# HKUDS/GPT-ST

Hardware: AMD Instinct MI355X
Metric: pretrain steps/sec at (B=32,T=12,N=170,C=64) (higher is better)
Workload: dtype f32; 1 GPU; BASELINE configs[1]: PEMS08-shape synthetic pretrain step, per-GPU B=32 T=12 N=170 C=64 base=1, epoch 200/300 (adaptive mask + KL), fwd+loss+bwd+clip+Adam, hipGraph=True, 4 full optimiser steps on 4 different resident batches per graph replay; global_batch=32, parallelism=dp1

## Files before the change

gpt-st_amd/csrc/encin.hip:

```cpp
#include "common.h"

#define EI_T 12
GPTST_STAMP_TABLES(encin)

template <int C>
__global__ __launch_bounds__(256) void encin_fwd_kernel(const float* __restrict__ src, int lda, const float* __restrict__ mask, float fill,
                                                        const float* __restrict__ w, const float* __restrict__ bi, const float* __restrict__ G,
                                                        const float* __restrict__ Wbt, const float* __restrict__ bbt, float* __restrict__ out,
                                                        float* __restrict__ ab, float* __restrict__ wv, int N) {
    constexpr int LPR = C / 4, RPP = 256 / LPR, NQ = 256 / C;
    extern __shared__ __attribute__((aligned(16))) float smem[];
    float* part = smem;
    float* vec = part + NQ * 2 * C;
    float* al = vec + 3 * C;
    float* be = al + N;
    float* mm = be + N;
    const int bt = blockIdx.x, b = bt / EI_T, t = bt % EI_T, tid = threadIdx.x;
    GPTST_WG_BEGIN(); GPTST_STAMP(0);
    {
        const int q = tid / C, o = tid % C;
        const float* W = Wbt + (size_t)bt * C * C;
        float aw = 0.f, abv = 0.f;
#pragma unroll 8
        for (int i = q * (C / NQ); i < (q + 1) * (C / NQ); ++i) {
            const float x = W[(size_t)i * C + o];
            aw = fmaf(w[i], x, aw);
            abv = fmaf(bi[i], x, abv);
        }
        part[(q * 2 + 0) * C + o] = aw;
        part[(q * 2 + 1) * C + o] = abv;
    }
    GPTST_STAMP(1);
    for (int n = tid; n < N; n += 256) {
        float g[EI_T];
        const float* gr = G + (size_t)n * EI_T * EI_T + t * EI_T;
#pragma unroll
        for (int k = 0; k < EI_T / 4; ++k) { const float4 v = ld4(gr + 4 * k); g[4 * k] = v.x; g[4 * k + 1] = v.y; g[4 * k + 2] = v.z; g[4 * k + 3] = v.w; }
        float sv[EI_T], mk[EI_T];
#pragma unroll
        for (int u = 0; u < EI_T; ++u) {
            const size_t r = ((size_t)b * EI_T + u) * N + n;
            sv[u] = src[r * lda];
            mk[u] = mask ? mask[r] : 1.f;
        }
        float a_ = 0.f, b_ = 0.f, mt = 0.f;
#pragma unroll
        for (int u = 0; u < EI_T; ++u) {
            const float m = mk[u] != 0.f ? sv[u] : fill;
            a_ = fmaf(g[u], m, a_);
            b_ += g[u];
            if (u == t) mt = m;
        }
        al[n] = a_; be[n] = b_; mm[n] = mt;
        ab[((size_t)bt * N + n) * 2] = a_;
        ab[((size_t)bt * N + n) * 2 + 1] = b_;
    }
    __syncthreads();
    GPTST_STAMP(2);
    if (tid < C) {
        float s0 = 0.f, s1 = 0.f;
#pragma unroll
        for (int q = 0; q < NQ; ++q) { s0 += part[(q * 2 + 0) * C + tid]; s1 += part[(q * 2 + 1) * C + tid]; }
        vec[tid] = s0; vec[C + tid] = s1; vec[2 * C + tid] = bbt[(size_t)bt * C + tid] + bi[tid];
        wv[(size_t)bt * 2 * C + tid] = s0;
        wv[(size_t)bt * 2 * C + C + tid] = s1;
    }
    __syncthreads();
    const int slot = tid / LPR, c4 = tid % LPR;
    const float4 wW = ld4(vec + 4 * c4), bW = ld4(vec + C + 4 * c4), cst = ld4(vec + 2 * C + 4 * c4), w4 = ld4(w + 4 * c4);
    for (int n = slot; n < N; n += RPP) {
        const float a_ = al[n], b_ = be[n], m = mm[n];
        float4 y = f4fma(a_, wW, f4fma(b_, bW, f4fma(m, w4, cst)));
        y.x = lrelu(y.x); y.y = lrelu(y.y); y.z = lrelu(y.z); y.w = lrelu(y.w);
        st4(out + ((size_t)bt * N + n) * C + 4 * c4, y);
    }
    GPTST_STAMP(3); GPTST_WG_END();
}

template <int C>
__global__ __launch_bounds__(256) void encin_bwd_kernel(const float* __restrict__ dPre, const float* __restrict__ src, int lda,
                                                        const float* __restrict__ mask, float fill, const float* __restrict__ w,
                                                        const float* __restrict__ bi, const float* __restrict__ Wbt, const float* __restrict__ ab,
                                                        const float* __restrict__ wv, float* __restrict__ dWb, float* __restrict__ dG,
                                                        float* __restrict__ dinp, int N, int B) {
    constexpr int LPR = C / 4, RPP = 256 / LPR, U = 4;
    extern __shared__ __attribute__((aligned(16))) float smem[];
    float* red = smem;
    float* vec = red + RPP * 4 * C;
    float* as_ = vec + 6 * C;
    float* cs_ = as_ + N;
    const int bt = blockIdx.x, b = bt / EI_T, t = bt % EI_T, tid = threadIdx.x;
    GPTST_WG_BEGIN(); GPTST_STAMP(0);
    if (tid < 2 * C) vec[4 * C + tid] = wv[(size_t)bt * 2 * C + tid];
    __syncthreads();
    const int slot = tid / LPR, c4 = tid % LPR;
    const float4 wW = ld4(vec + 4 * C + 4 * c4), bW = ld4(vec + 5 * C + 4 * c4);
    float4 A = f4zero(), Bv = f4zero(), Cv = f4zero(), Mv = f4zero();
    for (int n0 = slot; n0 < N; n0 += RPP * U) {
        float4 d[U];
        float a_[U], b_[U], m_[U];
#pragma unroll
        for (int u = 0; u < U; ++u) {
            const int n = min(n0 + u * RPP, N - 1);
            const size_t r = (size_t)bt * N + n;
            d[u] = ld4(dPre + r * C + 4 * c4);
            a_[u] = ab[r * 2]; b_[u] = ab[r * 2 + 1];
            m_[u] = (mask ? mask[r] : 1.f) != 0.f ? src[r * lda] : fill;
        }
#pragma unroll
        for (int u = 0; u < U; ++u) {
            const int n = n0 + u * RPP;
            const bool ok = n < N;
            const float4 dd = ok ? d[u] : f4zero();
            A = f4fma(a_[u], dd, A); Bv = f4fma(b_[u], dd, Bv); Cv = f4add(Cv, dd); Mv = f4fma(m_[u], dd, Mv);
            const float pa = group_sum<LPR>(f4dot(dd, wW)), pc = group_sum<LPR>(f4dot(dd, bW));
            if (ok && c4 == 0) { as_[n] = pa; cs_[n] = pc; }
        }
    }
    GPTST_STAMP(1);
    st4(red + (slot * 4 + 0) * C + 4 * c4, A); st4(red + (slot * 4 + 1) * C + 4 * c4, Bv);
    st4(red + (slot * 4 + 2) * C + 4 * c4, Cv); st4(red + (slot * 4 + 3) * C + 4 * c4, Mv);
    __syncthreads();
    for (int i = tid; i < 4 * C; i += 256) {
        float s = 0.f;
#pragma unroll 4
        for (int sl = 0; sl < RPP; ++sl) s += red[(sl * 4 + i / C) * C + i % C];
        vec[i] = s;
    }
    __syncthreads();
    GPTST_STAMP(2);
    float* row = dWb + (size_t)bt * (C * C + C);
    for (int f = tid; f < C * C / 4; f += 256) {
        const int i = f / LPR, o4 = f % LPR;
        const float wi = w[i], bb = bi[i];
        const float4 a4 = ld4(vec + 4 * o4), b4 = ld4(vec + C + 4 * o4);
        st4(row + (size_t)i * C + 4 * o4, make_float4(fmaf(wi, a4.x, bb * b4.x), fmaf(wi, a4.y, bb * b4.y), fmaf(wi, a4.z, bb * b4.z), fmaf(wi, a4.w, bb * b4.w)));
    }
    if (tid < C) row[C * C + tid] = vec[2 * C + tid];
    {
        constexpr int PP = 256 / C;
        const int i = tid / PP, pq = tid % PP;
        const float* Wr = Wbt + (size_t)bt * C * C + (size_t)i * C + pq * (C / PP);
        float p1 = 0.f, p2 = 0.f;
#pragma unroll
        for (int k = 0; k < C / PP / 4; ++k) {
            const float4 x = ld4(Wr + 4 * k);
            p1 += f4dot(x, ld4(vec + pq * (C / PP) + 4 * k));
            p2 += f4dot(x, ld4(vec + C + pq * (C / PP) + 4 * k));
        }
        p1 = group_sum<PP>(p1); p2 = group_sum<PP>(p2);
        if (pq == 0) {
            dinp[(size_t)bt * 2 * C + i] = vec[3 * C + i] + p1;
            dinp[(size_t)bt * 2 * C + C + i] = vec[2 * C + i] + p2;
        }
    }
    GPTST_STAMP(3);
    for (int n = tid; n < N; n += 256) {
        const float a = as_[n], c = cs_[n];
        float v[EI_T];
#pragma unroll
        for (int u = 0; u < EI_T; ++u) {
            const size_t r = ((size_t)b * EI_T + u) * N + n;
            const float m = (mask ? mask[r] : 1.f) != 0.f ? src[r * lda] : fill;
            v[u] = fmaf(m, a, c);
        }
        float* o = dG + ((size_t)b * N + n) * EI_T * EI_T + t * EI_T;
#pragma unroll
        for (int k = 0; k < EI_T / 4; ++k) st4(o + 4 * k, make_float4(v[4 * k], v[4 * k + 1], v[4 * k + 2], v[4 * k + 3]));
    }
    GPTST_STAMP(4); GPTST_WG_END();
}

extern "C" int gptst_encin_ht1_fwd(const float* src, int lda, const float* mask, float fill, const float* w, const float* bi, const float* G,
                                   const float* Wbt, const float* bbt, float* out, float* ab, float* wv, int B, int T, int N, int C, void* stream) {
    if (!src || !w || !bi || !G || !Wbt || !bbt || !out || !ab || !wv || B <= 0 || N <= 0 || lda <= 0) return GPTST_EARG;
    if (T != EI_T || (C != 64 && C != 128)) return GPTST_ESHAPE;
    const size_t smem = ((size_t)(256 / C) * 2 * C + 3 * C + 3 * (size_t)N) * sizeof(float);
    if (smem > 64 * 1024) return GPTST_ESHAPE;
    if (C == 64) hipLaunchKernelGGL((encin_fwd_kernel<64>), dim3(B * T), dim3(256), smem, (hipStream_t)stream, src, lda, mask, fill, w, bi, G, Wbt, bbt, out, ab, wv, N);
    else hipLaunchKernelGGL((encin_fwd_kernel<128>), dim3(B * T), dim3(256), smem, (hipStream_t)stream, src, lda, mask, fill, w, bi, G, Wbt, bbt, out, ab, wv, N);
    GPTST_CHECK_LAUNCH();
    return GPTST_OK;
}

extern "C" int gptst_encin_ht1_bwd(const float* dPre, const float* src, int lda, const float* mask, float fill, const float* w, const float* bi,
                                   const float* Wbt, const float* ab, const float* wv, float* dWb, float* dG, float* dinp, int B, int T, int N,
                                   int C, void* stream) {
    if (!dPre || !src || !w || !bi || !Wbt || !ab || !wv || !dWb || !dG || !dinp || B <= 0 || N <= 0 || lda <= 0) return GPTST_EARG;
    if (T != EI_T || (C != 64 && C != 128)) return GPTST_ESHAPE;
    const size_t smem = ((size_t)(256 / (C / 4)) * 4 * C + 6 * C + 2 * (size_t)N) * sizeof(float);
    if (smem > 64 * 1024) return GPTST_ESHAPE;
    if (C == 64) hipLaunchKernelGGL((encin_bwd_kernel<64>), dim3(B * T), dim3(256), smem, (hipStream_t)stream, dPre, src, lda, mask, fill, w, bi, Wbt, ab, wv, dWb, dG, dinp, N, B);
    else hipLaunchKernelGGL((encin_bwd_kernel<128>), dim3(B * T), dim3(256), smem, (hipStream_t)stream, dPre, src, lda, mask, fill, w, bi, Wbt, ab, wv, dWb, dG, dinp, N, B);
    GPTST_CHECK_LAUNCH();
    return GPTST_OK;
}
```

gpt-st_amd/csrc/poolgen.hip:

```cpp
#include "common.h"
#include "poolgen_dev.h"
#include <algorithm>
#include <vector>

#define PG_ROWS 16


#ifndef PJ_OCC
#define PJ_OCC 6
#endif

#define PG_MAXROWS 64
template <int V>
__device__ __forceinline__ void pj_fwd(const PJob& a, int bx, int by, int rows, float* __restrict__ embs ) {
    const float* __restrict__ emb = a.emb;
    const float* __restrict__ pool = a.pool;
    float* __restrict__ out = a.out;
    const int cols = a.cols, K = a.K, R = a.R;
    const int r0 = by * rows, nr = min(R, r0 + rows) - r0;
    for (int i = threadIdx.x; i < nr * PG_MAXK; i += 256) {
        const int r = i / PG_MAXK, k = i % PG_MAXK;
        embs[i] = k < K ? emb[(size_t)(r0 + r) * K + k] : 0.f;
    }
    const int c4 = bx * 256 + threadIdx.x;
    const bool ok = V * c4 < cols;
    float4 pv[PG_MAXK];
#pragma unroll
    for (int k = 0; k < PG_MAXK; ++k) pv[k] = (k < K && ok) ? ldv<V>(pool + (size_t)k * cols + V * c4) : f4zero();
    __syncthreads();
    if (!ok) return;
#pragma unroll 2
    for (int r = 0; r < nr; ++r) {
        float4 acc = f4zero();
#pragma unroll
        for (int k = 0; k < PG_MAXK; k += 4) {
            const float4 e = ld4(embs + r * PG_MAXK + k);
            acc = f4fma(e.x, pv[k], acc); acc = f4fma(e.y, pv[k + 1], acc); acc = f4fma(e.z, pv[k + 2], acc); acc = f4fma(e.w, pv[k + 3], acc);
        }
        stv<V>(out + (size_t)(r0 + r) * cols + V * c4, acc);
    }
}




#define PJ_DET_T 1024
__global__ __launch_bounds__(PJ_DET_T) void pool_emb_det_kernel(PJobs t) {
    __shared__ float fold[PJ_DET_T / 64][16][17];
    const int lane = threadIdx.x & 63, wave = threadIdx.x >> 6;
    const int i = lane & 15, kk = lane >> 4;
    int q0 = 0;
    for (int q = 1; q < t.n; ++q) if ((int)blockIdx.x >= t.j[q].blk0) q0 = q;
    const int g0 = t.j[q0].blk0, tile = blockIdx.x - g0;
    f32x4 acc = {0.f, 0.f, 0.f, 0.f};
    int chunk_id = 0, first = q0;
    for (int q = 0; q <= q0; ++q) {
        const PJob& a = t.j[q];
        if (a.blk0 != g0) continue;
        if (q < first) first = q;
        const bool v4 = ((a.cols | a.ldx) & 3) == 0;
        const int nch = (a.cols + 255) / 256;
        for (int ch = 0; ch < nch; ++ch, ++chunk_id) {
            if ((chunk_id & (PJ_DET_T / 64 - 1)) != wave) continue;
            if (v4) pj_emb_accum<4>(a, tile, ch, acc, threadIdx.x); else pj_emb_accum<1>(a, tile, ch, acc, threadIdx.x);
        }
    }
#pragma unroll
    for (int r = 0; r < 4; ++r) fold[wave][kk * 4 + r][i] = acc[r];
    __syncthreads();
    if (threadIdx.x < 256) {
        const int R = t.j[first].R, K = t.j[first].K;
        const int rr = threadIdx.x >> 4, k = threadIdx.x & 15, orow = tile * 16 + rr;
        float s = 0.f;
#pragma unroll
        for (int w = 0; w < PJ_DET_T / 64; ++w) s += fold[w][rr][k];
        if (orow < R && k < K) t.j[first].out[(size_t)orow * K + k] += s;
    }
}

__global__ __launch_bounds__(256, PJ_OCC) void pool_jobs_kernel(PJobs t, int fwd_rows, int fwd_mfma) {
    __shared__ __attribute__((aligned(16))) float fold[4][PG_MAXK][65];
    int p = 0;
    for (int q = 1; q < t.n; ++q) if ((int)blockIdx.x >= t.j[q].blk0) p = q;
    const PJob& a = t.j[p];
    const int rel = blockIdx.x - a.blk0, bx = rel % a.nbx, by = rel / a.nbx;
    const bool v4 = ((a.cols | a.ldx) & 3) == 0;
    if (a.kind == PJ_FWD) {
        if (v4 && fwd_mfma) pj_fwd_mfma(a, bx, by, fwd_mfma, threadIdx.x);
        else if (v4) pj_fwd<4>(a, bx, by, fwd_rows, &fold[0][0][0]);
        else pj_fwd<1>(a, bx, by, fwd_rows, &fold[0][0][0]);
    }
    else if (a.kind == PJ_GRAM) pj_gram(a, rel, &fold[0][0][0], 256);
    else if (a.kind == PJ_BWD_POOL) { if (v4) pj_bwd_pool<4>(a, bx, fold, threadIdx.x); else pj_bwd_pool<1>(a, bx, fold, threadIdx.x); }
// ... 3 lines not shown
thread_local int g_pg_rows = PG_ROWS;
thread_local int g_pg_sort = 1;
thread_local int g_pg_mfma = 1;
static int pj_blocks(PJob& j) {
    const int V = ((j.cols | j.ldx) & 3) ? 1 : 4;
    if (j.kind == PJ_FWD && V == 4 && g_pg_mfma) { j.nbx = (j.cols + 255) / 256; return j.nbx * ((j.R + PG_MFMA_ROWS - 1) / PG_MFMA_ROWS); }
    if (j.kind == PJ_FWD) { j.nbx = ((j.cols + V - 1) / V + 255) / 256; return j.nbx * ((j.R + g_pg_rows - 1) / g_pg_rows); }
    if (j.kind == PJ_GRAM) { const int nb = pj_gram_rows(j.K, j.cols); j.nbx = (j.R + nb - 1) / nb; return j.nbx; }
    if (j.kind == PJ_BWD_POOL) { j.nbx = (j.cols + 16 * V - 1) / (16 * V); return j.nbx; }
    j.nbx = (j.R + 15) / 16;
    return j.nbx * (((j.cols + 255) / 256 + 3) / 4);
}

extern "C" int gptst_pool_jobs_gram_rows(int K, int cols) { return (K <= 0 || K > PG_MAXK || cols <= 0 || cols % 12) ? 0 : pj_gram_rows(K, cols); }

static int pj_launch(PJobs& t, hipStream_t st) {
    int nb = 0;
    for (int p = 0; p < t.n; ++p) {
        PJob& j = t.j[p];
        if (j.R <= 0 || j.K <= 0 || j.K > PG_MAXK || j.cols <= 0 || j.nsplit <= 0 || !j.out) return GPTST_EARG;
        if ((j.kind == PJ_FWD || j.kind == PJ_BWD_POOL || j.kind == PJ_GRAM) && !j.emb) return GPTST_EARG;
        if (j.kind == PJ_GRAM && (!j.pool || j.cols % 12 || pj_gram_rows(j.K, j.cols) <= 0)) return GPTST_EARG;
        if ((j.kind == PJ_BWD_POOL || j.kind == PJ_BWD_EMB) && !j.x) return GPTST_EARG;
        if ((j.kind == PJ_FWD || j.kind == PJ_BWD_EMB) && !j.pool) return GPTST_EARG;
        j.blk0 = nb;
        if (j.ldx <= 0) j.ldx = j.cols;
        if (j.ldx < j.cols) return GPTST_EARG;
        nb += pj_blocks(j);
    }
    if (nb == 0) return GPTST_OK;
    hipLaunchKernelGGL(pool_jobs_kernel, dim3(nb), dim3(256), 0, st, t, g_pg_rows, g_pg_mfma ? PG_MFMA_ROWS : 0);
    GPTST_CHECK_LAUNCH();
    return GPTST_OK;
}

GPTST_INTERNAL int gptst_pj_embed_table(PJobs* t, int njobs, const int* kind, const void* const* emb, const void* const* pool, const void* const* out,
                                        const int* R, const int* K, const int* cols, int* nf, int* nvb, int* ngw) {
    if (njobs > PJ_MAX || !g_pg_mfma) return GPTST_ESHAPE;
    t->n = 0;
    *nf = *nvb = *ngw = 0;
    for (int pass = 0; pass < 2; ++pass) {
        for (int p = 0; p < njobs; ++p) {
            const int kd = kind ? kind[p] : (int)PJ_FWD;
            if (kd != PJ_FWD && kd != PJ_GRAM) return GPTST_ESHAPE;
            if ((kd == PJ_GRAM) != (pass == 1)) continue;
            PJob j{(const float*)emb[p], nullptr, (const float*)pool[p], (float*)out[p], R[p], K[p], cols[p], 1, 0, kd, 0, cols[p]};
            if (!j.emb || !j.pool || !j.out || j.R <= 0 || j.K <= 0 || j.K > PG_MAXK || j.cols <= 0) return GPTST_EARG;
            if (kd == PJ_FWD) {
                if (j.cols & 3) return GPTST_ESHAPE;
                j.blk0 = *nvb; *nvb += pj_blocks(j); ++*nf;
            } else {
                if (j.cols % 12 || pj_gram_rows(j.K, j.cols) <= 0) return GPTST_EARG;
                j.blk0 = *ngw; *ngw += pj_blocks(j);
            }
            t->j[t->n++] = j;
        }
    }
    return GPTST_OK;
}

GPTST_INTERNAL int gptst_pj_reduce_table(PJobs* t, int njobs, const int* kind, const void* const* emb, const void* const* x, const void* const* pool,
                                         const void* const* out, const int* R, const int* K, const int* cols, const int* nsplit, const int* ldx,
                                         int* npool, int* npb, int* neb) {
    if (njobs > PJ_MAX || g_deterministic) return GPTST_ESHAPE;
    t->n = 0;
    *npool = *npb = *neb = 0;
    for (int pass = 0; pass < 2; ++pass) {
        for (int p = 0; p < njobs; ++p) {
            if (kind[p] != PJ_BWD_POOL && kind[p] != PJ_BWD_EMB) return GPTST_ESHAPE;
            if ((kind[p] == PJ_BWD_EMB) != (pass == 1)) continue;
            PJob j{(const float*)emb[p], (const float*)x[p], (const float*)pool[p], (float*)out[p], R[p], K[p], cols[p], nsplit[p], 0, kind[p], 0, ldx ? ldx[p] : 0};
            if (j.R <= 0 || j.K <= 0 || j.K > PG_MAXK || j.cols <= 0 || j.nsplit <= 0 || !j.out || !j.x) return GPTST_EARG;
            if (kind[p] == PJ_BWD_POOL ? !j.emb : !j.pool) return GPTST_EARG;
            if (j.ldx <= 0) j.ldx = j.cols;
            if (j.ldx < j.cols) return GPTST_EARG;
            if (pass == 0) { j.blk0 = *npb; *npb += pj_blocks(j); ++*npool; }
            else { j.blk0 = *neb; *neb += pj_blocks(j); }
            t->j[t->n++] = j;
        }
    }
    return GPTST_OK;
}

extern "C" int gptst_pool_jobs(int njobs, const int* kind, const void* const* emb, const void* const* x, const void* const* pool,
                               const void* const* out, const int* R, const int* K, const int* cols, const int* nsplit, const int* ldx,
                               void* stream) {
    if (njobs < 0 || (njobs && (!kind || !emb || !x || !pool || !out || !R || !K || !cols || !nsplit))) return GPTST_EARG;
    for (int p = 0; p < njobs; ++p) if (kind[p] < PJ_FWD || kind[p] > PJ_GRAM) return GPTST_EARG;
    auto job = [&](int p) {
        return PJob{(const float*)emb[p], (const float*)x[p], (const float*)pool[p], (float*)out[p], R[p], K[p], cols[p], nsplit[p],
                    0, kind[p], 0, ldx ? ldx[p] : 0};
    };
    const bool det = g_deterministic != 0;
    std::vector<int> ord(njobs);
    std::vector<long> cost(njobs);
    for (int p = 0; p < njobs; ++p) {
        ord[p] = p;
        const long rr = (long)R[p] * nsplit[p], cc = cols[p];
        cost[p] = kind[p] == PJ_BWD_POOL ? rr * (cc < 64 ? cc : 64) : kind[p] == PJ_BWD_EMB ? 16L * nsplit[p] * (cc < 1024 ? cc : 1024)
                : kind[p] == PJ_FWD ? 64L * (cc < 256 ? cc : 256) : 1L;
    }
    if (g_pg_sort) std::stable_sort(ord.begin(), ord.end(), [&](int a, int b) { return cost[a] > cost[b]; });
    PJobs t; t.n = 0;
    for (int o = 0; o < njobs; ++o) {
        const int p = ord[o];
        if (det && kind[p] == PJ_BWD_EMB) continue;
        t.j[t.n++] = job(p);
        if (t.n == PJ_MAX) { const int rc = pj_launch(t, (hipStream_t)stream); if (rc) return rc; t.n = 0; }
    }
    if (t.n) { const int rc = pj_launch(t, (hipStream_t)stream); if (rc) return rc; }
    if (!det) return GPTST_OK;
    PJobs g; g.n = 0;
    int nb = 0;
    auto flush = [&]() {
        if (g.n) { hipLaunchKernelGGL(pool_emb_det_kernel, dim3(nb), dim3(PJ_DET_T), 0, (hipStream_t)stream, g); g.n = 0; nb = 0; }
    };
    for (int p = 0; p < njobs; ++p) {
        if (kind[p] != PJ_BWD_EMB) continue;
        bool seen = false;
        for (int q = 0; q < p; ++q) if (kind[q] == PJ_BWD_EMB && out[q] == out[p]) seen = true;
        if (seen) continue;
        int members = 0;
        for (int q = p; q < njobs; ++q) if (kind[q] == PJ_BWD_EMB && out[q] == out[p]) ++members;
        if (members > PJ_MAX) return GPTST_EARG;
        if (g.n + members > PJ_MAX) flush();
        const int tiles = (R[p] + 15) / 16;
        for (int q = p; q < njobs; ++q) {
            if (kind[q] != PJ_BWD_EMB || out[q] != out[p]) continue;
            if (R[q] != R[p] || K[q] != K[p]) return GPTST_EARG;
            PJob j = job(q);
            if (!j.x || !j.pool || !j.out || j.R <= 0 || j.K <= 0 || j.K > PG_MAXK || j.cols <= 0 || j.nsplit <= 0) return GPTST_EARG;
            if (j.ldx <= 0) j.ldx = j.cols;
            if (j.ldx < j.cols) return GPTST_EARG;
            j.blk0 = nb; j.nbx = tiles;
            g.j[g.n++] = j;
        }
        nb += tiles;
    }
    flush();
    GPTST_CHECK_LAUNCH();
    return GPTST_OK;
}

extern thread_local int g_wgrad_ns_override;
extern thread_local int g_wgrad_ns0_override;
extern thread_local int g_apply_v1;
extern thread_local int g_apply_tpw;
extern thread_local int g_tl_nb;
extern thread_local int g_wgrad_v1;
extern thread_local int g_apply128_v1;
extern thread_local int g_apply128_minwg;
extern thread_local int g_tl_mfma;
extern thread_local int g_cap_route_v2;
extern thread_local int g_cap_bwd_noroles;
extern thread_local int g_cap_split;
extern thread_local int g_cap_split_roles;
extern "C" int gptst_tune(int id, int value) {
    if (id == 15) g_tl_mfma = value;
    if (id == 20) g_cap_route_v2 = value;
    if (id == 23) g_cap_bwd_noroles = value;
    if (id == 25) g_cap_split = value;
    if (id == 26) g_cap_split_roles = value;
    if (id == 19) g_pg_sort = value;
    if (id == 1 && value > 0 && value <= PG_MAXROWS) g_pg_rows = value;
    if (id == 6 && value > 0) g_tl_nb = value;
    if (id == 2) g_wgrad_ns_override = value;
    if (id == 5) g_wgrad_ns0_override = value;
    if (id == 3) g_apply_v1 = value;
    if (id == 4) g_apply_tpw = value;
    if (id == 7) g_wgrad_v1 = value;
    if (id == 8) g_apply128_v1 = value;
    if (id == 24 && value > 0) g_apply128_minwg = value;
    if (id == 10) g_pg_mfma = value;
    return GPTST_OK;
}

extern "C" int gptst_poolgen_fwd_multi(const float* emb, int nprob, const void* pools, const void* outs, const int* cols, int R, int K,
                                       void* stream) {
    if (!emb || !pools || !outs || !cols || nprob <= 0 || nprob > PJ_MAX || K > PG_MAXK || K <= 0) return GPTST_EARG;
    PJobs t; t.n = nprob;
    for (int p = 0; p < nprob; ++p)
        t.j[p] = PJob{emb, nullptr, ((const float* const*)pools)[p], ((float* const*)outs)[p], R, K, cols[p], 1, 0, PJ_FWD, 0, 0};
    return pj_launch(t, (hipStream_t)stream);
}

// ... 38 lines not shown
```

gpt-st_amd/csrc/poolgen_dev.h:

```cpp
#pragma once
#include "common.h"

#define PG_MAXK 16
#define PG_MFMA_ROWS 64
#define PJ_MAX 112
enum { PJ_FWD = 0, PJ_BWD_POOL = 1, PJ_BWD_EMB = 2, PJ_GRAM = 3 };
struct PJob {
    const float* emb;
    const float* x;
    const float* pool;
    float* out;
    int R, K, cols, nsplit;
    int blk0, kind, nbx, ldx;
};
struct PJobs { PJob j[PJ_MAX]; int n; };

__device__ __forceinline__ void pj_fwd_mfma(const PJob& a, int bx, int by, int rows, int tid) {
    const float* __restrict__ emb = a.emb;
    const float* __restrict__ pool = a.pool;
    float* __restrict__ out = a.out;
    const int cols = a.cols, K = a.K, R = a.R;
    const int lane = tid & 63, wave = tid >> 6, j = lane & 15, kk = lane >> 4;
    const int c = bx * 256 + wave * 64 + 4 * j;
    if (bx * 256 + wave * 64 >= cols) return;
    const bool cok = c < cols;
    const int nks = (K + 3) >> 2;
    float4 bf[4];
#pragma unroll
    for (int s = 0; s < 4; ++s) bf[s] = (cok && 4 * s + kk < K) ? ld4(pool + (size_t)(4 * s + kk) * cols + c) : f4zero();
    const int r0 = by * rows, r1 = min(R, r0 + rows);
    for (int rt = r0; rt < r1; rt += 16) {
        float av[4];
        const int row = rt + j;
#pragma unroll
        for (int s = 0; s < 4; ++s) av[s] = (row < r1 && 4 * s + kk < K) ? emb[(size_t)row * K + 4 * s + kk] : 0.f;
        f32x4 acc[4];
#pragma unroll
        for (int ct = 0; ct < 4; ++ct) acc[ct] = (f32x4){0.f, 0.f, 0.f, 0.f};
#pragma unroll
        for (int s = 0; s < 4; ++s) {
            if (s < nks) {
                acc[0] = __builtin_amdgcn_mfma_f32_16x16x4f32(av[s], bf[s].x, acc[0], 0, 0, 0);
                acc[1] = __builtin_amdgcn_mfma_f32_16x16x4f32(av[s], bf[s].y, acc[1], 0, 0, 0);
                acc[2] = __builtin_amdgcn_mfma_f32_16x16x4f32(av[s], bf[s].z, acc[2], 0, 0, 0);
                acc[3] = __builtin_amdgcn_mfma_f32_16x16x4f32(av[s], bf[s].w, acc[3], 0, 0, 0);
            }
        }
        if (cok) {
#pragma unroll
            for (int r = 0; r < 4; ++r) {
                const int orow = rt + 4 * kk + r;
                if (orow < r1) st4(out + (size_t)orow * cols + c, make_float4(acc[0][r], acc[1][r], acc[2][r], acc[3][r]));
            }
        }
    }
}

#define PJ_GRAM_SCR (4 * PG_MAXK * 65)
__host__ __device__ inline int pj_gram_rows(int K, int cols) {
    const int nb = (PJ_GRAM_SCR - K * cols) / cols;
    return nb > 16 ? 16 : nb;
}
__device__ __forceinline__ void pj_gram(const PJob& a, int bx, float* __restrict__ scr, int nt) {
    const int K = a.K, cols = a.cols, Hm = cols / 12, NB = pj_gram_rows(K, cols);
    float* pl = scr;
    float* As = scr + K * cols;
    const int r0 = bx * NB, nr = min(NB, a.R - r0);
    for (int i = threadIdx.x; i < K * cols; i += nt) pl[i] = a.pool[i];
    __syncthreads();
    for (int i = threadIdx.x; i < nr * cols; i += nt) {
        const int r = i / cols, c = i % cols;
        const float* __restrict__ e = a.emb + (size_t)(r0 + r) * K;
        float acc = 0.f;
        for (int k = 0; k < K; ++k) acc = fmaf(e[k], pl[k * cols + c], acc);
        As[i] = acc;
    }
    __syncthreads();
    for (int i = threadIdx.x; i < nr * 144; i += nt) {
        const int r = i / 144, t = (i % 144) / 12, u = i % 12;
        const float* ar = As + r * cols;
        float s = 0.f;
        for (int h = 0; h < Hm; ++h) s = fmaf(ar[h * 12 + t], ar[h * 12 + u], s);
        a.out[(size_t)(r0 + r) * 144 + i % 144] = s;
    }
}

#ifndef PJ_UC
#define PJ_UC 4
#endif
#ifndef PJ_NU
#define PJ_NU 4
#endif
template <int V> __device__ __forceinline__ float4 ldv(const float* p) { return ld4(p); }
template <> __device__ __forceinline__ float4 ldv<1>(const float* p) { return make_float4(*p, 0.f, 0.f, 0.f); }
template <int V> __device__ __forceinline__ void stv(float* p, float4 v) { st4(p, v); }
template <> __device__ __forceinline__ void stv<1>(float* p, float4 v) { *p = v.x; }

template <int V>
__device__ __forceinline__ void pj_bwd_pool(const PJob& a, int bx, float (*fold)[PG_MAXK][65], int tid) {
    constexpr int SLAB = 16 * V;
    const float* __restrict__ emb = a.emb;
    const float* __restrict__ dW = a.x;
    float* __restrict__ dpool = a.out;
    const int cols = a.cols, R = a.R, K = a.K, RR = R * a.nsplit;
    const int lane = tid & 63, wave = tid >> 6;
    const int j = lane & 15, kk = lane >> 4;
    int nchunk = 4;
    if (nchunk * 16 > RR) nchunk = (RR + 15) / 16;
    int per = (RR + nchunk - 1) / nchunk;
    per = (per + 3) & ~3;
    const int r0 = wave < nchunk ? wave * per : RR, r1 = min(RR, r0 + per);
    const int c = bx * SLAB + V * j;
    const bool cok = c < cols;
    f32x4 acc[V];
#pragma unroll
    for (int e = 0; e < V; ++e) acc[e] = (f32x4){0.f, 0.f, 0.f, 0.f};
    constexpr int NU = PJ_NU;
    const int cl = cok ? c : 0;
    for (int rb = r0; rb < r1; rb += 4 * NU) {
        float av[NU];
        float4 b[NU];
#pragma unroll
        for (int u = 0; u < NU; ++u) {
            const int row = min(rb + 4 * u + kk, r1 - 1);
            av[u] = emb[(size_t)(row % R) * K + min(j, K - 1)];
            b[u] = ldv<V>(dW + (size_t)row * a.ldx + cl);
        }
        SB();
#pragma unroll
        for (int u = 0; u < NU; ++u) {
            const float a_ = (rb + 4 * u + kk < r1 && j < K) ? av[u] : 0.f;
            acc[0] = __builtin_amdgcn_mfma_f32_16x16x4f32(a_, b[u].x, acc[0], 0, 0, 0);
            if (V == 4) {
                acc[V > 1 ? 1 : 0] = __builtin_amdgcn_mfma_f32_16x16x4f32(a_, b[u].y, acc[V > 1 ? 1 : 0], 0, 0, 0);
                acc[V > 2 ? 2 : 0] = __builtin_amdgcn_mfma_f32_16x16x4f32(a_, b[u].z, acc[V > 2 ? 2 : 0], 0, 0, 0);
                acc[V > 3 ? 3 : 0] = __builtin_amdgcn_mfma_f32_16x16x4f32(a_, b[u].w, acc[V > 3 ? 3 : 0], 0, 0, 0);
            }
        }
    }
#pragma unroll
    for (int e = 0; e < V; ++e)
#pragma unroll
        for (int r = 0; r < 4; ++r) fold[wave][kk * 4 + r][V * j + e] = acc[e][r];
    __syncthreads();
    for (int o = tid; o < PG_MAXK * SLAB; o += 256) {
        const int k = o / SLAB, cc = o % SLAB, col = bx * SLAB + cc;
        if (k < K && col < cols) {
            float* d = dpool + (size_t)k * cols + col;
            *d += (fold[0][k][cc] + fold[1][k][cc]) + (fold[2][k][cc] + fold[3][k][cc]);
        }
    }
}

template <int V>
__device__ __forceinline__ void pj_emb_accum(const PJob& a, int bx, int chunk, f32x4& acc, int tid) {
    constexpr int chunk_cols = 256;
    const int lane = tid & 63;
    const int i = lane & 15, kk = lane >> 4;
    const int R = a.R, K = a.K;
    const int row = bx * 16 + i;
    const float* __restrict__ w = a.x;
    const float* __restrict__ pl = a.pool;
    const int cc = a.cols, ns = a.nsplit, ldx = a.ldx;
    const int cbeg = chunk * chunk_cols, cend = min(cc, cbeg + chunk_cols);
    if (cbeg >= cc) return;
    if (V == 4) {
        constexpr int UC = PJ_UC;
        const int rowc = min(row, R - 1), ic = min(i, K - 1);
        const bool rok = row < R, kok = i < K;
        for (int c0 = cbeg; c0 < cend; c0 += 16 * UC) {
            float4 av[UC], b[UC];
#pragma unroll
            for (int u = 0; u < UC; ++u) {
                const int c = min(c0 + 16 * u + 4 * kk, cc - 4);
                av[u] = ld4(w + (size_t)rowc * ldx + c);
                b[u] = ld4(pl + (size_t)ic * cc + c);
            }
            for (int s = 1; s < ns; ++s) {
#pragma unroll
                for (int u = 0; u < UC; ++u) {
                    const int c = min(c0 + 16 * u + 4 * kk, cc - 4);
                    av[u] = f4add(av[u], ld4(w + ((size_t)s * R + rowc) * ldx + c));
                }
            }
            SB();
#pragma unroll
            for (int u = 0; u < UC; ++u) {
                const bool ok = c0 + 16 * u + 4 * kk < cend;
                const float4 a_ = (ok && rok) ? av[u] : f4zero();
                const float4 b_ = (ok && kok) ? b[u] : f4zero();
                acc = __builtin_amdgcn_mfma_f32_16x16x4f32(a_.x, b_.x, acc, 0, 0, 0);
                acc = __builtin_amdgcn_mfma_f32_16x16x4f32(a_.y, b_.y, acc, 0, 0, 0);
                acc = __builtin_amdgcn_mfma_f32_16x16x4f32(a_.z, b_.z, acc, 0, 0, 0);
                acc = __builtin_amdgcn_mfma_f32_16x16x4f32(a_.w, b_.w, acc, 0, 0, 0);
            }
        }
    } else {
        for (int c = cbeg + kk; c < cend + kk; c += 4) {
            float av = 0.f, b = 0.f;
            if (c < cend) {
                if (row < R) for (int s = 0; s < ns; ++s) av += w[((size_t)s * R + row) * ldx + c];
                if (i < K) b = pl[(size_t)i * cc + c];
            }
            acc = __builtin_amdgcn_mfma_f32_16x16x4f32(av, b, acc, 0, 0, 0);
        }
    }
}

template <int V>
__device__ __forceinline__ void pj_bwd_emb(const PJob& a, int bx, int by, int tid) {
    const int lane = tid & 63, wave = tid >> 6;
    const int i = lane & 15, kk = lane >> 4;
    f32x4 acc = {0.f, 0.f, 0.f, 0.f};
    pj_emb_accum<V>(a, bx, by * 4 + wave, acc, tid);
#pragma unroll
    for (int r = 0; r < 4; ++r) {
        const int orow = bx * 16 + kk * 4 + r;
        if (orow < a.R && i < a.K && (by * 4 + wave) * 256 < a.cols) atomicAdd(a.out + (size_t)orow * a.K + i, acc[r]);
    }
}
```

gpt-st_amd/csrc/timefeat.hip:

```cpp
#include "common.h"

struct TfParams {
    const float *wd, *bd, *ww, *bw, *w1, *b1, *w2, *b2, *w3, *b3;
};
struct TfGrads {
    float *wd, *bd, *ww, *bw, *w1, *b1, *w2, *b2, *w3, *b3;
};

template <int E, int NT = 256> struct TfCfg { static constexpr int ROWS = NT / E; };

template <int E>
__device__ __forceinline__ float tf_matvec(const float (&wrow)[E], float b, const float* __restrict__ xline) {
    float s = b;
#pragma unroll
    for (int i = 0; i < E; ++i) s = fmaf(wrow[i], xline[i], s);
    return s;
}

template <int E>
__device__ __forceinline__ float tf_input(const TfParams& p, const float* __restrict__ tidx, int r, int e, int K) {
    float s = p.bd[e] + p.bw[e];
    for (int k = 0; k < K; ++k) {
        s = fmaf(p.wd[e * K + k], tidx[((size_t)r * K + k) * 2 + 0], s);
        s = fmaf(p.ww[e * K + k], tidx[((size_t)r * K + k) * 2 + 1], s);
    }
    return s;
}

#define TF_SH_FLOATS (7 * 128 * 3)

template <int E>
__device__ __forceinline__ void tf_fwd_body(const TfParams& p, const float* __restrict__ tidx, float* __restrict__ out,
                                            int rows, int K, int blk, float* __restrict__ shraw) {
    constexpr int ROWS = TfCfg<E>::ROWS;
    float (*line)[E + 1] = reinterpret_cast<float (*)[E + 1]>(shraw);
    const int e = threadIdx.x % E, rl = threadIdx.x / E;
    const int r = blk * ROWS + rl;
    const bool valid = r < rows;
    float w1[E], w2[E], w3[E];
#pragma unroll
    for (int i = 0; i < E; ++i) { w1[i] = p.w1[e * E + i]; w2[i] = p.w2[e * E + i]; w3[i] = p.w3[e * E + i]; }
    line[rl][e] = valid ? tf_input<E>(p, tidx, r, e, K) : 0.f;
    __syncthreads();
    float h = fmaxf(tf_matvec<E>(w1, p.b1[e], line[rl]), 0.f);
    __syncthreads();
    line[rl][e] = h;
    __syncthreads();
    h = fmaxf(tf_matvec<E>(w2, p.b2[e], line[rl]), 0.f);
    __syncthreads();
    line[rl][e] = h;
    __syncthreads();
    h = tf_matvec<E>(w3, p.b3[e], line[rl]);
    if (valid) out[(size_t)r * E + e] = h;
}

template <bool DET> __device__ __forceinline__ void tf_add(float* p, float v) { if (DET) *p += v; else atomicAdd(p, v); }

template <int E, bool DET, int NT>
__device__ __forceinline__ void tf_bwd_body(const TfParams& p, const TfGrads& g, const float* __restrict__ tidx,
                                            const float* __restrict__ dout, int rows, int K, int blk, float* __restrict__ shraw) {
    constexpr int ROWS = TfCfg<E, NT>::ROWS;
    float (*sh)[ROWS][E + 1] = reinterpret_cast<float (*)[ROWS][E + 1]>(shraw);
    const int tid = threadIdx.x, e = tid % E, rl = tid / E;
    const int r = blk * ROWS + rl;
    const bool valid = r < rows;
    float w1[E], w2[E], w3[E], c1[E], c2[E], c3[E];
#pragma unroll
    for (int i = 0; i < E; ++i) {
        w1[i] = p.w1[e * E + i]; w2[i] = p.w2[e * E + i]; w3[i] = p.w3[e * E + i];
        c1[i] = p.w1[i * E + e]; c2[i] = p.w2[i * E + e]; c3[i] = p.w3[i * E + e];
    }
    const float h0 = valid ? tf_input<E>(p, tidx, r, e, K) : 0.f;
    sh[0][rl][e] = h0;
    __syncthreads();
    const float h1 = fmaxf(tf_matvec<E>(w1, p.b1[e], sh[0][rl]), 0.f);
    sh[1][rl][e] = h1;
    __syncthreads();
    const float h2 = fmaxf(tf_matvec<E>(w2, p.b2[e], sh[1][rl]), 0.f);
    sh[2][rl][e] = h2;
    const float d3 = valid ? dout[(size_t)r * E + e] : 0.f;
    sh[3][rl][e] = d3;
    __syncthreads();
    const float z2 = h2 > 0.f ? tf_matvec<E>(c3, 0.f, sh[3][rl]) : 0.f;
    sh[4][rl][e] = z2;
    __syncthreads();
    const float z1 = h1 > 0.f ? tf_matvec<E>(c2, 0.f, sh[4][rl]) : 0.f;
    sh[5][rl][e] = z1;
    __syncthreads();
    const float z0 = tf_matvec<E>(c1, 0.f, sh[5][rl]);
    sh[6][rl][e] = z0;
    __syncthreads();
    const int nrow = min(ROWS, rows - blk * ROWS);
    for (int idx = tid; idx < 3 * E * E; idx += NT) {
        const int which = idx / (E * E), eo = (idx / E) % E, i = idx % E;
        const int ga = which == 0 ? 3 : (which == 1 ? 4 : 5), gb = which == 0 ? 2 : (which == 1 ? 1 : 0);
        float s = 0.f;
        for (int rr = 0; rr < nrow; ++rr) s = fmaf(sh[ga][rr][eo], sh[gb][rr][i], s);
        float* dst = which == 0 ? g.w3 : (which == 1 ? g.w2 : g.w1);
        tf_add<DET>(dst + eo * E + i, s);
    }
    for (int idx = tid; idx < 4 * E; idx += NT) {
        const int which = idx / E, eo = idx % E;
        const int ga = which == 0 ? 3 : (which == 1 ? 4 : (which == 2 ? 5 : 6));
        float s = 0.f;
        for (int rr = 0; rr < nrow; ++rr) s += sh[ga][rr][eo];
        if (which == 0) tf_add<DET>(g.b3 + eo, s);
        else if (which == 1) tf_add<DET>(g.b2 + eo, s);
        else if (which == 2) tf_add<DET>(g.b1 + eo, s);
        else { tf_add<DET>(g.bd + eo, s); tf_add<DET>(g.bw + eo, s); }
    }
    for (int idx = tid; idx < 2 * E * K; idx += NT) {
        const int ch = idx / (E * K), eo = (idx / K) % E, k = idx % K;
        float s = 0.f;
        for (int rr = 0; rr < nrow; ++rr)
            s = fmaf(sh[6][rr][eo], tidx[((size_t)(blk * ROWS + rr) * K + k) * 2 + ch], s);
        tf_add<DET>((ch == 0 ? g.wd : g.ww) + eo * K + k, s);
    }
}

#define TF_MAXJ 16
struct TfJob { TfParams p; TfGrads g; const float* tidx; float* out; const float* dout; int rows, K, E, blk0; };
struct TfJobs { TfJob j[TF_MAXJ]; int n; };

#define TF_DET_T 1024
template <int BWD>
__global__ __launch_bounds__(BWD == 2 ? TF_DET_T : 256) void timefeat_jobs_kernel(TfJobs t) {
    constexpr int NT = BWD == 2 ? TF_DET_T : 256;
    __shared__ float shraw[TF_SH_FLOATS * (NT / 256)];
    int q = 0;
    if (BWD == 2) q = blockIdx.x;
    else for (int i = 1; i < t.n; ++i) if ((int)blockIdx.x >= t.j[i].blk0) q = i;
    const TfJob& a = t.j[q];
    const int blk = blockIdx.x - a.blk0;
    const int nblk = (a.rows + NT / a.E - 1) / (NT / a.E);
#define TF_CASE(EE)                                                                              \
    case EE:                                                                                     \
        if (BWD == 2) { for (int b2 = 0; b2 < nblk; ++b2) { tf_bwd_body<EE, true, NT>(a.p, a.g, a.tidx, a.dout, a.rows, a.K, b2, shraw); __syncthreads(); } } \
        else if (BWD == 1) tf_bwd_body<EE, false, NT>(a.p, a.g, a.tidx, a.dout, a.rows, a.K, blk, shraw); \
        else tf_fwd_body<EE>(a.p, a.tidx, a.out, a.rows, a.K, blk, shraw);                       \
        break;
    switch (a.E) { TF_CASE(2) TF_CASE(4) TF_CASE(8) TF_CASE(16) default: break; }
#undef TF_CASE
}

static int tf_launch(TfJobs& t, int bwd, hipStream_t st) {
    int nb = 0;
    for (int q = 0; q < t.n; ++q) {
        TfJob& a = t.j[q];
        if (!a.p.wd || !a.tidx || a.rows <= 0 || a.K <= 0 || (bwd ? (!a.dout || !a.g.wd) : !a.out)) return GPTST_EARG;
        if (a.E != 2 && a.E != 4 && a.E != 8 && a.E != 16) return GPTST_ESHAPE;
        const int rows_per = 256 / a.E;
        a.blk0 = nb;
        nb += (a.rows + rows_per - 1) / rows_per;
    }
    if (bwd && g_deterministic) hipLaunchKernelGGL(timefeat_jobs_kernel<2>, dim3(t.n), dim3(TF_DET_T), 0, st, t);
    else if (bwd) hipLaunchKernelGGL(timefeat_jobs_kernel<1>, dim3(nb), dim3(256), 0, st, t);
    else hipLaunchKernelGGL(timefeat_jobs_kernel<0>, dim3(nb), dim3(256), 0, st, t);
    GPTST_CHECK_LAUNCH();
    return GPTST_OK;
}

extern "C" int gptst_timefeat_fwd(const float* wd, const float* bd, const float* ww, const float* bw, const float* w1, const float* b1,
                                  const float* w2, const float* b2, const float* w3, const float* b3, const float* tidx, float* out,
                                  int rows, int K, int E, void* stream) {
    TfJobs t; t.n = 1;
    t.j[0] = TfJob{TfParams{wd, bd, ww, bw, w1, b1, w2, b2, w3, b3}, TfGrads{}, tidx, out, nullptr, rows, K, E, 0};
    return tf_launch(t, 0, (hipStream_t)stream);
}

extern "C" int gptst_timefeat_bwd(const float* wd, const float* bd, const float* ww, const float* bw, const float* w1, const float* b1,
                                  const float* w2, const float* b2, const float* w3, const float* b3, float* gwd, float* gbd, float* gww,
                                  float* gbw, float* gw1, float* gb1, float* gw2, float* gb2, float* gw3, float* gb3, const float* tidx,
                                  const float* dout, int rows, int K, int E, void* stream) {
    TfJobs t; t.n = 1;
    t.j[0] = TfJob{TfParams{wd, bd, ww, bw, w1, b1, w2, b2, w3, b3}, TfGrads{gwd, gbd, gww, gbw, gw1, gb1, gw2, gb2, gw3, gb3}, tidx,
                   nullptr, dout, rows, K, E, 0};
    return tf_launch(t, 1, (hipStream_t)stream);
}

extern "C" int gptst_timefeat_jobs(int njobs, int bwd, const void* const* params, const void* const* grads, const float* tidx,
                                   const void* const* io, const int* rows, const int* K, const int* E, void* stream) {
    if (njobs <= 0 || njobs > TF_MAXJ || !params || !io || !rows || !K || !E || (bwd && !grads)) return GPTST_EARG;
    TfJobs t; t.n = njobs;
    for (int q = 0; q < njobs; ++q) {
        const float* const* pp = (const float* const*)params + 10 * q;
        TfGrads g{};
        if (bwd) { float* const* gg = (float* const*)grads + 10 * q; g = TfGrads{gg[0], gg[1], gg[2], gg[3], gg[4], gg[5], gg[6], gg[7], gg[8], gg[9]}; }
        t.j[q] = TfJob{TfParams{pp[0], pp[1], pp[2], pp[3], pp[4], pp[5], pp[6], pp[7], pp[8], pp[9]}, g, tidx,
                       bwd ? nullptr : (float*)io[q], bwd ? (const float*)io[q] : nullptr, rows[q], K[q], E[q], 0};
    }
    return tf_launch(t, bwd, (hipStream_t)stream);
}
```

gpt-st_amd/csrc/tmix.hip:

```cpp
#include "common.h"

#define TT 12
#define TT2 144

__global__ __launch_bounds__(256) void gram_fwd_kernel(const float* __restrict__ A, float* __restrict__ G, int N, int Hm) {
    const int idx = blockIdx.x * 256 + threadIdx.x;
    if (idx >= N * TT2) return;
    const int n = idx / TT2, t = (idx % TT2) / TT, u = idx % TT;
    const float* a = A + (size_t)n * Hm * TT;
    float s = 0.f;
    for (int h = 0; h < Hm; ++h) s = fmaf(a[h * TT + t], a[h * TT + u], s);
    G[idx] = s;
}

__global__ __launch_bounds__(256) void gram_bwd_kernel(const float* __restrict__ A, const float* __restrict__ dG,
                                                       float* __restrict__ dA, int N, int Hm, int nsplit) {
    __shared__ float gs[TT2];
    const int gn = blockIdx.x, l = gn / N, n = gn % N;
    if (threadIdx.x < TT2) {
        const float* g = dG + ((size_t)l * nsplit * N + n) * TT2 + threadIdx.x;
        float part[8];
#pragma unroll
        for (int k = 0; k < 8; ++k) part[k] = 0.f;
        for (int sp0 = 0; sp0 < nsplit; sp0 += 8) {
            float v[8];
#pragma unroll
            for (int k = 0; k < 8; ++k) v[k] = sp0 + k < nsplit ? g[(size_t)(sp0 + k) * N * TT2] : 0.f;
#pragma unroll
            for (int k = 0; k < 8; ++k) part[k] += v[k];
        }
        gs[threadIdx.x] = ((part[0] + part[1]) + (part[2] + part[3])) + ((part[4] + part[5]) + (part[6] + part[7]));
    }
    __syncthreads();
    if (threadIdx.x >= Hm * TT) return;
    const int h = threadIdx.x / TT, t = threadIdx.x % TT;
    const float* a = A + ((size_t)gn * Hm + h) * TT;
    float s = 0.f;
#pragma unroll
    for (int u = 0; u < TT; ++u) s = fmaf(a[u], gs[t * TT + u] + gs[u * TT + t], s);
    dA[((size_t)gn * Hm + h) * TT + t] = s;
}

template <int C, bool ADD_DPRE>
__global__ __launch_bounds__(256) void tmix_kernel(const float* __restrict__ X, const float* __restrict__ G,
                                                   const float* __restrict__ dOut, const float* __restrict__ Y,
                                                   float* __restrict__ out, int N) {
    constexpr int LPR = C / 4;
    constexpr int NPB = 256 / LPR;
    __shared__ float Gs[NPB][TT2];
    const int b = blockIdx.y, n0 = blockIdx.x * NPB;
    for (int i = threadIdx.x; i < NPB * TT2; i += 256) {
        const int nl = i / TT2;
        Gs[nl][i % TT2] = (n0 + nl < N) ? G[(size_t)(n0 + nl) * TT2 + i % TT2] : 0.f;
    }
    __syncthreads();
    const int nl = threadIdx.x / LPR, c4 = threadIdx.x % LPR;
    const int n = n0 + nl;
    if (n >= N) return;
    const size_t base = ((size_t)b * TT * N + n) * C + 4 * c4;
    const size_t tstride = (size_t)N * C;
    float4 x[TT];
#pragma unroll
    for (int u = 0; u < TT; ++u) x[u] = ld4(X + base + u * tstride);
#pragma unroll
    for (int t = 0; t < TT; ++t) {
        float4 acc = f4zero();
        if (ADD_DPRE) {
            const float4 d = ld4(dOut + base + t * tstride), y = ld4(Y + base + t * tstride);
            acc = make_float4(d.x * lrelu_grad_from_out(y.x), d.y * lrelu_grad_from_out(y.y),
                              d.z * lrelu_grad_from_out(y.z), d.w * lrelu_grad_from_out(y.w));
        }
#pragma unroll
        for (int u = 0; u < TT; ++u) acc = f4fma(Gs[nl][t * TT + u], x[u], acc);
        st4(out + base + t * tstride, acc);
    }
}

template <int C>
__global__ __launch_bounds__(256) void tmix_dgraph_kernel(const float* __restrict__ dR, const float* __restrict__ X,
                                                          float* __restrict__ dG, int B, int N) {
    __shared__ float red[4][TT2];
    const int n = blockIdx.x, lane = threadIdx.x & 63, wave = threadIdx.x >> 6;
    const int i = lane & 15, kk = lane >> 4;
    f32x4 acc = {0.f, 0.f, 0.f, 0.f};
    const size_t tstride = (size_t)N * C;
    for (int b = wave; b < B; b += 4) {
        const size_t base = ((size_t)b * TT * N + n) * C + 4 * kk;
        float4 a[C / 16], x[C / 16];
#pragma unroll
        for (int q = 0; q < C / 16; ++q) {
            a[q] = f4zero(); x[q] = f4zero();
            if (i < TT) {
                a[q] = ld4(dR + base + i * tstride + 16 * q);
                x[q] = ld4(X + base + i * tstride + 16 * q);
            }
        }
#pragma unroll
        for (int q = 0; q < C / 16; ++q) {
            acc = __builtin_amdgcn_mfma_f32_16x16x4f32(a[q].x, x[q].x, acc, 0, 0, 0);
            acc = __builtin_amdgcn_mfma_f32_16x16x4f32(a[q].y, x[q].y, acc, 0, 0, 0);
            acc = __builtin_amdgcn_mfma_f32_16x16x4f32(a[q].z, x[q].z, acc, 0, 0, 0);
            acc = __builtin_amdgcn_mfma_f32_16x16x4f32(a[q].w, x[q].w, acc, 0, 0, 0);
        }
    }
#pragma unroll
    for (int r = 0; r < 4; ++r) {
        const int t = kk * 4 + r, u = i;
        if (t < TT && u < TT) red[wave][t * TT + u] = acc[r];
    }
    __syncthreads();
    if (threadIdx.x < TT2) {
        const int e = threadIdx.x;
        dG[(size_t)n * TT2 + e] = red[0][e] + red[1][e] + red[2][e] + red[3][e];
    }
}

template <int C, int CH = 0>
__global__ __launch_bounds__(256, 2) void tmix_bwd_dgraph_kernel(const float* __restrict__ dR, const float* __restrict__ X,
                                                                 const float* __restrict__ G, const float* __restrict__ dOut,
                                                                 const float* __restrict__ Y, float* __restrict__ dX,
                                                                 float* __restrict__ dG, int B, int N) {
    constexpr int Q = C / 16, H2 = C / 64, P = C + 4;
    __shared__ float red[4][TT2];
// ... 25 lines not shown
            for (int s = 0; s < 4; ++s)
#pragma unroll
                for (int hf = 0; hf < H2; ++hf) {
                    st4(&tile[wave][0][4 * kk + s][64 * hf + 4 * j], drc[s][hf]);
                    st4(&tile[wave][1][4 * kk + s][64 * hf + 4 * j], xc[s][hf]);
                }
        }
        SB();
        float4 drr[Q], xr[Q];
#pragma unroll
        for (int q = 0; q < Q; ++q) {
            drr[q] = f4zero(); xr[q] = f4zero();
            if (j < TT) { drr[q] = ld4(&tile[wave][0][j][16 * q + 4 * kk]); xr[q] = ld4(&tile[wave][1][j][16 * q + 4 * kk]); }
        }
        SB();
#pragma unroll
        for (int q = 0; q < Q; ++q) {
            g0 = __builtin_amdgcn_mfma_f32_16x16x4f32(drr[q].x, xr[q].x, g0, 0, 0, 0);
            g1 = __builtin_amdgcn_mfma_f32_16x16x4f32(drr[q].y, xr[q].y, g1, 0, 0, 0);
            g2 = __builtin_amdgcn_mfma_f32_16x16x4f32(drr[q].z, xr[q].z, g2, 0, 0, 0);
            g3 = __builtin_amdgcn_mfma_f32_16x16x4f32(drr[q].w, xr[q].w, g3, 0, 0, 0);
        }
        f32x4 acc[4 * H2];
#pragma unroll
        for (int ct = 0; ct < 4 * H2; ++ct) acc[ct] = (f32x4){0.f, 0.f, 0.f, 0.f};
#pragma unroll
        for (int s = 0; s < 4; ++s)
#pragma unroll
            for (int hf = 0; hf < H2; ++hf) {
                acc[4 * hf + 0] = __builtin_amdgcn_mfma_f32_16x16x4f32(ga[s], drc[s][hf].x, acc[4 * hf + 0], 0, 0, 0);
                acc[4 * hf + 1] = __builtin_amdgcn_mfma_f32_16x16x4f32(ga[s], drc[s][hf].y, acc[4 * hf + 1], 0, 0, 0);
                acc[4 * hf + 2] = __builtin_amdgcn_mfma_f32_16x16x4f32(ga[s], drc[s][hf].z, acc[4 * hf + 2], 0, 0, 0);
                acc[4 * hf + 3] = __builtin_amdgcn_mfma_f32_16x16x4f32(ga[s], drc[s][hf].w, acc[4 * hf + 3], 0, 0, 0);
            }
        SB();
        if (kk < 3) {
#pragma unroll
            for (int r = 0; r < 4; ++r)
#pragma unroll
                for (int hf = 0; hf < H2; ++hf) {
                    const float4 d = doc[r][hf];
                    float4 o4;
                    if (CH == 0) {
                        const float4 y = yc[r][hf];
                        o4 = make_float4(fmaf(d.x, lrelu_grad_from_out(y.x), acc[4 * hf + 0][r]), fmaf(d.y, lrelu_grad_from_out(y.y), acc[4 * hf + 1][r]),
                                         fmaf(d.z, lrelu_grad_from_out(y.z), acc[4 * hf + 2][r]), fmaf(d.w, lrelu_grad_from_out(y.w), acc[4 * hf + 3][r]));
                    } else {
                        o4 = make_float4(d.x + acc[4 * hf + 0][r], d.y + acc[4 * hf + 1][r], d.z + acc[4 * hf + 2][r], d.w + acc[4 * hf + 3][r]);
                        if (CH == 2) {
                            const float4 x = xc[r][hf];
                            o4.x *= lrelu_grad_from_out(x.x); o4.y *= lrelu_grad_from_out(x.y); o4.z *= lrelu_grad_from_out(x.z); o4.w *= lrelu_grad_from_out(x.w);
                        }
                    }
                    st4(dX + base + (4 * kk + r) * tstride + 64 * hf + 4 * j, o4);
                }
        }
    }
#pragma unroll
    for (int r = 0; r < 4; ++r) {
        const int t = kk * 4 + r, u = j;
        if (t < TT && u < TT) red[wave][t * TT + u] = (g0[r] + g1[r]) + (g2[r] + g3[r]);
    }
    __syncthreads();
    if (threadIdx.x < TT2) {
        const int e = threadIdx.x;
        dG[(size_t)n * TT2 + e] = (red[0][e] + red[1][e]) + (red[2][e] + red[3][e]);
    }
}

extern "C" int gptst_gram_fwd(const float* A, float* G, int N, int Hm, void* stream) {
    if (!A || !G) return GPTST_EARG;
    hipLaunchKernelGGL(gram_fwd_kernel, dim3((N * TT2 + 255) / 256), dim3(256), 0, (hipStream_t)stream, A, G, N, Hm);
    GPTST_CHECK_LAUNCH();
    return GPTST_OK;
}

extern "C" int gptst_gram_bwd(const float* A, const float* dG, float* dA, int L, int N, int Hm, int nsplit, void* stream) {
    if (!A || !dG || !dA || L <= 0 || N <= 0 || nsplit <= 0 || Hm * TT > 256) return GPTST_EARG;
    hipLaunchKernelGGL(gram_bwd_kernel, dim3(L * N), dim3(256), 0, (hipStream_t)stream, A, dG, dA, N, Hm, nsplit);
    GPTST_CHECK_LAUNCH();
    return GPTST_OK;
}

extern "C" int gptst_tmix_bwd_chain(const float* dR, const float* X, const float* G, const float* dPre, int premul, float* dX, float* dG,
                                    int B, int T, int N, int C, void* stream) {
    if (!dR || !X || !G || !dPre || !dX || !dG || T != TT || B < 1 || N < 1) return GPTST_EARG;
    hipStream_t st = (hipStream_t)stream;
    if (C == 64 && premul) hipLaunchKernelGGL((tmix_bwd_dgraph_kernel<64, 2>), dim3(N), dim3(256), 0, st, dR, X, G, dPre, nullptr, dX, dG, B, N);
    else if (C == 64) hipLaunchKernelGGL((tmix_bwd_dgraph_kernel<64, 1>), dim3(N), dim3(256), 0, st, dR, X, G, dPre, nullptr, dX, dG, B, N);
    else if (C == 128 && premul) hipLaunchKernelGGL((tmix_bwd_dgraph_kernel<128, 2>), dim3(N), dim3(256), 0, st, dR, X, G, dPre, nullptr, dX, dG, B, N);
    else if (C == 128) hipLaunchKernelGGL((tmix_bwd_dgraph_kernel<128, 1>), dim3(N), dim3(256), 0, st, dR, X, G, dPre, nullptr, dX, dG, B, N);
    else return GPTST_ESHAPE;
    GPTST_CHECK_LAUNCH();
    return GPTST_OK;
}

extern "C" int gptst_tmix(const float* X, const float* G, const float* dOut, const float* Y, float* out, int B, int T, int N,
                          int C, void* stream) {
    if (!X || !G || !out || T != TT) return GPTST_EARG;
    if (dOut && !Y) return GPTST_EARG;
    hipStream_t st = (hipStream_t)stream;
    if (C == 64) {
        dim3 grid((N + 15) / 16, B);
        if (dOut) hipLaunchKernelGGL((tmix_kernel<64, true>), grid, dim3(256), 0, st, X, G, dOut, Y, out, N);
        else hipLaunchKernelGGL((tmix_kernel<64, false>), grid, dim3(256), 0, st, X, G, dOut, Y, out, N);
    } else if (C == 128) {
        dim3 grid((N + 7) / 8, B);
        if (dOut) hipLaunchKernelGGL((tmix_kernel<128, true>), grid, dim3(256), 0, st, X, G, dOut, Y, out, N);
        else hipLaunchKernelGGL((tmix_kernel<128, false>), grid, dim3(256), 0, st, X, G, dOut, Y, out, N);
    } else return GPTST_ESHAPE;
    GPTST_CHECK_LAUNCH();
    return GPTST_OK;
}

extern "C" int gptst_tmix_dgraph(const float* dR, const float* X, float* dG, int B, int T, int N, int C, void* stream) {
    if (!dR || !X || !dG || T != TT) return GPTST_EARG;
    hipStream_t st = (hipStream_t)stream;
    if (C == 64) hipLaunchKernelGGL((tmix_dgraph_kernel<64>), dim3(N), dim3(256), 0, st, dR, X, dG, B, N);
    else if (C == 128) hipLaunchKernelGGL((tmix_dgraph_kernel<128>), dim3(N), dim3(256), 0, st, dR, X, dG, B, N);
    else return GPTST_ESHAPE;
    GPTST_CHECK_LAUNCH();
    return GPTST_OK;
}

extern "C" int gptst_tmix_bwd(const float* dR, const float* X, const float* G, const float* dOut, const float* Y, float* dX, float* dG,
                              int B, int T, int N, int C, void* stream) {
    if (!dR || !X || !G || !dOut || !Y || !dX || !dG || T != TT || B < 1 || N < 1) return GPTST_EARG;
    hipStream_t st = (hipStream_t)stream;
    if (C == 64) hipLaunchKernelGGL((tmix_bwd_dgraph_kernel<64>), dim3(N), dim3(256), 0, st, dR, X, G, dOut, Y, dX, dG, B, N);
    else if (C == 128) hipLaunchKernelGGL((tmix_bwd_dgraph_kernel<128>), dim3(N), dim3(256), 0, st, dR, X, G, dOut, Y, dX, dG, B, N);
    else return GPTST_ESHAPE;
    GPTST_CHECK_LAUNCH();
    return GPTST_OK;
}
```

gpt-st_amd/engine.py:

```python
import contextlib
import gc
import os
import threading
from typing import Any, NamedTuple

import torch

from . import _C, ops
from .ops import (EPI_ADD_DPRE, EPI_ADD_PREMUL, EPI_LRELU, EPI_PREMUL, EPI_PLAIN, EPI_RES_LRELU, MODE_NODE, MODE_SHARED, MODE_TIME, PRO_DPRE, PRO_NONE)

TF_NAMES = ("ln_day", "ln_week", "ln1", "ln2", "ln")


class ZeroArena:

    def __init__(self, device):
        self.device, self.buf, self.off, self.need = device, None, 0, 0

    def begin(self, zero=True):
        pending = None
        if self.buf is None or self.buf.numel() < self.need:
            self.buf = torch.zeros(max(self.need, 1), device=self.device) if self.need else None
        elif self.buf is not None:
            if zero:
                self.buf.zero_()
            else:
                pending = self.buf
        self.off, self.need = 0, 0
        return pending

    def zeros(self, *shape):
        n = 1
        for d in shape:
            n *= d
        n4 = (n + 3) // 4 * 4
        self.need += n4
        if self.buf is None or self.off + n4 > self.buf.numel():
            return torch.zeros(*shape, device=self.device)
        t = self.buf[self.off:self.off + n].view(*shape)
        self.off += n4
        return t


class _Context(threading.local):
    ARENA = None
    NODE_REDUCE = None
    NO_HANDOFFS = False


CTX = _Context()




class Reductions:

    def __init__(self):
        self.jobs = ops.PoolJobs()
        self.late = ops.PoolJobs()
        self.no_carry = False
        self.grams = []
        self.tf = []
        self.keep = []
        self.on_bucket = None
        self.nbucket = 0
        self.bucket_inline = False
        self.fork_side = None
        self.forked = False
        self._dG = self._dA = None

    def take_carry(self, mb):
        if not CARRY_RED or self.no_carry or self.on_bucket is not None or CTX.NODE_REDUCE is not None or not self.jobs.jobs:
            return None
        take, rest, nb = [], [], 0.0
        for j in self.jobs.jobs:
            b = 4.0 * j.R * j.cols * j.nsplit / 2 ** 20
            if j.kind in (ops.PoolJobs.BWD_POOL, ops.PoolJobs.BWD_EMB) and nb + b <= mb and len(take) < 100 and (j.cols | j.ldx) % 4 == 0:
                take.append(j); nb += b
            else:
                rest.append(j)
        if not take:
            return None
        self.jobs.jobs = rest
        c = ops.PoolJobs()
        c.jobs = take
        return c

    def untake(self, carry):
        if carry is not None and carry.jobs:
            self.jobs.jobs = carry.jobs + self.jobs.jobs
            carry.jobs = []

    def gram(self, A, dG, dA, N, nsG):
        self.grams.append((A, dG, dA, N, nsG))

    def timefeat(self, p, g, pfx, tidx, dout, spg=False):
        self.tf.append(_tf_job(p, pfx, tidx, spg)._replace(grads=_tf_tensors(g, pfx), dout=dout))

    def flush_async(self, tidx):
        if self.bucket_inline and self.on_bucket is not None and self.nbucket == 0 and (self.jobs.jobs or self.late.jobs or self.grams or self.tf):
            self._run(tidx)
            self.fork_side.wait_stream(torch.cuda.current_stream())
            with torch.cuda.stream(self.fork_side):
                self.on_bucket(0)
            self.forked = True
            self.nbucket += 1

    def flush(self, tidx):
        self._run(tidx)
        if self.forked:
            torch.cuda.current_stream().wait_stream(self.fork_side)
            self.forked = False

    def _run(self, tidx):
        gr, self.grams = sorted(self.grams, key=lambda t: t[0].data_ptr()), []
        while gr:
            A, dG, dA, N, nsG = gr.pop(0)
            while gr and gr[0][0].data_ptr() == A.data_ptr() + 4 * A.numel() and gr[0][1].data_ptr() == dG.data_ptr() + 4 * dG.numel() \
                    and gr[0][2].data_ptr() == dA.data_ptr() + 4 * dA.numel() and gr[0][3:] == (N, nsG):
                A2, dG2, dA2 = gr.pop(0)[:3]
                A = torch.as_strided(A, (A.shape[0] + A2.shape[0],) + tuple(A.shape[1:]), A.stride())
                dG = torch.as_strided(dG, (dG.shape[0] + dG2.shape[0],) + tuple(dG.shape[1:]), dG.stride())
                dA = torch.as_strided(dA, (dA.shape[0] + dA2.shape[0],) + tuple(dA.shape[1:]), dA.stride())
            ops.gram_bwd(A, dG, out=dA, layers=A.shape[0] // N, nsplit=nsG)
        self.jobs.jobs, self.late.jobs = self.jobs.jobs + self.late.jobs, []
        self.jobs.launch()
        tf, self.tf = self.tf, []
        ops.timefeat_jobs_bwd(tf, tidx)
        self.keep = []


def _zeros(ref, *shape):
    if CTX.ARENA is not None:
        return CTX.ARENA.zeros(*shape)
    return torch.zeros(*shape, device=ref.device)


def _tf_tensors(d, pfx):
    out = []
    for n in TF_NAMES:
        out += [d[pfx + n + ".weight"], d[pfx + n + ".bias"]]
    return out


def _tf_job(p, pfx, tidx, spg=False):
    B, T = tidx.shape[0], tidx.shape[1]
    rows, K = (B, T) if spg else (B * T, 1)
    return ops.TimefeatJob(_tf_tensors(p, pfx), rows, K)


DROP_R = os.environ.get("GPTST_DROP_R", "0") == "1"


class HtSaved(NamedTuple):
    x: Any
    R: Any
    out: Any
    G: Any
    Wbt: Any


class WgradParts(NamedTuple):
    dW: Any
    ns: int
    db: Any


def _ht_fused_bwd(dims):
    return dims[3] == 64 and FUSE_HT_BWD


def hypertem_core_fwd(x, G, Wbt, bbt, dims):
    B, T, N, C = dims
    if C == 64:
        keep = not (DROP_R and _ht_fused_bwd(dims) and ops.wgrad_nsplit(MODE_TIME, B * T, N, C) == 1)
        R, out = ops.hypertem_fwd(x.view(B, T, N, C), G, Wbt, bbt, want_R=keep)
        R, out = (R.view(-1, C) if keep else None), out.view(-1, C)
    else:
        R = ops.tmix(x.view(B, T, N, C), G).view(-1, C)
        out = ops.apply(R, Wbt, MODE_TIME, B * T, N, bias=bbt, resid=x, epi=EPI_RES_LRELU)
    return out, HtSaved(x, R, out, G, Wbt)


FUSE_HT_BWD = True


def graph_grad_splits(dims):
    return dims[0] if dims[3] == 64 else 1


CHAIN128 = os.environ.get("GPTST_CHAIN128", "1") == "1"


def chain_ok(dims):
    return _ht_fused_bwd(dims) or (CHAIN128 and dims[3] == 128)


def _wb_parts(dWb, C, ns=1):
    return WgradParts(dWb[:, :C * C], ns, dWb[:, C * C:])


def _wgrad_parts(a, dout, out, mode, dims):
    B, T, N, C = dims
    dWb, ns = ops.wgrad(a, dout, mode, B * T, N, D2=out, pro=PRO_NONE if out is None else PRO_DPRE, colsum_d=True)
    return _wb_parts(dWb, C, ns)


def _genlin_bwd(dout, out, x, W, mode, dims, chain, premul=False):
    B, T, N, C = dims
    BT = B * T
    if C == 64:
        dx, dW, db, ns = ops.apply_wgrad(dout, None if chain else out, x, W, mode, BT, N, premul=chain and premul)
        return dx, WgradParts(dW, ns, db)
    if chain:
        dx = (ops.apply(dout, W, mode, BT, N, transw=True, resid2=x, epi=EPI_PREMUL) if premul
              else ops.apply(dout, W, mode, BT, N, transw=True))
        return dx, _wgrad_parts(x, dout, None, mode, dims)
    dx = ops.apply(dout, W, mode, BT, N, A2=out, transw=True, pro=PRO_DPRE)
    return dx, _wgrad_parts(x, dout, out, mode, dims)


def hypertem_core_bwd(saved, dout, dG_out, dims, chain=False, premul=False):
    B, T, N, C = dims
    x, R, out, G, Wbt = saved
    BT = B * T
    v = lambda a: a.view(B, T, N, C)
    assert not chain or chain_ok(dims)
    if _ht_fused_bwd(dims):
        dx, dWb, ns, _ = ops.hypertem_bwd_wgrad(v(dout), None if chain else v(out), v(x), G, Wbt, v(R) if R is not None else None, dG=dG_out,
                                                premul=chain and premul)
        return dx.view(-1, C), _wb_parts(dWb, C, ns)
    hp = _wgrad_parts(R, dout, None if chain else out, MODE_TIME, dims)
    if C == 64:
        dx, _, _ = ops.hypertem_bwd(v(dout), v(out), v(x), G, Wbt, dG=dG_out, want_dbias=False)
    elif chain:
        dR = ops.apply(dout, Wbt, MODE_TIME, BT, N, transw=True)
        dx, _ = ops.tmix_bwd_chain(v(dR), v(x), G, v(dout), premul=premul, dG=dG_out[0])
    else:
        dR = ops.apply(dout, Wbt, MODE_TIME, BT, N, A2=out, transw=True, pro=PRO_DPRE)
        dx, _ = ops.tmix_bwd(v(dR), v(x), G, v(dout), v(out), dG=dG_out[0])
    return dx.view(-1, C), hp


CARRY_RED = os.environ.get("GPTST_CARRY_RED", "1") == "1"
CARRY_MB = float(os.environ.get("GPTST_CARRY_MB", "25"))
CARRY_KL = os.environ.get("GPTST_CARRY_KL", "1") == "1"
PAIR_UNDER_DP = os.environ.get("GPTST_PAIR_UNDER_DP", "1") == "1"
PAIR_BWD = os.environ.get("GPTST_PAIR_BWD", "1") == "1"


@contextlib.contextmanager
def no_handoffs():
    from . import _C
    keep = (CTX.NO_HANDOFFS, _C.lib().value("gptst_mask_cooperative_state"))
    CTX.NO_HANDOFFS = True
    _C.lib().call("gptst_mask_cooperative", 0)
    try:
        yield
    finally:
        CTX.NO_HANDOFFS = keep[0]
        _C.lib().call("gptst_mask_cooperative", keep[1])


def pair_bwd_on():
    return PAIR_BWD and not CTX.NO_HANDOFFS


def cross_role():
    return 0 if CTX.NO_HANDOFFS else CROSS_ROLE


def _ht_pair_shape_ok(dims):
    B, T, N, C = dims
    if T != 12 or C != 64:
        return False
    ns = ops.wgrad_nsplit(MODE_TIME, B * T, N, C)
    rps = (-(-N // ns) + 1) & ~1
    return -(-N // rps) == ns


def ht_pair_ok(saved1, saved0, dims):
    return (pair_bwd_on() and dims[3] == 64 and not isinstance(saved1, EncIn) and saved1.R is not None and saved0.R is not None
            and _ht_fused_bwd(dims) and _ht_pair_shape_ok(dims))


class PendingH1:

    def __init__(self, saved, dd, dG, dWb):
        self.saved, self.dd, self.dG, self.dWb = saved, dd, dG, dWb


def ht_pair_bwd(saved1, saved0, dout, dG1, dG0, dims, dWb1=None):
    B, T, N, C = dims
    if not ht_pair_ok(saved1, saved0, dims):
        assert dWb1 is None
        return None
    s1, s0 = saved1, saved0
    v = lambda a: a.view(B, T, N, C)
    r = ops.hypertem_bwd_pair(v(dout), v(s1.x), s1.G, s1.Wbt, v(s1.R), v(s0.x), s0.G, s0.Wbt, v(s0.R), dG1, dG0, _zeros(dout, B), dWb1=dWb1)
    assert r is not None or dWb1 is None
    if r is None:
        return None
    dmid, dx0, dWb1, dWb0, ns = r
    return dx0.view(-1, C), _wb_parts(dWb1, C, ns), _wb_parts(dWb0, C, ns)


FUSE_CROSS = os.environ.get("GPTST_FUSE_CROSS", "1") == "1"
CAP_LIN = os.environ.get("GPTST_CAP_LIN", "1") == "1"
CROSS_ROLE = int(os.environ.get("GPTST_CROSS_ROLE", "1"))


class CapSaved(NamedTuple):
    x: Any
    out: Any
    rec: Any
    c: Any
    s: Any
    v: Any
    Ht: Any
    Rt: Any
    dyn: Any
    Wn: Any
    Y: Any


class CapParts(NamedTuple):
    wn: WgradParts
    ddyn: Any
    dlogit: Any


def cap_head_fwd(p, pfx, x, dadj, dyn, dims, num_route, HS, HT):
    B, T, N, C = dims
    c, s, Y = ops.cap_route_fwd(x.view(B, T, N, C), p[pfx + "ln_p.weight"], p[pfx + "ln_p.bias"], dadj, HS, num_route,
                                reduce_nodes=CTX.NODE_REDUCE, want_Y=True)
    fused = ops.cap_cross_rec_fwd(s, dyn, p[pfx + "mask_template"], c, B, T, N, HS, HT) if (FUSE_CROSS and CTX.NODE_REDUCE is None) else None
    if fused is not None:
        v, Ht, Rt, rec = fused
    else:
        v, Ht, Rt = ops.cap_cross_fwd(s, dyn, p[pfx + "mask_template"], B, T, HS, HT)
        rec = ops.cap_rec_fwd(c, v, N, C)
    return rec, c, (s, v, Ht, Rt, Y)


def cap_core_fwd(p, pfx, x, dadj, dyn, Wn, bn, dims, num_route, HS, HT):
    B, T, N, C = dims
    rec, c, (s, v, Ht, Rt, Y) = cap_head_fwd(p, pfx, x, dadj, dyn, dims, num_route, HS, HT)
    out = ops.apply(rec, Wn, MODE_NODE, B * T, N, bias=bn, resid=x, epi=EPI_RES_LRELU)
    return out, c, CapSaved(x, out, rec, c, s, v, Ht, Rt, dyn, Wn, Y)


CHAIN_FWD = os.environ.get("GPTST_CHAIN_FWD", "1") == "1"
# ... 198 lines not shown
        adj0 = p[which[0] + "hyperTem1.adj"]
        Hm = adj0.shape[1]
        A_all = torch.empty(L, N, Hm * T, device=tidx.device)
        G_all = torch.empty(L, N, T, T, device=tidx.device)
        for k, pfx in enumerate(which):
            sthcn[pfx] = _sthcn_gen_jobs(p, pfx, embs[3 * k:3 * k + 3], jobs, A_all[4 * k:4 * k + 4], dims, G_all[4 * k:4 * k + 4], (k, len(which)))
    now.launch()
    return GenAll(sthcn, gd, jobs if defer else None)


def sthcn_fwd(p, pfx, tidx, x, dims, num_route, gen=None, head=None, next_gen=None, kl=None):
    if gen is None:
        gen = gen_all(p, tidx, dims, which=(pfx,), guide=False).sthcn[pfx]
    ht = gen.ht
    cap = lambda i, x: cap_core_fwd(p, gen.cps[i], x, gen.dadj[i], gen.dyn[i], *gen.Wn[i], dims, num_route, gen.HS, gen.HT)
    pairs = chain_fwd_ok(dims)
    nhead = None
    x, h1 = head if head is not None else hypertem_core_fwd(x, *ht(0), dims)
    x, c1, sc1 = cap(0, x)
    if pairs:
        if kl is not None and kl.c1 is None:
            kl.c1 = c1
        (h2, h3), x = ht_chain_fwd(x, [ht(1), ht(2)], dims, kl)
    else:
        x, h2 = hypertem_core_fwd(x, *ht(1), dims)
        x, h3 = hypertem_core_fwd(x, *ht(2), dims)
    x, _, sc2 = cap(1, x)
    if pairs and next_gen is not None:
        (h4, h1n), xn = ht_chain_fwd(x, [ht(3), next_gen.ht(0)], dims, kl)
        x, nhead = h4.out, (xn, h1n)
    else:
        x, h4 = hypertem_core_fwd(x, *ht(3), dims)
    return x, c1, SthcnSaved(h1, h2, h3, h4, sc1, sc2, gen.emb, gen, gen.slot), nhead


def _grad_buffers(red, slot, N, T, HmT, ref, nsG):
    if slot is None:
        return torch.empty(4, nsG, N, T, T, device=ref.device), torch.empty(4, N, HmT, device=ref.device)
    k, n = slot
    if red._dG is None or red._dG.shape[0] != 4 * n:
        red._dG = torch.empty(4 * n, nsG, N, T, T, device=ref.device)
        red._dA = torch.empty(4 * n, N, HmT, device=ref.device)
    return red._dG[4 * k:4 * k + 4], red._dA[4 * k:4 * k + 4]


def sthcn_bwd(p, g, pfx, tidx, sv, dout, dims, red, chain=False, premul_in=False, defer_h1=False, after_pending=None):
    B, T, N, C = dims
    time_eb, teb, tes = sv.emb
    gn = sv.gen
    A_all, hts, cps, d, Hm, ds, HS, HT = gn.A_all, gn.hts, gn.cps, gn.d, gn.Hm, gn.ds, gn.HS, gn.HT
    ne, nes = p[pfx + "node_embeddings"], p[pfx + "node_embeddings_spg"]
    dne, dnes = g[pfx + "node_embeddings"], g[pfx + "node_embeddings_spg"]
    d_te, d_teb, d_tes = _zeros(time_eb, *time_eb.shape), _zeros(teb, *teb.shape), _zeros(tes, *tes.shape)
    nsG = graph_grad_splits(dims)
    dG_all, dA_all = _grad_buffers(red, sv.slot, N, T, Hm * T, dout, nsG)
    J = red.jobs
    e_te, e_node, e_spg, e_teb = (time_eb, d_te), (nes, dnes), (tes, d_tes), (teb, d_teb)

    if isinstance(dout, PendingH1):
        up = dout
        dd, _, hp4 = ht_pair_bwd(up.saved, sv.h4, up.dd, up.dG, dG_all[3], dims, dWb1=up.dWb)
        red.keep.append(up)
        if after_pending is not None:
            after_pending()
    else:
        dd, hp4 = hypertem_core_bwd(sv.h4, dout, dG_all[3], dims, chain, True)
    queue_ht(J, p, g, hts[3], hp4, *e_te)
    dd, cp2 = cap_core_bwd(p, g, cps[1], sv.c2, dd, dims, HS, HT, red, chain)
    queue_cap(J, p, g, cps[1], cp2, e_node, e_spg, e_teb)
    pair = ht_pair_bwd(sv.h3, sv.h2, dd, dG_all[2], dG_all[1], dims) if chain and pair_bwd_on() else None
    if pair is not None:
        dd, hp3, hp2 = pair
    else:
        dd, hp3 = hypertem_core_bwd(sv.h3, dd, dG_all[2], dims, chain, True)
        dd, hp2 = hypertem_core_bwd(sv.h2, dd, dG_all[1], dims, chain, True)
    queue_ht(J, p, g, hts[2], hp3, *e_te)
    queue_ht(J, p, g, hts[1], hp2, *e_te)
    dd, cp1 = cap_core_bwd(p, g, cps[0], sv.c1, dd, dims, HS, HT, red, chain)
    queue_cap(J, p, g, cps[0], cp1, e_node, e_spg, e_teb)
    if isinstance(sv.h1, EncIn):
        assert chain
        e = sv.h1
        w, bi = p["encoder.dim_in_flow.weight"], p["encoder.dim_in_flow.bias"]
        if nsG == B:
            dWb, _, dinp = ops.encin_ht1_bwd(dd.view(B, T, N, C), e.source, e.mask, e.fill, w, bi, e.Wbt, e.ab, e.wv, dG=dG_all[0])
        else:
            dWb, dGb, dinp = ops.encin_ht1_bwd(dd.view(B, T, N, C), e.source, e.mask, e.fill, w, bi, e.Wbt, e.ab, e.wv)
            torch.sum(dGb, 0, out=dG_all[0][0])
        hp1 = _wb_parts(dWb, C)
        wb = _wb_view(g["encoder.dim_in_flow.weight"], g["encoder.dim_in_flow.bias"])
        if wb is not None:
            red.jobs.bwd_pool(_ones(dd.device, dinp.shape[0]), dinp, wb)
        else:
            g["encoder.dim_in_flow.weight"].add_(dinp[:, :C].sum(0).view(C, 1))
            g["encoder.dim_in_flow.bias"].add_(dinp[:, C:].sum(0))
        red.keep.append((dinp, dWb))
        dd = None
    elif defer_h1:
        assert chain and premul_in
        ns = ops.wgrad_nsplit(MODE_TIME, B * T, N, C)
        dWb = torch.empty(ns * B * T, C * C + C, device=dd.device, dtype=torch.float32)
        hp1 = _wb_parts(dWb, C, ns)
        dd = PendingH1(sv.h1, dd, dG_all[0], dWb)
    else:
        dd, hp1 = hypertem_core_bwd(sv.h1, dd, dG_all[0], dims, chain, premul_in)
    queue_ht(J, p, g, hts[0], hp1, *e_te)
    red.gram(A_all.view(4 * N, Hm, T), dG_all, dA_all.view(4 * N, Hm, T), N, nsG)
    for i, h in enumerate(hts):
        red.late.bwd_pool(ne, dA_all[i], g[h + "adj"].view(d, Hm * T))
        red.late.bwd_emb(dA_all[i], p[h + "adj"].view(d, Hm * T), dne)
    red.timefeat(p, g, pfx + "time_feature1.", tidx, d_te)
    red.timefeat(p, g, pfx + "time_feature1_.", tidx, d_teb)
    red.timefeat(p, g, pfx + "time_feature2.", tidx, d_tes, spg=True)
    red.keep.append((sv, hp1, hp2, hp3, hp4, cp1, cp2, dout))
    return dd


class EncIn:

    def __init__(self, source, mask, fill, Wbt, ab, wv):
        self.source, self.mask, self.fill, self.Wbt, self.ab, self.wv = source, mask, fill, Wbt, ab, wv


ENCIN = os.environ.get("GPTST_ENCIN", "1") == "1"


def encin_ok(dims, base):
    return ENCIN and base == 1 and dims[3] in (64, 128) and dims[1] == 12 and chain_ok(dims)


GUIDEIN = os.environ.get("GPTST_GUIDEIN", "1") == "1"
GUIDE_HEAD = os.environ.get("GPTST_GUIDE_HEAD", "1") == "1"


class LowRankIn(NamedTuple):
    Wspa: Any


class GuideSaved(NamedTuple):
    t4m: Any
    spa: Any
    tem: Any
    h2: Any
    label: Any


def guide_fwd(p, source, tidx, dims, base, gen=None, lowrank_in=False):
    B, T, N, C = dims
    if gen is None:
        gen = gen_all(p, tidx, dims, which=(), guide=True).guide
    t4m, Wspa, bspa, Wtem, btem = gen
    m = "encoder.MLP_RL."
    if lowrank_in and GUIDEIN and GUIDE_HEAD and base == 1 and C == 64:
        r = ops.guide_head_fwd(source, p[m + "ln1.weight"], p[m + "ln1.bias"], Wspa, bspa, Wtem, btem, p[m + "ln3.weight"], p[m + "ln3.bias"])
        if r is not None:
            h1, h2, prob, label = r
            return prob, GuideSaved(t4m, LowRankIn(Wspa), CondLinSaved(h1, h2, Wtem), h2, label)
    if lowrank_in and GUIDEIN and base == 1 and C in (64, 128):
        h1 = ops.guide_in_fwd(source, p[m + "ln1.weight"], p[m + "ln1.bias"], Wspa, bspa)
        s1 = LowRankIn(Wspa)
    else:
        h0 = ops.lin_in(source, base + 2, base, p[m + "ln1.weight"], p[m + "ln1.bias"], C)
        h1, s1 = condlin_fwd(h0, Wspa, bspa, MODE_NODE, dims)
    h2, s2 = condlin_fwd(h1, Wtem, btem, MODE_TIME, dims)
    prob, label = ops.rowdot(h2, p[m + "ln3.weight"], p[m + "ln3.bias"], softmax=True, want_label=True)
    return prob, GuideSaved(t4m, s1, s2, h2, label)


# ... 114 lines not shown
            ts = [dh2, h1, Wtem, dh1, dW, db]
        else:
            dh1, _ = self.out.tem
            dWb, dinp = torch.empty(N, C * C + C, **f), torch.empty(N, 2 * C, **f)
            self.out.inp = (dWb, dinp)
            ts = [dh1, self.source, p[m + "ln1.weight"], p[m + "ln1.bias"], sv_g.spa.Wspa, dWb, dinp]
        self.stage = st
        return (st, ts, 0, ops.kl_guest_blocks(st, B, T, N), HS, self.source.shape[-1], self.w)


def _in_proj_grads(source, base, dY, gW, gb, mask, fill, red):
    wb = _wb_view(gW, gb)
    if base == 1 and wb is not None:
        C = dY.shape[1]
        part = ops.rowouter_part(source, base + 2, base, dY, mask=mask, fill=fill)
        red.jobs.bwd_pool(_ones(dY.device, part.shape[0]), part[:, :2 * C], wb)
        red.keep.append(part)
    else:
        ops.rowouter(source, base + 2, base, dY, gW, 0, csum=gb, mask=mask, fill=fill)


class Forward(NamedTuple):
    emb: Any
    c1: Any
    dec: Any
    out: Any
    sv_e: Any
    sv_d: Any


def autoencoder_fwd(p, source, mask, dims, base, num_route, scaler_zeros, gen=None, tidx=None, lowrank_in=False, kl=None, head=True,
                    decoder=True, join=True):
    B, T, N, C = dims
    if tidx is None:
        tidx = source[:, :, 0, base:base + 2].contiguous()
    gen_e, gen_d = (gen.sthcn[ENC], gen.sthcn[DEC] if decoder else None) if gen is not None else (None, None)
    first = None
    if lowrank_in and gen_e is not None and encin_ok(dims, base):
        w, bi = p["encoder.dim_in_flow.weight"], p["encoder.dim_in_flow.bias"]
        G1, Wbt1, bbt1 = gen_e.ht(0)
        o1, ab, wv = ops.encin_ht1_fwd(source, base, mask, 0.0 if mask is None else scaler_zeros, w, bi, G1, Wbt1, bbt1)
        first = (o1.view(-1, C), EncIn(source, mask, 0.0 if mask is None else scaler_zeros, Wbt1, ab, wv))
        x0 = None
    else:
        x0 = ops.lin_in(source, base + 2, base, p["encoder.dim_in_flow.weight"], p["encoder.dim_in_flow.bias"], C,
                        mask=mask, fill=scaler_zeros)
    emb, c1, sv_e, dec_h1 = sthcn_fwd(p, ENC, tidx, x0, dims, num_route, gen=gen_e, head=first, next_gen=gen_d if join else None, kl=kl)
    if not decoder:
        return Forward(emb, c1, None, None, sv_e, None)
    dec, _, sv_d, _ = sthcn_fwd(p, DEC, tidx, emb, dims, num_route, gen=gen_d, head=dec_h1, kl=kl)
    out = ops.rowdot(dec, p["decoder.dim_flow_out.weight"], p["decoder.dim_flow_out.bias"]) if head else None
    return Forward(emb, c1, dec, out, sv_e, sv_d)


def model_bwd(p, g, source, mask, tidx, sv_e, sv_d, dec, d_out, d_dec, dims, base, scaler_zeros, red, dd=None, chain=False):
    B, T, N, C = dims
    if dd is None:
        dd = _linear_out_bwd(p, g, "decoder.dim_flow_out.", dec, d_out, C, chain, d_h=d_dec)
    defer = (chain and (red.on_bucket is None or PAIR_UNDER_DP) and not isinstance(sv_d.h1, EncIn)
             and ht_pair_ok(sv_d.h1, sv_e.h4, dims))
    late = defer and red.on_bucket is not None
    d_emb = sthcn_bwd(p, g, DEC, tidx, sv_d, dd, dims, red, chain, True, defer_h1=defer)
    if not late:
        red.flush_async(tidx)
    d_x0 = sthcn_bwd(p, g, ENC, tidx, sv_e, d_emb, dims, red, chain, False,
                     after_pending=(lambda: red.flush_async(tidx)) if late else None)
    red.flush_async(tidx)
    if d_x0 is not None:
        _in_proj_grads(source, base, d_x0, g["encoder.dim_in_flow.weight"], g["encoder.dim_in_flow.bias"], mask, scaler_zeros, red)


def encoder_bwd(p, g, source, tidx, sv_e, d_emb, dims, base, red):
    d_x0 = sthcn_bwd(p, g, ENC, tidx, sv_e, d_emb, dims, red, chain=False, premul_in=False)
    _in_proj_grads(source, base, d_x0, g["encoder.dim_in_flow.weight"], g["encoder.dim_in_flow.bias"], None, 0.0, red)


def step_bwd(p, g, source, mask, tidx, fw, prob, sv_g, dims, base, scaler_zeros, red, loss, stats, sws=None, with_kl=False, kl=None):
    B, T, N, C = dims
    sigma, mu, thresh = loss
    if sws is not None:
        chain = chain_ok(dims)
        done = kl.out if kl is not None else KlOut()
        _, dd = loss_tail(p, g, fw.dec, source, mask, base, sigma, mu, thresh, sws, red, chain=chain)
        model_bwd(p, g, source, mask, tidx, fw.sv_e, fw.sv_d, fw.dec, None, None, dims, base, scaler_zeros, red, dd=dd, chain=chain)
        if with_kl:
            dh2 = kl_head(p, g, sv_g, prob, fw.c1, N, 0.1, sws, red, chain=chain, carried=done.head)
            guide_bwd(p, g, source, tidx, sv_g, None, dims, base, red, dh2=dh2, chain=chain, carried=done)
    else:
        M = B * T * N
        ops.mae_fwd(fw.out, source, base + 2, mask, sigma, mu, thresh, M, base, stats)
        d_out = ops.mae_bwd(fw.out, source, base + 2, mask, sigma, mu, thresh, M, base, stats, normalize=False)
        model_bwd(p, g, source, mask, tidx, fw.sv_e, fw.sv_d, fw.dec, d_out, None, dims, base, scaler_zeros, red)
        if with_kl:
            dlogit = ops.kl(prob, fw.c1, N, 0.1, stats)
            guide_bwd(p, g, source, tidx, sv_g, dlogit, dims, base, red)


def module_bwd(p, g, source, mask, tidx, fw, prob, sv_g, dims, base, scaler_zeros, red, d_out, d_dec=None, d_prob=None, chain=False):
    model_bwd(p, g, source, mask, tidx, fw.sv_e, fw.sv_d, fw.dec, d_out, d_dec, dims, base, scaler_zeros, red, chain=chain)
    if d_prob is not None:
        dlogit = (prob * (d_prob - (d_prob * prob).sum(-1, keepdim=True))).contiguous()
        guide_bwd(p, g, source, tidx, sv_g, dlogit, dims, base, red, chain=chain)


def warm_up(fn):
    s = torch.cuda.Stream()
    s.wait_stream(torch.cuda.current_stream())
    with torch.cuda.stream(s):
        for _ in range(2):
            fn()
    torch.cuda.current_stream().wait_stream(s)
    torch.cuda.synchronize()


_GC_LOCK, _GC_HELD = threading.Lock(), [0, False]


@contextlib.contextmanager
def quiet_gc():
    with _GC_LOCK:
        if _GC_HELD[0] == 0:
            gc.collect()
            _GC_HELD[1] = gc.isenabled()
            gc.disable()
        _GC_HELD[0] += 1
    try:
        yield
    finally:
        with _GC_LOCK:
            _GC_HELD[0] -= 1
            if _GC_HELD[0] == 0 and _GC_HELD[1]:
                gc.enable()
```

gpt-st_amd/ops.py:

```python
import contextlib
import ctypes
import math
from typing import Any, NamedTuple

import torch

from . import _C

MODE_TIME, MODE_NODE, MODE_SHARED = 0, 1, 2
PRO_NONE, PRO_DPRE = 0, 1
EPI_PLAIN, EPI_RES_LRELU, EPI_ADD_DPRE, EPI_LRELU, EPI_ADD_PREMUL, EPI_PREMUL = 0, 1, 2, 3, 4, 5

_p = _C.ptr


TIMER = None
LAST_CALL = {}


CALL_LOCK = None


def _call(name, *args, tag="", nbytes=0):
    if CALL_LOCK is not None:
        with CALL_LOCK:
            _C.lib().call(name, *args, _C.stream())
        return
    if TIMER is None:
        _C.lib().call(name, *args, _C.stream())
        return
    e0, e1 = torch.cuda.Event(enable_timing=True), torch.cuda.Event(enable_timing=True)
    e0.record()
    _C.lib().call(name, *args, _C.stream())
    e1.record()
    TIMER.append((name, tag, e0, e1, nbytes))
    LAST_CALL[(name, tag)] = args


def _nb(*ts):
    return sum(t.numel() * t.element_size() for t in ts if t is not None)


def _chk(*ts):
    for t in ts:
        if t is not None:
            assert t.is_cuda and t.dtype == torch.float32 and t.is_contiguous(), (t.device, t.dtype, t.is_contiguous())


def poolgen(emb, pool, pool2=None):
    _chk(emb, pool, pool2)
    R, K = emb.shape
    cols = pool.numel() // K
    out = torch.empty((R,) + tuple(pool.shape[1:]), device=emb.device, dtype=torch.float32)
    out2, cols2 = None, 0
    if pool2 is not None:
        cols2 = pool2.numel() // K
        out2 = torch.empty((R,) + tuple(pool2.shape[1:]), device=emb.device, dtype=torch.float32)
    _call("gptst_poolgen_fwd", _p(emb), _p(pool), _p(out), cols, _p(pool2), _p(out2), cols2, R, K, nbytes=_nb(emb, pool, out, pool2, out2))
    return (out, out2) if pool2 is not None else out


def poolgen_bwd_pool(emb, dW, dpool, dW2=None, dpool2=None, nsplit=1):
    _chk(emb, dW, dpool, dW2, dpool2)
    R, K = emb.shape
    cols = dpool.numel() // K
    cols2 = dpool2.numel() // K if dpool2 is not None else 0
    _call("gptst_poolgen_bwd_pool", _p(emb), _p(dW), _p(dpool), cols, _p(dW2), _p(dpool2), cols2, R, nsplit, K,
          nbytes=_nb(emb, dW, dpool, dW2, dpool2))


def poolgen_bwd_emb(dW, pool, demb, dW2=None, pool2=None, nsplit=1):
    _chk(dW, pool, demb, dW2, pool2)
    R, K = demb.shape
    cols = pool.numel() // K
    cols2 = pool2.numel() // K if pool2 is not None else 0
    _call("gptst_poolgen_bwd_emb", _p(dW), _p(pool), cols, _p(dW2), _p(pool2), cols2, _p(demb), R, nsplit, K,
          nbytes=_nb(dW, pool, dW2, pool2, demb))


def _ptrs(ts):
    return (ctypes.c_void_p * len(ts))(*[t.data_ptr() for t in ts])


def _ints(vs):
    return (ctypes.c_int * len(vs))(*[int(v) for v in vs])


def poolgen_multi(emb, pools, outs=None):
    _chk(emb, *pools)
    R, K = emb.shape
    if outs is None:
        outs = [torch.empty((R,) + tuple(pl.shape[1:]), device=emb.device, dtype=torch.float32) for pl in pools]
    cols = [pl.numel() // K for pl in pools]
    _call("gptst_poolgen_fwd_multi", _p(emb), len(pools), _ptrs(pools), _ptrs(outs), _ints(cols), R, K, nbytes=_nb(emb, *pools, *outs))
    return outs


def poolgen_bwd_pool_multi(emb, dWs, dpools, nsplits=None):
    _chk(emb, *dWs, *dpools)
    R, K = emb.shape
    cols = [dp.numel() // K for dp in dpools]
    ns = nsplits if nsplits is not None else [1] * len(dWs)
    _call("gptst_poolgen_bwd_pool_multi", _p(emb), len(dWs), _ptrs(dWs), _ptrs(dpools), _ints(cols), _ints(ns), R, K,
          nbytes=_nb(emb, *dWs, *dpools))


def poolgen_bwd_emb_multi(dWs, pools, demb, nsplits=None):
    _chk(demb, *dWs, *pools)
    R, K = demb.shape
    cols = [pl.numel() // K for pl in pools]
    ns = nsplits if nsplits is not None else [1] * len(dWs)
    _call("gptst_poolgen_bwd_emb_multi", len(dWs), _ptrs(dWs), _ptrs(pools), _ints(cols), _ints(ns), _p(demb), R, K,
          nbytes=_nb(demb, *dWs, *pools))


class PoolJob(NamedTuple):
    kind: int
    emb: Any
    dW: Any
    pool: Any
    out: Any
    R: int
    K: int
    cols: int
    nsplit: int
    ldx: int


class PoolJobs:
    FWD, BWD_POOL, BWD_EMB, GRAM = 0, 1, 2, 3

    def __init__(self):
        self.jobs = []
        self.post = []

    def fwd(self, emb, pool, out=None):
        _chk(emb, pool, out)
        R, K = emb.shape
        if out is None:
            out = torch.empty((R,) + tuple(pool.shape[1:]), device=emb.device, dtype=torch.float32)
        self.jobs.append(PoolJob(self.FWD, emb, None, pool, out, R, K, pool.numel() // K, 1, 0))
        return out

    def gram(self, emb, pool, out, A=None):
        _chk(emb, pool, out, A)
        R, K = emb.shape
        cols = pool.numel() // K
        assert cols % 12 == 0 and out.numel() == R * 144 and out.is_contiguous()
        if _C.lib().value("gptst_pool_jobs_gram_rows", K, cols) <= 0:
            assert A is not None and A.numel() == R * cols, "gram job does not fit and no forward output was given"
            self.post.append((A, out, R, cols // 12))
            return out
        self.jobs.append(PoolJob(self.GRAM, emb, None, pool, out, R, K, cols, 1, 0))
        return out

    @staticmethod
    def _ldx(dW, cols):
        assert dW.is_cuda and dW.dtype == torch.float32 and dW.dim() == 2 and dW.shape[1] == cols and dW.stride(1) == 1, (dW.shape, dW.stride(), cols)
        return dW.stride(0)

    def bwd_pool(self, emb, dW, dpool, nsplit=1):
        _chk(emb, dpool)
        R, K = emb.shape
        cols = dpool.numel() // K
        self.jobs.append(PoolJob(self.BWD_POOL, emb, dW, None, dpool, R, K, cols, nsplit, self._ldx(dW, cols)))

    def bwd_emb(self, dW, pool, demb, nsplit=1):
        _chk(pool, demb)
        R, K = demb.shape
        cols = pool.numel() // K
        self.jobs.append(PoolJob(self.BWD_EMB, None, dW, pool, demb, R, K, cols, nsplit, self._ldx(dW, cols)))

    @staticmethod
    def columns(js, fields=PoolJob._fields):
        return [len(js)] + [(_ptrs0 if f in ("emb", "dW", "pool", "out") else _ints)([getattr(j, f) for j in js])
                            for f in PoolJob._fields if f in fields]

    def launch(self):
        js, self.jobs = self.jobs, []
        post, self.post = self.post, []
        if js:
            _call("gptst_pool_jobs", *self.columns(js), nbytes=_nb(*[t for j in js for t in (j.emb, j.dW, j.pool, j.out)]))
        for A, G, rows, Hm in post:
            _call("gptst_gram_fwd", _p(A), _p(G), rows, Hm)


def _ptrs0(ts):
    return (ctypes.c_void_p * len(ts))(*[(t.data_ptr() if t is not None else None) for t in ts])


def apply(A, W, mode, BT, N, bias=None, resid=None, A2=None, transw=False, pro=PRO_NONE, epi=EPI_PLAIN, colsum=None,
          out=None, resid2=None):
    _chk(A, W, bias, resid, A2, resid2)
    C = A.shape[-1]
    if out is None:
        out = torch.empty_like(A)
    cs, ns = None, 0
    if colsum is not None:
        G = BT if mode == MODE_TIME else (N if mode == MODE_NODE else 1)
        ns = _C.lib().value("gptst_apply_nsplit", mode, BT, N, C)
        cs = torch.empty(ns * G, C, device=A.device, dtype=torch.float32)
    _call("gptst_apply", _p(A), _p(A2), _p(W), int(W.dim() == 3), int(transw), _p(bias), _p(resid), _p(resid2), _p(out), _p(cs),
          mode, pro, epi, BT, N, C, tag="mode%d pro%d epi%d" % (mode, pro, epi), nbytes=_nb(A, A2, W, bias, resid, resid2, out))
    if colsum is True:
        return out, cs, ns
    if colsum is not None:
        colsum.add_(cs.view(ns, -1, C).sum(0).view_as(colsum))
    return out


def apply_wgrad(dOut, Y, S, W, mode, BT, N, premul=False):
    _chk(dOut, Y, S, W)
    C = dOut.shape[-1]
    G = BT if mode == MODE_TIME else N
    ns = _C.lib().value("gptst_apply_wgrad_nsplit", mode, BT, N)
    dS = torch.empty_like(dOut)
    dW = torch.empty(ns * G, C * C, device=dOut.device, dtype=torch.float32)
    db = torch.empty(ns * G, C, device=dOut.device, dtype=torch.float32)
    _call("gptst_apply_wgrad", _p(dOut), _p(Y), _p(S), _p(W), _p(dS), _p(dW), _p(db), int(premul), mode, BT, N, C, tag="mode%d" % mode,
          nbytes=_nb(dOut, Y, S, W, dS, dW))
    return dS, dW, db, ns


def linear_bwd(dY, X, Wp, dOut, out, premul=False):
    _chk(dY, X, Wp, dOut, out)
    rows, C = dY.shape
    ns = _C.lib().value("gptst_linear_bwd_nsplit", rows)
    dX = torch.empty_like(dY)
    dWp = torch.empty(ns, C * C, device=dY.device, dtype=torch.float32)
    dbp = torch.empty(ns, C, device=dY.device, dtype=torch.float32)
    _call("gptst_linear_bwd", _p(dY), _p(X), _p(Wp), _p(dOut), _p(out), _p(dX), _p(dWp), _p(dbp), int(premul), rows, C,
          nbytes=_nb(dY, X, dOut, out, dX, dWp))
    return dX, dWp, dbp, ns


def wgrad_nsplit(mode, BT, N, C=64):
    return _C.lib().value("gptst_wgrad_nsplit", mode, BT, N, C)


def wgrad(A, D, mode, BT, N, D2=None, pro=PRO_NONE, colsum_a=False, colsum_d=False):
    _chk(A, D, D2)
    C = A.shape[-1]
    ns = wgrad_nsplit(mode, BT, N, C)
    G = BT if mode == MODE_TIME else (N if mode == MODE_NODE else 1)
    if colsum_a or colsum_d:
        dW = torch.empty(ns * G, C * C + C, device=A.device, dtype=torch.float32)
        _call("gptst_wgrad_colsum", _p(A), _p(D), _p(D2), _p(dW), mode, pro, 1 if colsum_a else 2, BT, N, C,
              tag="mode%d pro%d cs" % (mode, pro), nbytes=_nb(A, D, D2, dW))
    else:
        dW = torch.empty(ns * G, C, C, device=A.device, dtype=torch.float32)
        _call("gptst_wgrad", _p(A), _p(D), _p(D2), _p(dW), mode, pro, BT, N, C, tag="mode%d pro%d" % (mode, pro), nbytes=_nb(A, D, D2, dW))
    return dW, ns


def gram_fwd(A):
    N, Hm, T = A.shape
    G = torch.empty(N, T, T, device=A.device, dtype=torch.float32)
    _call("gptst_gram_fwd", _p(A), _p(G), N, Hm)
    return G


def gram_bwd(A, dG, out=None, layers=1, nsplit=1):
    LN, Hm, T = A.shape
    dA = out if out is not None else torch.empty_like(A)
    _call("gptst_gram_bwd", _p(A), _p(dG), _p(dA), layers, LN // layers, Hm, nsplit)
    return dA


def tmix(X, G, dOut=None, Y=None):
    _chk(X, G, dOut, Y)
    B, T, N, C = X.shape
    out = torch.empty_like(X)
    _call("gptst_tmix", _p(X), _p(G), _p(dOut), _p(Y), _p(out), B, T, N, C, tag="bwd" if dOut is not None else "fwd",
          nbytes=_nb(X, G, dOut, Y, out))
    return out


def hypertem_fwd(X, G, Wbt, bbt, want_R=True):
    _chk(X, G, Wbt, bbt)
    B, T, N, C = X.shape
    R = torch.empty_like(X) if want_R else None
    out = torch.empty_like(X)
    _call("gptst_hypertem_fwd", _p(X), _p(G), _p(Wbt), _p(bbt), _p(R), _p(out), B, T, N, C, nbytes=_nb(X, G, Wbt, bbt, R, out))
    return R, out


def hypertem_chain_fwd(X, stages, want_R=True, guest=None):
    B, T, N, C = X.shape
    _chk(X, *[t for st in stages for t in st])
    f = lambda: torch.empty(B, T, N, C, device=X.device, dtype=torch.float32)
    Rs = [f() if want_R else None for _ in stages]
    outs = [f() for _ in stages]
    chain = (_p(X), len(stages), _ptrs0([st[0] for st in stages]), _ptrs0([st[1] for st in stages]), _ptrs0([st[2] for st in stages]),
             _ptrs0(Rs), _ptrs0(outs), B, T, N, C)
    if guest is None:
        _call("gptst_hypertem_chain_fwd", *chain, tag="x%d" % len(stages), nbytes=_nb(X, *Rs, *outs))
    else:
        stage, ts, v0, v1, HS, lda, w = guest
        _chk(*ts)
        _call("gptst_hypertem_chain_fwd_kl", *chain, stage, _ptrs0(ts), v0, v1, HS, lda, float(w), tag="x%d+kl%d" % (len(stages), stage),
              nbytes=_nb(X, *Rs, *outs))
    return list(zip(Rs, outs))


def kl_guest_blocks(stage, B, T, N):
    return _C.lib().value("gptst_kl_guest_blocks", stage, B, T, N)


def encin_ht1_fwd(source, base, mask, fill, w, bi, G, Wbt, bbt):
    B, T, N, F = source.shape
    C = Wbt.shape[-1]
    assert base == 1
    _chk(source, mask, w, bi, G, Wbt, bbt)
    f = dict(device=source.device, dtype=torch.float32)
    out, ab, wv = torch.empty(B, T, N, C, **f), torch.empty(B * T * N, 2, **f), torch.empty(B * T, 2 * C, **f)
    _call("gptst_encin_ht1_fwd", _p(source), F, _p(mask), float(fill), _p(w), _p(bi), _p(G), _p(Wbt), _p(bbt), _p(out), _p(ab), _p(wv), B, T, N, C,
          nbytes=_nb(Wbt, out))
    return out, ab, wv


def encin_ht1_bwd(dPre, source, mask, fill, w, bi, Wbt, ab, wv, dG=None):
    B, T, N, F = source.shape
    C = Wbt.shape[-1]
    _chk(dPre, source, mask, w, bi, Wbt, ab, wv, dG)
    f = dict(device=source.device, dtype=torch.float32)
    dWb, dinp = torch.empty(B * T, C * C + C, **f), torch.empty(B * T, 2 * C, **f)
    if dG is None:
        dG = torch.empty(B, N, T, T, **f)
    _call("gptst_encin_ht1_bwd", _p(dPre), _p(source), F, _p(mask), float(fill), _p(w), _p(bi), _p(Wbt), _p(ab), _p(wv), _p(dWb), _p(dG), _p(dinp),
          B, T, N, C, nbytes=_nb(dPre, Wbt, dWb, dG))
    return dWb, dG, dinp


def guide_in_fwd(source, w1, b1, Wn, bn):
    B, T, N, F = source.shape
    C = Wn.shape[-1]
    _chk(source, w1, b1, Wn, bn)
    h1 = torch.empty(B * T * N, C, device=source.device, dtype=torch.float32)
    _call("gptst_guide_in_fwd", _p(source), F, _p(w1), _p(b1), _p(Wn), _p(bn), _p(h1), B * T, N, C, nbytes=_nb(Wn, h1))
    return h1


def guide_head_fwd(source, w1, b1, Wn, bn, Wbt, bbt, W3, b3):
    B, T, N, F = source.shape
    C, J = Wn.shape[-1], W3.shape[0]
    if C != 64 or J > 16:
        return None
    _chk(source, w1, b1, Wn, bn, Wbt, bbt, W3, b3)
    dev = source.device
    f = dict(device=dev, dtype=torch.float32)
    uc = torch.empty(N, 2 * C, **f)
    h1, h2 = torch.empty(B * T * N, C, **f), torch.empty(B * T * N, C, **f)
    prob = torch.empty(B * T * N, J, **f)
    label = torch.empty(B * T * N, device=dev, dtype=torch.int32)
    _call("gptst_guide_head_fwd", _p(source), F, _p(w1), _p(b1), _p(Wn), _p(bn), _p(Wbt), _p(bbt), _p(W3), _p(b3), _p(uc), _p(h1), _p(h2), _p(prob),
          _p(label), B * T, N, C, J, nbytes=_nb(Wbt, h1, h2, prob))
    return h1, h2, prob, label


def guide_in_bwd(dPre, source, w1, b1, Wn):
    B, T, N, F = source.shape
    C = Wn.shape[-1]
    _chk(dPre, source, w1, b1, Wn)
    f = dict(device=source.device, dtype=torch.float32)
    dWb, dinp = torch.empty(N, C * C + C, **f), torch.empty(N, 2 * C, **f)
    _call("gptst_guide_in_bwd", _p(dPre), _p(source), F, _p(w1), _p(b1), _p(Wn), _p(dWb), _p(dinp), B * T, N, C, nbytes=_nb(dPre, Wn, dWb))
    return dWb, dinp


def hypertem_ntiles(N):
    return _C.lib().value("gptst_hypertem_ntiles", N)


def hypertem_bwd(dOut, Y, X, G, Wbt, dG=None, want_dbias=True, premul=False):
    _chk(dOut, Y, X, G, Wbt, dG)
    B, T, N, C = X.shape
    dX = torch.empty_like(X)
    nt = hypertem_ntiles(N)
    dbias = torch.empty(nt * B * T, C, device=X.device, dtype=torch.float32) if want_dbias else None
    if dG is None:
        dG = torch.empty(B, N, T, T, device=X.device, dtype=torch.float32)
    _call("gptst_hypertem_bwd", _p(dOut), _p(Y), _p(X), _p(G), _p(Wbt), _p(dX), _p(dbias), _p(dG), int(premul), B, T, N, C,
          nbytes=_nb(dOut, Y, X, G, Wbt, dX))
    return dX, dbias, dG


def hypertem_bwd_wgrad(dOut, Y, X, G, Wbt, R, dG=None, premul=False):
    _chk(dOut, Y, X, G, Wbt, R, dG)
    B, T, N, C = X.shape
    dX = torch.empty_like(X)
    if dG is None:
        dG = torch.empty(B, N, T, T, device=X.device, dtype=torch.float32)
    ns = wgrad_nsplit(MODE_TIME, B * T, N, C)
    dWb = torch.empty(ns * B * T, C * C + C, device=X.device, dtype=torch.float32)
    _call("gptst_hypertem_bwd_wgrad", _p(dOut), _p(Y), _p(X), _p(G), _p(Wbt), _p(R), _p(dX), _p(dG), _p(dWb), int(premul), B, T, N, C,
          nbytes=_nb(dOut, Y, X, G, Wbt, R, dX, dWb))
    return dX, dWb, ns, dG


def hypertem_bwd_pair(dOut1, X1, G1, Wbt1, R1, X0, G0, Wbt0, R0, dG1, dG0, cnt, dWb1=None):
    _chk(dOut1, X1, G1, Wbt1, R1, X0, G0, Wbt0, R0, dG1, dG0, cnt, dWb1)
    B, T, N, C = X1.shape
    if C != 64:
        return None
    dXmid, dX0 = torch.empty_like(X1), torch.empty_like(X0)
    ns = wgrad_nsplit(MODE_TIME, B * T, N, C)
    dWb0 = torch.empty(ns * B * T, C * C + C, device=X1.device, dtype=torch.float32)
    if dWb1 is None:
        dWb1 = torch.empty_like(dWb0)
    assert dWb1.shape == dWb0.shape
    try:
        _call("gptst_hypertem_bwd_pair", _p(dOut1), _p(X1), _p(G1), _p(Wbt1), _p(R1), _p(X0), _p(G0), _p(Wbt0), _p(R0), _p(dXmid), _p(dX0),
              _p(dG1), _p(dG0), _p(dWb1), _p(dWb0), _p(cnt), B, T, N, C, nbytes=_nb(dOut1, X1, R1, X0, R0, dXmid, dX0, dWb0, dWb1))
# ... 340 lines not shown
    label = torch.empty(rows, device=prob.device, dtype=torch.int32)
    counts = torch.empty(HS, device=prob.device, dtype=torch.int32)
    _call("gptst_mask_labels", _p(prob), rows, HS, _p(label), _p(counts))
    return label, counts


def mask_adaptive(label, counts, list_c, nums, noise_a, noise_r, ada_all, base, ws=None, u24=False, jobs=None):
    M, HS = label.numel(), list_c.numel()
    m_ada = torch.empty(M, device=label.device, dtype=torch.float32)
    m_rnd = torch.empty_like(m_ada)
    mask = torch.empty(M * base, device=label.device, dtype=torch.float32)
    fj = _fused_jobs(jobs, u24)
    if fj is not None:
        _call("gptst_mask_u24_fwd_jobs", 1, _p(label), _p(counts), _p(list_c), _p(nums), _p(noise_a), _p(noise_r), int(ada_all), M, HS, base, 0,
              _p(m_ada), _p(m_rnd), _p(mask), _p(ws if ws is not None else _mask_ws(label.device)), int(ws is not None), *fj[1])
        return m_ada, m_rnd, mask
    _call("gptst_mask_adaptive_u24" if u24 else "gptst_mask_adaptive", _p(label), _p(counts), _p(list_c), _p(nums), _p(noise_a), _p(noise_r),
          int(ada_all), M, HS, base, _p(m_ada), _p(m_rnd), _p(mask), _p(ws if ws is not None else _mask_ws(label.device)), int(ws is not None))
    return m_ada, m_rnd, mask


def lin_in(a, lda, J, W, b, C, mask=None, fill=0.0, wlayout=0, rows=None):
    rows = rows if rows is not None else a.numel() // lda
    Y = torch.empty(rows, C, device=a.device, dtype=torch.float32)
    _call("gptst_lin_in", _p(a), lda, _p(mask), float(fill), _p(W), wlayout, _p(b), _p(Y), rows, J, C, nbytes=_nb(a, mask, W, b, Y))
    return Y


def rowdot(X, W, b, softmax=False, want_label=False):
    rows, C = X.shape
    J = W.shape[0]
    Z = torch.empty(rows, J, device=X.device, dtype=torch.float32)
    label = torch.empty(rows, device=X.device, dtype=torch.int32) if want_label else None
    _call("gptst_rowdot", _p(X), _p(W), _p(b), _p(Z), rows, J, C, int(softmax), _p(label), nbytes=_nb(X, W, b, Z))
    return (Z, label) if want_label else Z


def rowouter(a, lda, J, X, out, olayout, csum=None, asum=None, mask=None, fill=0.0):
    rows, C = X.shape
    ws = torch.empty(_C.lib().value("gptst_rowouter_ws_floats", J, C), device=X.device, dtype=torch.float32)
    _call("gptst_rowouter", _p(a), lda, _p(mask), float(fill), _p(X), _p(out), olayout, _p(csum), _p(asum), _p(ws), rows, J, C,
          nbytes=_nb(a, mask, X, out))


def rowouter_part(a, lda, J, X, mask=None, fill=0.0, want_asum=False):
    rows, C = X.shape
    nparts = _C.lib().value("gptst_rowouter_nparts", rows)
    part = torch.empty(nparts, J * C + C + J, device=X.device, dtype=torch.float32)
    _call("gptst_rowouter_part", _p(a), lda, _p(mask), float(fill), _p(X), _p(part), int(want_asum), rows, J, C, nbytes=_nb(X))
    return part


def timefeat_fwd(params, tidx, rows, K):
    E = params[1].numel()
    out = torch.empty(rows, E, device=tidx.device, dtype=torch.float32)
    _call("gptst_timefeat_fwd", *[_p(t) for t in params], _p(tidx), _p(out), rows, K, E)
    return out


def timefeat_bwd(params, grads, tidx, dout, rows, K):
    E = params[1].numel()
    _call("gptst_timefeat_bwd", *[_p(t) for t in params], *[_p(t) for t in grads], _p(tidx), _p(dout), rows, K, E)


class TimefeatJob(NamedTuple):
    params: Any
    rows: int
    K: int
    grads: Any = None
    dout: Any = None

    @property
    def E(self):
        return self.params[1].numel()


def timefeat_jobs_fwd(jobs, tidx):
    outs = [torch.empty(j.rows, j.E, device=tidx.device, dtype=torch.float32) for j in jobs]
    _call("gptst_timefeat_jobs", len(jobs), 0, _ptrs([t for j in jobs for t in j.params]), None, _p(tidx), _ptrs(outs),
          _ints([j.rows for j in jobs]), _ints([j.K for j in jobs]), _ints([j.E for j in jobs]))
    return outs


def timefeat_jobs_bwd(jobs, tidx):
    if not jobs:
        return
    _call("gptst_timefeat_jobs", len(jobs), 1, _ptrs([t for j in jobs for t in j.params]), _ptrs([t for j in jobs for t in j.grads]), _p(tidx),
          _ptrs([j.dout for j in jobs]), _ints([j.rows for j in jobs]), _ints([j.K for j in jobs]), _ints([j.E for j in jobs]))


def mae_fwd(out, src, lda, mask, sigma, mu, thresh, rows, J, stats):
    _call("gptst_mae_fwd", _p(out), _p(src), lda, _p(mask), float(sigma), float(mu), float(thresh), rows, J, _p(stats))


def mae_bwd(out, src, lda, mask, sigma, mu, thresh, rows, J, stats, normalize=True):
    dOut = torch.empty_like(out)
    _call("gptst_mae_bwd", _p(out), _p(src), lda, _p(mask), float(sigma), float(mu), float(thresh), rows, J, _p(stats), int(normalize),
          _p(dOut))
    return dOut


def kl(prob, c, N, w, stats, want_grad=True):
    rows, HS = prob.shape
    dlogit = torch.empty_like(prob) if want_grad else None
    _call("gptst_kl", _p(prob), _p(c), rows, N, HS, float(w), _p(dlogit), _p(stats))
    return dlogit


TAIL_MAXJ = 16


def set_deterministic(on):
    _C.lib().call("gptst_set_deterministic", int(bool(on)))


@contextlib.contextmanager
def deterministic():
    keep = _C.lib().value("gptst_deterministic_state")
    set_deterministic(True)
    try:
        yield
    finally:
        set_deterministic(keep)


def tail_parts(rows):
    return _C.lib().value("gptst_tail_parts", rows)


def tail_sws(rows, device):
    return torch.zeros(_C.lib().value("gptst_tail_parts", rows), 4, device=device, dtype=torch.float32)


def tail_mae(dec, W, b, src, lda, mask, sigma, mu, thresh, sws, premul=False):
    rows, C = dec.shape
    J = W.shape[0]
    nparts = _C.lib().value("gptst_tail_parts", rows)
    out = torch.empty(rows, J, device=dec.device, dtype=torch.float32)
    d_dec = torch.empty_like(dec)
    part = torch.empty(nparts, J * C + J, device=dec.device, dtype=torch.float32)
    _call("gptst_tail_mae", _p(dec), _p(W), _p(b), _p(src), lda, _p(mask), float(sigma), float(mu), float(thresh), _p(out), _p(d_dec),
          _p(part), _p(sws), int(premul), rows, J, C, nbytes=_nb(dec, d_dec))
    return out, d_dec, part


def tail_kl(h2, W3, prob, c, N, w, sws, premul=False):
    rows, C = h2.shape
    HS = W3.shape[0]
    nparts = _C.lib().value("gptst_tail_parts", rows)
    d_h2 = torch.empty_like(h2)
    part = torch.empty(nparts, HS * C + HS, device=h2.device, dtype=torch.float32)
    _call("gptst_tail_kl", _p(h2), _p(W3), _p(prob), _p(c), float(w), _p(d_h2), _p(part), _p(sws), int(premul), rows, N, HS, C, nbytes=_nb(h2, d_h2))
    return d_h2, part


def stats_fold(sws, stats):
    _call("gptst_stats_fold", _p(sws), sws.shape[0], _p(stats))


_ADAM_WS = {}


def step_begin(z0, z1, src, base, noise=None, rng=None):
    B, T, N, lda = src.shape
    tidx = torch.empty(B, T, 2, device=src.device, dtype=torch.float32)
    _call("gptst_step_begin", _p(z0), z0.numel(), _p(z1), z1.numel() if z1 is not None else 0, _p(src), _p(tidx), B * T, N, lda, base,
          _p(noise), noise.numel() if noise is not None else 0, _p(rng))
    return tidx


class PinnedRing:
# ... 338 lines not shown
```

gpt-st_amd/step.py:

```python
import contextlib
import dataclasses
import itertools
import os
import random
from typing import Any, NamedTuple

import torch

from . import engine, ops

DEFER_GEN = os.environ.get("GPTST_DEFER_GEN", "1") == "1"
U24 = os.environ.get("GPTST_MASK_U24", "1") == "1"


class Part1(NamedTuple):
    tidx: Any
    gen: Any
    red: Any
    prob: Any
    sv_g: Any


@dataclasses.dataclass(eq=False)
class Enqueued:
# ... 41 lines not shown
        self.rng_words = self.hc[16 + self.HS + 2:]
        self.noise_seed = 1234567 + seed
        self._ring = ops.PinnedRing(self.hc.numel(), slots=self.RING)
        self.phase_kl = False
        self._gK, self._group_failed = 0, False
        self.stats_out = torch.zeros(8, device=self.dev)
        self.mask_buf = torch.ones(M * self.base, device=self.dev)
        self.last_mask = None
        self.force_mask = False
        self.tA = self.tB = 0
        self.lr = args.lr_init
        self.rng = random.Random(seed)
        self.graphs = {}
        self._g_graphs = {}
        self._graph_comm_failed = False
        self._ctx_keep = []
        self._sws = None
        self.inject_noise = False
        self.global_count_scale = False
        self.node_reduce = None
        self.join_enc_dec = True
        self.safe_mode = False
        self.lost_steps = 0
        self.lost_batches = 0
        self._ledger = []
        self._holder = {}
        self._ids = itertools.count()
        self.arena = engine.ZeroArena(self.dev)
        self.fused_tails = os.environ.get("GPTST_FUSED_TAILS", "1") == "1" and engine.fused_tails_ok(model.param_views(), self.C, self.base, self.HS)
        self.W = dp.world if dp is not None else 1
        self.gmask = bool(global_mask) and dp is not None and self.W > 1
        if self.gmask:
            Mg = M * self.W
            self.noise_g = torch.zeros(Mg * self.base, device=self.dev)
            self.noise_ar_g = torch.zeros(2 * Mg, device=self.dev)
            self.noise_a_g, self.noise_r_g = self.noise_ar_g[:Mg], self.noise_ar_g[Mg:]
            self.label_l = torch.zeros(M, dtype=torch.int32, device=self.dev)
            self.label_g = torch.zeros(Mg, dtype=torch.int32, device=self.dev)
        self.always_guide = os.environ.get("GPTST_ALWAYS_GUIDE", "0") == "1"
        self.dp_overlap = (os.environ.get("GPTST_DP_OVERLAP", "0") != "0" and dp is not None and getattr(dp, "capturable", False)
                           and (self.W > 1 or os.environ.get("GPTST_FORCE_DP", "0") == "1"))
        self.dec_lo, self.dec_hi = self._decoder_bucket(model)
        self.rank_weight = 1.0
        self.fork_side = torch.cuda.Stream() if self.dp_overlap else None

    def _needs_exchange(self, phase):
        return self.gmask and phase == 1 and not self.force_mask

    @staticmethod
    def _decoder_bucket(model):
        offs = [(o, model.state_dict()[k].numel()) for k, o in model._offs.items() if k.startswith("decoder.") and o < model.nA]
        lo = min(o for o, _ in offs)
        hi = max(o + (n + 3) // 4 * 4 for o, n in offs)
        assert hi == model.nA and all(o >= lo for o, _ in offs), (lo, hi, model.nA)
        assert not any(lo <= o < hi for k, o in model._offs.items() if not k.startswith("decoder.")), "decoder bucket is not contiguous"
        return lo, hi

    def _allreduce(self, sl):
        if self.rank_weight != 1.0:
            assert not self.use_graph, "a rank weight is baked into a captured graph: tail rounds use eager steppers"
            lost = self.stats[5:6].clone()
            sl.mul_(self.rank_weight)
            self.stats[5:6].copy_(lost)
        self.dp.allreduce_(sl)

    def _bucket_ready(self, k):
        if k == 0:
            self._allreduce(self.gbuf[self.dec_lo:self.dec_hi])
            self._dec_reduced = True

    def _dp_in_graph(self):
        return self.dp is not None and getattr(self.dp, "capturable", False) and not self._graph_comm_failed

    def _part1(self, phase):
        p, dims, base = self.model.param_views(), self.dims, self.base
        engine.CTX.ARENA, engine.CTX.NODE_REDUCE = self.arena, self.node_reduce
        src = self.src
        noise = None if self.inject_noise or self.force_mask else self._noise_buffer(phase)
        tidx = ops.step_begin(self.gbuf, self.arena.begin(zero=False), src, base, noise=noise, rng=self.rng_words)
        need_guide = self._need_guide(phase)
        gen = engine.gen_all(p, tidx, dims, guide=need_guide, defer=DEFER_GEN)
        red = engine.Reductions()
        red.no_carry = self.deterministic
        self._dec_reduced = False
        if self.dp_overlap and self._dp_in_graph():
            red.on_bucket = self._bucket_ready
            red.bucket_inline, red.fork_side = True, self.fork_side
        lowrank = self.fused_tails and engine.chain_ok(dims)
        prob, sv_g = engine.guide_fwd(p, src, tidx, dims, base, gen=gen.guide, lowrank_in=lowrank) if need_guide else (None, None)
        if self._needs_exchange(phase):
            self.label_l.copy_(sv_g.label)
        return Part1(tidx, gen, red, prob, sv_g)

    def _part2(self, phase, ctx):
        if not self.safe_mode:
            return self._part2_impl(phase, ctx)
        with engine.no_handoffs():
            return self._part2_impl(phase, ctx)

    def _part2_impl(self, phase, ctx):
        mdl, p, g, dims, base = self.model, self.model.param_views(), self.g, self.dims, self.base
        a = self.args
        src, tidx, gen, red, prob, sv_g = self.src, ctx.tidx, ctx.gen, ctx.red, ctx.prob, ctx.sv_g
        engine.CTX.ARENA, engine.CTX.NODE_REDUCE = self.arena, self.node_reduce
        pend = gen.pending
        mask = self._make_mask(phase, prob, sv_g.label if sv_g is not None else None, pend)
        if pend is not None:
            pend.launch()
        self.last_mask = mask
        fused = self.fused_tails
        kl, sws = None, None
        if phase == 1 and self._carry_kl(sv_g):
            sws = self._tail_sws()
            kl = engine.KlCarry(p, sv_g, prob, src, dims, 0.1, sws)
        fw = engine.autoencoder_fwd(p, src, mask, dims, base, mdl.num_route, mdl.scaler_zeros, gen=gen, tidx=tidx,
                                    lowrank_in=fused and engine.chain_ok(dims), kl=kl, head=not fused, join=self.join_enc_dec)
        if fused and sws is None:
            sws = self._tail_sws()
        engine.step_bwd(p, g, src, mask, tidx, fw, prob, sv_g, dims, base, mdl.scaler_zeros, red, (self.std, self.mean, a.mape_thresh),
                        self.stats, sws=sws, with_kl=phase == 1, kl=kl)
        self._fold_stats(sws)
        red.flush(tidx)
        engine.CTX.ARENA = engine.CTX.NODE_REDUCE = None
        self._after_backward(phase)

    def _noise_buffer(self, phase):
        if self.gmask:
            return self.noise_g if phase == 0 else self.noise_ar_g
        return self.noise if phase == 0 else self.noise_ar

    def _need_guide(self, phase):
        return phase == 1 or self.always_guide

    def _make_mask(self, phase, prob, label, pend):
        a = self.args
        if self.force_mask:
            return self.mask_buf
        noise = self._noise_buffer(phase)
        if phase == 0:
            mask = ops.mask_random(noise, int(noise.numel() * a.mask_ratio), ws=self._mask_ws(), u24=U24, jobs=pend)
        else:
            noise_a, noise_r = noise.chunk(2)
            mask = ops.mask_adaptive(self._mask_labels(label), None, self.ctrl[:self.HS], self.ctrl[self.HS:], noise_a, noise_r,
                                     a.ada_type == "all", self.base, ws=self._mask_ws(), u24=U24, jobs=pend)[2]
        return self._mask_cut(mask)

    def _mask_labels(self, label):
        return self.label_g if self.gmask else label

    def _mask_cut(self, mask):
        if not self.gmask:
            return mask
        self.last_mask_global = mask
        return self.dp.rows_of(mask, self.B * self.T * self.N * self.base)

    def _fold_stats(self, sws):
        if sws is None:
            return
        if self.dp is None:
            self._sws = sws
        else:
            ops.stats_fold(sws, self.stats)

    def _after_backward(self, phase):
        if self.dp is None:
            self._optim()
# ... 388 lines not shown
```

include/gptst_hip.h:

```cpp
#ifndef GPTST_HIP_H
#define GPTST_HIP_H
#include <stdint.h>

#ifdef __cplusplus
extern "C" {
#endif
#if defined(__GNUC__)
#pragma GCC visibility push(default)
#endif

#define GPTST_ABI_VERSION 23
int gptst_abi_version(void);
int gptst_set_deterministic(int on);
int gptst_deterministic_state(void);
int gptst_handoff_timeouts(int* out);
int gptst_handoff_reset(void);
int gptst_mask_cooperative(int on);
int gptst_mask_cooperative_state(void);
int gptst_set_handoff_guard(int on);

int gptst_poolgen_fwd(const float* emb, const float* pool, float* out, int cols, const float* pool2, float* out2,
                      int cols2, int R, int K, void* stream);
int gptst_poolgen_bwd_pool(const float* emb, const float* dW, float* dpool, int cols, const float* dW2, float* dpool2,
                           int cols2, int R, int nsplit, int K, void* stream);
int gptst_poolgen_bwd_emb(const float* dW, const float* pool, int cols, const float* dW2, const float* pool2, int cols2,
                          float* demb, int R, int nsplit, int K, void* stream);

int gptst_poolgen_fwd_multi(const float* emb, int nprob, const void* pools, const void* outs, const int* cols, int R, int K,
                            void* stream);
int gptst_poolgen_bwd_pool_multi(const float* emb, int nprob, const void* dWs, const void* dpools, const int* cols, const int* nsplit,
                                 int R, int K, void* stream);
int gptst_poolgen_bwd_emb_multi(int nprob, const void* dWs, const void* pools, const int* cols, const int* nsplit, float* demb, int R,
                                int K, void* stream);

int gptst_pool_jobs(int njobs, const int* kind, const void* const* emb, const void* const* x, const void* const* pool,
                    const void* const* out, const int* R, const int* K, const int* cols, const int* nsplit, const int* ldx, void* stream);
int gptst_pool_jobs_gram_rows(int K, int cols);

int gptst_apply_nsplit(int mode, int BT, int N, int C);
int gptst_apply(const float* A, const float* A2, const float* W, int w_per_group, int transw, const float* bias,
                const float* resid, const float* resid2, float* out, float* colsum, int mode, int pro, int epi, int BT,
                int N, int C, void* stream);
int gptst_wgrad_nsplit(int mode, int BT, int N, int C);
int gptst_wgrad(const float* A, const float* D, const float* D2, float* dW, int mode, int pro, int BT, int N, int C,
                void* stream);
int gptst_wgrad_colsum(const float* A, const float* D, const float* D2, float* dW, int mode, int pro, int which, int BT, int N, int C,
                       void* stream);

int gptst_apply_wgrad_nsplit(int mode, int BT, int N);
int gptst_apply_wgrad(const float* dOut, const float* Y, const float* S, const float* W, float* dS, float* dW, float* colsum, int premul,
                      int mode, int BT, int N, int C, void* stream);

int gptst_linear_bwd_nsplit(int rows);
int gptst_linear_bwd(const float* dY, const float* X, const float* Wp, const float* dOut, const float* out, float* dX, float* dWp, float* dbp,
                     int premul, int rows, int C, void* stream);

int gptst_gram_fwd(const float* A, float* G, int N, int Hm, void* stream);
int gptst_gram_bwd(const float* A, const float* dG, float* dA, int L, int N, int Hm, int nsplit, void* stream);
int gptst_tmix(const float* X, const float* G, const float* dOut, const float* Y, float* out, int B, int T, int N, int C,
               void* stream);
int gptst_tmix_dgraph(const float* dR, const float* X, float* dG, int B, int T, int N, int C, void* stream);
int gptst_tmix_bwd(const float* dR, const float* X, const float* G, const float* dOut, const float* Y, float* dX, float* dG, int B, int T,
                   int N, int C, void* stream);
int gptst_tmix_bwd_chain(const float* dR, const float* X, const float* G, const float* dPre, int premul, float* dX, float* dG, int B, int T,
                         int N, int C, void* stream);

int gptst_hypertem_fwd(const float* X, const float* G, const float* Wbt, const float* bbt, float* R_out, float* out, int B, int T,
                       int N, int C, void* stream);
int gptst_hypertem_chain_fwd(const float* X, int nstage, const void* Gs, const void* Wbts, const void* bbts, const void* Rs, const void* outs,
                             int B, int T, int N, int C, void* stream);
int gptst_hypertem_chain_fwd_kl(const float* X, int nstage, const void* Gs, const void* Wbts, const void* bbts, const void* Rs, const void* outs,
                                int B, int T, int N, int C, int stage, const void* ops, int v0, int v1, int HS, int lda, float w, void* stream);
int gptst_kl_guest_blocks(int stage, int B, int T, int N);

int gptst_encin_ht1_fwd(const float* src, int lda, const float* mask, float fill, const float* w, const float* bi, const float* G,
                        const float* Wbt, const float* bbt, float* out, float* ab, float* wv, int B, int T, int N, int C, void* stream);
int gptst_encin_ht1_bwd(const float* dPre, const float* src, int lda, const float* mask, float fill, const float* w, const float* bi,
                        const float* Wbt, const float* ab, const float* wv, float* dWb, float* dG, float* dinp, int B, int T, int N, int C,
                        void* stream);

int gptst_guide_in_fwd(const float* src, int lda, const float* w1, const float* b1, const float* Wn, const float* bn, float* h1, int BT, int N,
                       int C, void* stream);
int gptst_guide_in_bwd(const float* dPre, const float* src, int lda, const float* w1, const float* b1, const float* Wn, float* dWb, float* dinp,
                       int BT, int N, int C, void* stream);
int gptst_guide_uc_floats(int N, int C);
int gptst_guide_head_fwd(const float* src, int lda, const float* w1, const float* b1, const float* Wn, const float* bn, const float* Wbt,
                         const float* bbt, const float* W3, const float* b3, float* uc, float* h1, float* h2, float* prob, int* label,
                         int BT, int N, int C, int J, void* stream);

int gptst_hypertem_ntiles(int N);
int gptst_hypertem_bwd(const float* dOut, const float* Y, const float* X, const float* G, const float* Wbt, float* dX, float* dbias,
                       float* dG, int premul, int B, int T, int N, int C, void* stream);
int gptst_hypertem_bwd_wgrad(const float* dOut, const float* Y, const float* X, const float* G, const float* Wbt, const float* R, float* dX,
                             float* dG, float* dWb, int premul, int B, int T, int N, int C, void* stream);
int gptst_hypertem_bwd_pair(const float* dOut1, const float* X1, const float* G1, const float* Wbt1, const float* R1, const float* X0,
                            const float* G0, const float* Wbt0, const float* R0, float* dXmid, float* dX0, float* dG1, float* dG0,
                            float* dWb1, float* dWb0, void* cnt, int B, int T, int N, int C, void* stream);

int gptst_cap_route_fwd(const float* X, const float* Wp, const float* bp, const float* dadj, float* c_out, float* s_out, int BT, int N,
                        int C, int HS, int R, void* stream);
int gptst_cap_cross_fwd(const float* s, const float* dyn, const float* tmpl, float* v, float* Ht, float* Rt, int B, int T, int C,
                        int HS, int HT, void* stream);
int gptst_cap_cross_ws_floats(int B, int T, int C, int HS, int HT);
int gptst_cap_cross_bwd(const float* dv, const float* s, const float* Rt, const float* Ht, const float* dyn, const float* tmpl,
                        float* dS, float* ddyn, float* ws, int B, int T, int C, int HS, int HT, void* stream);
int gptst_cap_rec_fwd(const float* c, const float* v, float* rec, int BT, int N, int C, int HS, void* stream);
int gptst_cap_cross_rec_fwd(const float* s, const float* dyn, const float* tmpl, const float* c, float* v, float* Ht, float* Rt, float* rec,
                            int B, int T, int N, int C, int HS, int HT, void* stream);
int gptst_cap_rec_bwd(const float* drec, const float* c, const float* v, float* dc1, float* dv, int BT, int N, int C, int HS,
                      void* stream);
int gptst_cap_route_bwd(const float* X, const float* Wp, const float* bp, const float* c, const float* dc1, const float* dS,
                        float* dY, float* dlogit, int BT, int N, int C, int HS, void* stream);
int gptst_cap_cross_route_bwd(const float* X, const float* Wp, const float* bp, const float* c, const float* dc1, const float* dv,
                              const float* s, const float* Rt, const float* Ht, const float* dyn, const float* tmpl, float* dY,
                              float* dlogit, float* ddyn, float* dS_ws, void* flags, int B, int T, int N, int C, int HS, int HT, void* stream);
int gptst_cap_cross_route_lin_bwd(const float* X, const float* Wp, const float* bp, const float* c, const float* dc1, const float* dv,
                                  const float* s, const float* Rt, const float* Ht, const float* dyn, const float* tmpl,
                                  const float* dPre, const float* out, int premul, float* dX, float* dWp, float* dbp, float* dlogit,
                                  float* ddyn, float* dS_ws, void* flags, int B, int T, int N, int C, int HS, int HT, void* stream);
int gptst_cap_route_roles_ok(int B, int T, int N, int C, int HS, int HT);
int gptst_cap_cross_route_lin_bwd_jobs(const float* X, const float* Wp, const float* bp, const float* c, const float* dc1, const float* dv,
                                       const float* s, const float* Rt, const float* Ht, const float* dyn, const float* tmpl,
                                       const float* dPre, const float* out, int premul, float* dX, float* dWp, float* dbp, float* dlogit,
                                       float* ddyn, float* dS_ws, void* flags, int B, int T, int N, int C, int HS, int HT,
                                       int njobs, const int* jkind, const void* const* jemb, const void* const* jx, const void* const* jpool,
                                       const void* const* jout, const int* jR, const int* jK, const int* jcols, const int* jnsplit, const int* jldx,
                                       void* stream);
int gptst_cap_split_units(int BT, int N, int C, int HS);
int gptst_cap_cross_route_lin_bwd_split(const float* X, const float* Wp, const float* bp, const float* c, const float* dc1, const float* dv,
                                        const float* s, const float* Rt, const float* Ht, const float* dyn, const float* tmpl,
                                        const float* dPre, const float* out, int premul, float* dX, float* dWp, float* dbp, float* dlogit,
                                        float* ddyn, float* dS_ws, void* flags, int B, int T, int N, int C, int HS, int HT, int nsplit,
                                        int njobs, const int* jkind, const void* const* jemb, const void* const* jx, const void* const* jpool,
                                        const void* const* jout, const int* jR, const int* jK, const int* jcols, const int* jnsplit, const int* jldx,
                                        void* stream);

int gptst_cap_fits_lds(int N, int C, int HS);
int gptst_capbig_squash_rows(float* Y, long rows, int C, void* stream);
int gptst_capbig_softmax(const float* bl, const float* l0, float* cs, int BT, int HS, int N, int use_bl, int use_l0, void* stream);
int gptst_capbig_type1(const float* cs, const float* P, float* S, int BT, int HS, int N, int C, void* stream);
int gptst_capbig_post(const float* S, const float* V0, float* out, long rows, int C, int post, void* stream);
int gptst_capbig_type2(const float* V, const float* P, float* bl, int BT, int HS, int N, int C, void* stream);
int gptst_capbig_rec_fwd(const float* c, const float* v, float* rec, int BT, int HS, int N, int C, void* stream);
int gptst_capbig_rec_bwd_dc(const float* drec, const float* v, float* dc1, int BT, int HS, int N, int C, void* stream);
int gptst_capbig_route_bwd_rows(const float* Y, const float* c, const float* dc1, const float* dS, float* dY, float* dlogit, int BT,
                                int HS, int N, int C, void* stream);

int gptst_capflow_supported(int HS, int C);
int gptst_capflow_nparts(int N);
int gptst_capflow_squash(const float* Y, const float* dadj, float* P, float* part, int BT, int HS, int N, int C, void* stream);
int gptst_capflow_route(const float* rows, const float* V, const float* bl_in, float* bl_out, const float* l0, const float* c_in,
                        float* c_out, float* part, int BT, int HS, int N, int C, void* stream);
int gptst_capflow_post(const float* part, int nparts, int prow, float* V0, float* Vout, int mode, int BT, int HS, int C, void* stream);
int gptst_capflow_rec_fwd(const float* c, const float* v, float* rec, int BT, int HS, int N, int C, void* stream);
int gptst_capflow_route_bwd(const float* Y, const float* c, const float* dc1, const float* dS, float* dY, float* dlogit, int BT,
                            int HS, int N, int C, void* stream);

int gptst_metrics_accum(const float* out, const float* src, int lda, const float* vis, float sigma, float mu, int has_mae_thresh,
                        float mae_thresh, float mape_thresh, int B, int T, int N, int D, double* sums_t, double* sums_tn, void* stream);

int gptst_mask_ws_bytes(void);
int gptst_mask_random(const float* noise, int M, int k, float* mask, void* ws, int ws_zeroed, void* stream);
// ... 24 lines not shown
                             int rows, int C, void* stream);
int gptst_stgcn_tapgemm(const float* X, int ldx, int ci, int ntap, int dt0, int dt1, int dt2, int dt3, const float* W, const float* bias,
                        const float* R, int ldr, int res_w, float* Y, int co, float* S, float* A, int act, int rows, int T, int N,
                        void* stream);
int gptst_stgcn_gate_bwd(const float* dOut, const float* out, const float* S, const float* A, float* dPre, int act, int rows, int co,
                         void* stream);
int gptst_stgcn_wgrad_nsplit(int rows, int cw, int Ktot);
int gptst_stgcn_wgrad(const float* D, int cw, const float* X, int ldx, int ci, int ntap, int dt0, int dt1, int dt2, int dt3, float* part,
                      float* bpart, int nsplit, int rows, int T, int N, void* stream);
int gptst_stgcn_nodemix(const float* L, int Np, int ks, const float* In, float* Out, const float* R, int c, int reduce, int units, int N,
                        void* stream);
int gptst_stgcn_ln_fwd(const float* X, const float* gamma, const float* beta, float* Y, float* mean, float* rstd, int units, int M,
                       float eps, void* stream);
int gptst_stgcn_ln_bwd(const float* dY, const float* X, const float* gamma, const float* mean, const float* rstd, float* dX, int units,
                       int M, void* stream);
int gptst_stgcn_ln_nsplit(int units);
int gptst_stgcn_ln_bwd_param(const float* dY, const float* X, const float* mean, const float* rstd, float* pg, float* pb, int nsplit,
                             int units, int M, void* stream);
int gptst_tgcn_lds_bytes(int N, int Hp, int B);
int gptst_tgcn_fwd_gates(const float* L, int Np, const float* W0h, const float* h, const float* Gx0, float* u, float* r, float* q,
                         float* z, int ldz, int zoff, int B, int T, int N, int Hp, int t, int tiles, void* stream);
int gptst_tgcn_fwd_state(const float* L, int Np, const float* W1h, const float* q, const float* Gx1, const float* u, const float* h,
                         float* h_out, float* c, float* z, int ldz, int zoff, int B, int T, int N, int Hp, int t, int tiles,
                         void* stream);
int gptst_tgcn_bwd_cand(const float* LT, int Np, const float* W1hT, const float* dh, const float* u, const float* c, const float* r,
                        const float* h, float* dpre1, float* dpre0, float* dh_part, int B, int T, int N, int Hp, int t, int tiles,
                        void* stream);
int gptst_tgcn_bwd_state(const float* LT, int Np, const float* W0hT, const float* dpre0, const float* dh_part, float* dh_out, int B,
                         int T, int N, int Hp, int t, int tiles, void* stream);
int gptst_mtgnn_tapgemm(const float* X, int ldx, int ci, const float* XM, int ntap, const int* offs, const float* W, const float* bias,
                        const float* R, int ldr, int Tr, int roff, const float* OM, float* Y, int co, float* Tn, float* S, int gated,
                        int B, int Tsrc, int Tdst, int N, void* stream);
int gptst_mtgnn_gate_bwd(const float* dG, const float* Tn, const float* S, const float* OM, float* dPre, int rows, int co, void* stream);
int gptst_mtgnn_wgrad(const float* D, int cw, const float* X, int ldx, int ci, const float* XM, int ntap, const int* offs, float* part,
                      float* bpart, int nsplit, int B, int Tsrc, int Tdst, int N, void* stream);
int gptst_mtgnn_graphgrad_nsplit(int units, int N, int ks);
int gptst_mtgnn_graphgrad(const float* D, int ldd, int dcol0, const float* X, int ldx, int c, int ks, float* part, int nsplit, int units,
                          int N, void* stream);
int gptst_astgcn_attmix(const float* Tp, int Np, int ks, const float* S, const float* In, float* Out, const float* R, int c, int reduce,
                        int B, int T, int N, void* stream);
int gptst_astgcn_attgrad(const float* Tp, int Np, int ks, const float* X, const float* G, float* dS, int c, int B, int T, int N,
                         void* stream);
int gptst_astgcn_rowln_fwd(const float* X, const float* gamma, const float* beta, float* Y, float* mean, float* rstd, long rows, int c,
                           float eps, void* stream);
int gptst_astgcn_rowln_bwd(const float* dY, const float* X, const float* gamma, const float* mean, const float* rstd, float* dX, long rows,
                           int c, void* stream);
int gptst_astgcn_rowln_nsplit(long rows);
int gptst_astgcn_rowln_bwd_param(const float* dY, const float* X, const float* mean, const float* rstd, float* pg, float* pb, int nsplit,
                                 long rows, int c, void* stream);
int gptst_stsgcn_mix(const float* L, int Np, const float* In, float* Out, int c, int mode, int B, int T, int N, void* stream);
int gptst_stsgcn_wingemm(const float* X, int ci, const float* Wt, const float* bias, int shared, float* Y, int co, float* S, float* A, int act,
                         float* best, int* which, int opj, int B, int W, int R, int N, void* stream);
int gptst_stsgcn_gate_bwd(const float* up, const float* dBest, const int* which, int opj, const float* S, const float* A, float* dPre, int B,
                          int W, int R, int N, int co, void* stream);
int gptst_stsgcn_winwgrad_nsplit(int wrows, int cw, int ci, int W);
int gptst_stsgcn_winwgrad(const float* D, int cw, const float* X, int ci, float* part, float* bpart, int nsplit, int B, int W, int R,
                          void* stream);
int gptst_stfgnn_mix(const float* S, const float* D, int Np, const float* In, float* Out, int c, int mode, int B, int T, int N, void* stream);

int gptst_rowouter_ws_floats(int J, int C);
int gptst_rowouter_nparts(int rows);
int gptst_rowouter_part(const float* a, int lda, const float* mask, float fill, const float* X, float* part, int want_asum, int rows,
                        int J, int C, void* stream);
int gptst_rowouter(const float* a, int lda, const float* mask, float fill, const float* X, float* out, int olayout, float* csum,
                   float* asum, float* ws, int rows, int J, int C, void* stream);

int gptst_timefeat_fwd(const float* wd, const float* bd, const float* ww, const float* bw, const float* w1, const float* b1,
                       const float* w2, const float* b2, const float* w3, const float* b3, const float* tidx, float* out, int rows,
                       int K, int E, void* stream);
int gptst_timefeat_bwd(const float* wd, const float* bd, const float* ww, const float* bw, const float* w1, const float* b1,
                       const float* w2, const float* b2, const float* w3, const float* b3, float* gwd, float* gbd, float* gww,
                       float* gbw, float* gw1, float* gb1, float* gw2, float* gb2, float* gw3, float* gb3, const float* tidx,
                       const float* dout, int rows, int K, int E, void* stream);

int gptst_tail_parts(int rows);
int gptst_tail_mae(const float* dec, const float* W, const float* b, const float* src, int lda, const float* mask, float sigma, float mu,
                   float thresh, float* out, float* d_dec, float* part, float* sws, int premul, int rows, int J, int C, void* stream);
int gptst_tail_kl(const float* h2, const float* W3, const float* prob, const float* c, float w, float* d_h2, float* part, float* sws,
                  int premul, int rows, int N, int HS, int C, void* stream);
int gptst_stats_fold(const float* sws, int rows, float* stats, void* stream);

int gptst_timefeat_jobs(int njobs, int bwd, const void* const* params, const void* const* grads, const float* tidx,
                        const void* const* io, const int* rows, const int* K, const int* E, void* stream);

int gptst_step_begin(float* z0, long n0, float* z1, long n1, const float* src, float* tidx, int BT, int N, int lda, int base,
                     float* noise, long n_noise, const int* rng, void* stream);

int gptst_mae_fwd(const float* out, const float* src, int lda, const float* mask, float sigma, float mu, float thresh, int rows,
                  int J, float* stats, void* stream);
int gptst_mae_bwd(const float* out, const float* src, int lda, const float* mask, float sigma, float mu, float thresh, int rows,
                  int J, const float* stats, int normalize, float* dOut, void* stream);
int gptst_kl(const float* prob, const float* c, int rows, int N, int HS, float w, float* dlogit, float* stats, void* stream);
int gptst_clip_adam_ws_floats(void);
int gptst_clip_adam(float* p, const float* g, float* m, float* v, long nA, long nB, const float* hyper, float* stats, float* ws,
                    float* stats_out, const float* sws, int sws_rows, void* stream);

int gptst_layer_bytes(int kind, int B, int T, int N, int C, int d, int Hm, int ds, int HS, int HT, int base, long* saved_bytes,
                      long* scratch_bytes);
int gptst_hypertem_layer_fwd(const float* x, const float* node_emb, const float* time_eb, const float* adj, const float* wpool,
                             const float* bpool, float* out, void* saved, long saved_bytes, int B, int T, int N, int C, int d, int Hm,
                             void* stream);
int gptst_hypertem_layer_bwd(const float* dout, const float* x, const float* out, const float* node_emb, const float* time_eb,
                             const float* adj, const float* wpool, const float* bpool, const void* saved, long saved_bytes, float* dx,
                             float* d_node_emb, float* d_time_eb, float* d_adj, float* d_wpool, float* d_bpool, void* scratch,
                             long scratch_bytes, int B, int T, int N, int C, int d, int Hm, void* stream);
int gptst_cap_layer_fwd(const float* x, const float* node_emb_spg, const float* time_eb_spg, const float* teb, const float* ln_p_w,
                        const float* ln_p_b, const float* adj, const float* t_adj, const float* wspa, const float* bspa,
                        const float* mask_template, float* out, float* c_out, float* dyn_out, void* saved, long saved_bytes, int B, int T,
                        int N, int C, int d, int ds, int HS, int HT, int R, void* stream);
int gptst_cap_layer_bwd(const float* dout, const float* x, const float* out, const float* c, const float* dyn, const float* node_emb_spg,
                        const float* time_eb_spg, const float* teb, const float* ln_p_w, const float* ln_p_b, const float* adj,
                        const float* t_adj, const float* wspa, const float* bspa, const float* mask_template, const void* saved,
                        long saved_bytes, float* dx, float* d_node_emb_spg, float* d_time_eb_spg, float* d_teb, float* d_ln_p_w,
                        float* d_ln_p_b, float* d_adj, float* d_t_adj, float* d_wspa, float* d_bspa, void* scratch, long scratch_bytes, int B,
                        int T, int N, int C, int d, int ds, int HS, int HT, void* stream);
int gptst_mlprl_layer_fwd(const float* a, int lda, const float* time_eb, const float* node_emb, const float* ln1_w, const float* ln1_b,
                          const float* wpool_spa, const float* bpool_spa, const float* wpool_tem, const float* bpool_tem, const float* ln3_w,
                          const float* ln3_b, float* logits, void* saved, long saved_bytes, int B, int T, int N, int C, int d, int base,
                          int HS, void* stream);
int gptst_mlprl_layer_bwd(const float* dlogits, const float* a, int lda, const float* time_eb, const float* node_emb, const float* ln1_w,
                          const float* wpool_spa, const float* bpool_spa, const float* wpool_tem, const float* bpool_tem, const float* ln3_w,
                          const void* saved, long saved_bytes, float* d_time_eb, float* d_node_emb, float* d_ln1_w, float* d_ln1_b,
                          float* d_wpool_spa, float* d_bpool_spa, float* d_wpool_tem, float* d_bpool_tem, float* d_ln3_w, float* d_ln3_b,
                          void* scratch, long scratch_bytes, int B, int T, int N, int C, int d, int base, int HS, void* stream);

int gptst_comm_available(void);
int gptst_comm_unique_id(void* out128);
int gptst_comm_init(int rank, int world, const void* unique_id, void** comm_out);
int gptst_allreduce_f32(void* comm, float* buf, long n, void* stream);
int gptst_allgather_i32(void* comm, const int* send, int* recv, long n, void* stream);
int gptst_comm_count(void* comm, int* out);
int gptst_comm_destroy(void* comm);

#if defined(__GNUC__)
#pragma GCC visibility pop
#endif
#ifdef __cplusplus
}
#endif
#endif
```

Measured before the change: 923.1 steps/s.

## Piggyback pending pool/emb reduction jobs onto encin, gram and timefeat backward launches

Result: faster. 936.7 steps/s (median of 6 runs) (+1.5%).

```diff
diff --git a/gpt-st_amd/csrc/encin.hip b/gpt-st_amd/csrc/encin.hip
--- a/gpt-st_amd/csrc/encin.hip
+++ b/gpt-st_amd/csrc/encin.hip
@@ -1,4 +1,5 @@
 #include "common.h"
+#include "poolgen_dev.h"
 
 #define EI_T 12
 GPTST_STAMP_TABLES(encin)
@@ -78,18 +79,17 @@
 }
 
 template <int C>
-__global__ __launch_bounds__(256) void encin_bwd_kernel(const float* __restrict__ dPre, const float* __restrict__ src, int lda,
-                                                        const float* __restrict__ mask, float fill, const float* __restrict__ w,
-                                                        const float* __restrict__ bi, const float* __restrict__ Wbt, const float* __restrict__ ab,
-                                                        const float* __restrict__ wv, float* __restrict__ dWb, float* __restrict__ dG,
-                                                        float* __restrict__ dinp, int N, int B) {
+__device__ __forceinline__ void encin_bwd_body(const float* __restrict__ dPre, const float* __restrict__ src, int lda,
+                                               const float* __restrict__ mask, float fill, const float* __restrict__ w,
+                                               const float* __restrict__ bi, const float* __restrict__ Wbt, const float* __restrict__ ab,
+                                               const float* __restrict__ wv, float* __restrict__ dWb, float* __restrict__ dG,
+                                               float* __restrict__ dinp, int N, int bt, float* __restrict__ smem) {
     constexpr int LPR = C / 4, RPP = 256 / LPR, U = 4;
-    extern __shared__ __attribute__((aligned(16))) float smem[];
     float* red = smem;
     float* vec = red + RPP * 4 * C;
     float* as_ = vec + 6 * C;
     float* cs_ = as_ + N;
-    const int bt = blockIdx.x, b = bt / EI_T, t = bt % EI_T, tid = threadIdx.x;
+    const int b = bt / EI_T, t = bt % EI_T, tid = threadIdx.x;
     GPTST_WG_BEGIN(); GPTST_STAMP(0);
     if (tid < 2 * C) vec[4 * C + tid] = wv[(size_t)bt * 2 * C + tid];
     __syncthreads();
@@ -169,6 +169,30 @@
         for (int k = 0; k < EI_T / 4; ++k) st4(o + 4 * k, make_float4(v[4 * k], v[4 * k + 1], v[4 * k + 2], v[4 * k + 3]));
     }
     GPTST_STAMP(4); GPTST_WG_END();
+}
+
+static size_t encin_bwd_smem(int C, int N) { return ((size_t)(256 / (C / 4)) * 4 * C + 6 * C + 2 * (size_t)N) * sizeof(float); }
+
+struct EncinBwdArgs {
+    const float *dPre, *src, *mask, *w, *bi, *Wbt, *ab, *wv;
+    float *dWb, *dG, *dinp;
+    int lda, N;
+    float fill;
+};
+
+template <int C>
+__global__ __launch_bounds__(256) void encin_bwd_kernel(EncinBwdArgs a) {
+    extern __shared__ __attribute__((aligned(16))) float smem[];
+    encin_bwd_body<C>(a.dPre, a.src, a.lda, a.mask, a.fill, a.w, a.bi, a.Wbt, a.ab, a.wv, a.dWb, a.dG, a.dinp, a.N, blockIdx.x, smem);
+}
+
+template <int C>
+__global__ __launch_bounds__(256, PJ_OCC) void encin_bwd_jobs_kernel(EncinBwdArgs a, int nhost, PJCarry jc) {
+    extern __shared__ __attribute__((aligned(16))) float smem[];
+    if ((int)blockIdx.x < nhost)
+        encin_bwd_body<C>(a.dPre, a.src, a.lda, a.mask, a.fill, a.w, a.bi, a.Wbt, a.ab, a.wv, a.dWb, a.dG, a.dinp, a.N, blockIdx.x, smem);
+    else
+        pj_reduce_block(jc, (int)blockIdx.x - nhost, reinterpret_cast<float (*)[PG_MAXK][65]>(smem), threadIdx.x);
 }
 
 extern "C" int gptst_encin_ht1_fwd(const float* src, int lda, const float* mask, float fill, const float* w, const float* bi, const float* G,
@@ -183,15 +207,49 @@
     return GPTST_OK;
 }
 
+static int encin_bwd_check(const float* dPre, const float* src, int lda, const float* w, const float* bi, const float* Wbt, const float* ab,
+                           const float* wv, float* dWb, float* dG, float* dinp, int B, int T, int N, int C) {
+    if (!dPre || !src || !w || !bi || !Wbt || !ab || !wv || !dWb || !dG || !dinp || B <= 0 || N <= 0 || lda <= 0) return GPTST_EARG;
+    if (T != EI_T || (C != 64 && C != 128)) return GPTST_ESHAPE;
+    if (encin_bwd_smem(C, N) > 64 * 1024) return GPTST_ESHAPE;
+    return GPTST_OK;
+}
+
 extern "C" int gptst_encin_ht1_bwd(const float* dPre, const float* src, int lda, const float* mask, float fill, const float* w, const float* bi,
                                    const float* Wbt, const float* ab, const float* wv, float* dWb, float* dG, float* dinp, int B, int T, int N,
                                    int C, void* stream) {
-    if (!dPre || !src || !w || !bi || !Wbt || !ab || !wv || !dWb || !dG || !dinp || B <= 0 || N <= 0 || lda <= 0) return GPTST_EARG;
-    if (T != EI_T || (C != 64 && C != 128)) return GPTST_ESHAPE;
-    const size_t smem = ((size_t)(256 / (C / 4)) * 4 * C + 6 * C + 2 * (size_t)N) * sizeof(float);
-    if (smem > 64 * 1024) return GPTST_ESHAPE;
-    if (C == 64) hipLaunchKernelGGL((encin_bwd_kernel<64>), dim3(B * T), dim3(256), smem, (hipStream_t)stream, dPre, src, lda, mask, fill, w, bi, Wbt, ab, wv, dWb, dG, dinp, N, B);
-    else hipLaunchKernelGGL((encin_bwd_kernel<128>), dim3(B * T), dim3(256), smem, (hipStream_t)stream, dPre, src, lda, mask, fill, w, bi, Wbt, ab, wv, dWb, dG, dinp, N, B);
+    const int rc = encin_bwd_check(dPre, src, lda, w, bi, Wbt, ab, wv, dWb, dG, dinp, B, T, N, C);
+    if (rc) return rc;
+    const EncinBwdArgs a{dPre, src, mask, w, bi, Wbt, ab, wv, dWb, dG, dinp, lda, N, fill};
+    const size_t smem = encin_bwd_smem(C, N);
+    if (C == 64) hipLaunchKernelGGL((encin_bwd_kernel<64>), dim3(B * T), dim3(256), smem, (hipStream_t)stream, a);
+    else hipLaunchKernelGGL((encin_bwd_kernel<128>), dim3(B * T), dim3(256), smem, (hipStream_t)stream, a);
     GPTST_CHECK_LAUNCH();
     return GPTST_OK;
 }
+
+extern "C" int gptst_encin_ht1_bwd_jobs(const float* dPre, const float* src, int lda, const float* mask, float fill, const float* w, const float* bi,
+                                        const float* Wbt, const float* ab, const float* wv, float* dWb, float* dG, float* dinp, int B, int T, int N,
+                                        int C, int njobs, const int* jkind, const void* const* jemb, const void* const* jx, const void* const* jpool,
+                                        const void* const* jout, const int* jR, const int* jK, const int* jcols, const int* jnsplit, const int* jldx,
+                                        void* stream) {
+    int rc = encin_bwd_check(dPre, src, lda, w, bi, Wbt, ab, wv, dWb, dG, dinp, B, T, N, C);
+    if (rc) return rc;
+    const PJCols cols{njobs, jkind, jemb, jx, jpool, jout, jR, jK, jcols, jnsplit, jldx};
+    PJCarry jc;
+    int taken = 0;
+    if (C == 64) {
+        taken = gptst_pj_carry_take(&jc, &cols);
+        if (taken < 0) return taken;
+    } else if (njobs < 0) return GPTST_EARG;
+    if (taken == 0) {
+        rc = gptst_encin_ht1_bwd(dPre, src, lda, mask, fill, w, bi, Wbt, ab, wv, dWb, dG, dinp, B, T, N, C, stream);
+    } else {
+        const EncinBwdArgs a{dPre, src, mask, w, bi, Wbt, ab, wv, dWb, dG, dinp, lda, N, fill};
+        const size_t fold = (size_t)4 * PG_MAXK * 65 * sizeof(float), own = encin_bwd_smem(C, N);
+        hipLaunchKernelGGL((encin_bwd_jobs_kernel<64>), dim3(B * T + jc.npb + jc.neb), dim3(256), own > fold ? own : fold, (hipStream_t)stream, a, B * T, jc);
+        GPTST_CHECK_LAUNCH();
+    }
+    if (rc) return rc;
+    return gptst_pj_carry_rest(&cols, taken, stream);
+}
diff --git a/gpt-st_amd/csrc/poolgen.hip b/gpt-st_amd/csrc/poolgen.hip
--- a/gpt-st_amd/csrc/poolgen.hip
+++ b/gpt-st_amd/csrc/poolgen.hip
@@ -6,9 +6,6 @@
 #define PG_ROWS 16
 
 
-#ifndef PJ_OCC
-#define PJ_OCC 6
-#endif
 
 #define PG_MAXROWS 64
 template <int V>
@@ -178,6 +175,66 @@
     return GPTST_OK;
 }
 
+static std::vector<int> pj_order(int njobs, const int* kind, const int* R, const int* cols, const int* nsplit) {
+    std::vector<int> ord(njobs);
+    std::vector<long> cost(njobs);
+    for (int p = 0; p < njobs; ++p) {
+        ord[p] = p;
+        const long rr = (long)R[p] * nsplit[p], cc = cols[p];
+        cost[p] = kind[p] == PJ_BWD_POOL ? rr * (cc < 64 ? cc : 64) : kind[p] == PJ_BWD_EMB ? 16L * nsplit[p] * (cc < 1024 ? cc : 1024)
+                : kind[p] == PJ_FWD ? 64L * (cc < 256 ? cc : 256) : 1L;
+    }
+    if (g_pg_sort) std::stable_sort(ord.begin(), ord.end(), [&](int a, int b) { return cost[a] > cost[b]; });
+    return ord;
+}
+
+struct PJGathered {
+    std::vector<int> kind, R, K, cols, nsplit, ldx;
+    std::vector<const void*> emb, x, pool, out;
+    PJGathered(const PJCols& j, const std::vector<int>& ord, int first, int last) {
+        for (int o = first; o < last; ++o) {
+            const int p = ord[o];
+            kind.push_back(j.kind[p]); R.push_back(j.R[p]); K.push_back(j.K[p]); cols.push_back(j.cols[p]); nsplit.push_back(j.nsplit[p]);
+            ldx.push_back(j.ldx ? j.ldx[p] : 0);
+            emb.push_back(j.emb[p]); x.push_back(j.x[p]); pool.push_back(j.pool[p]); out.push_back(j.out[p]);
+        }
+    }
+};
+
+static bool pj_cols_ok(const PJCols* j) {
+    return j && j->njobs >= 0 && (j->njobs == 0 || (j->kind && j->emb && j->x && j->pool && j->out && j->R && j->K && j->cols && j->nsplit));
+}
+
+GPTST_INTERNAL int gptst_pj_carry_take(PJCarry* c, const PJCols* j) {
+    if (!c || !pj_cols_ok(j)) return GPTST_EARG;
+    c->t.n = c->npool = c->npb = c->neb = 0;
+    if (j->njobs == 0 || g_deterministic) return 0;
+    for (int p = 0; p < j->njobs; ++p) {
+        if (j->kind[p] < PJ_FWD || j->kind[p] > PJ_GRAM) return GPTST_EARG;
+        if (j->kind[p] != PJ_BWD_POOL && j->kind[p] != PJ_BWD_EMB) return 0;
+    }
+    const std::vector<int> ord = pj_order(j->njobs, j->kind, j->R, j->cols, j->nsplit);
+    const int take = j->njobs < PJ_MAX ? j->njobs : PJ_MAX;
+    const PJGathered g(*j, ord, 0, take);
+    const int rc = gptst_pj_reduce_table(&c->t, take, g.kind.data(), g.emb.data(), g.x.data(), g.pool.data(), g.out.data(), g.R.data(), g.K.data(),
+                                         g.cols.data(), g.nsplit.data(), g.ldx.data(), &c->npool, &c->npb, &c->neb);
+    if (rc == GPTST_ESHAPE) { c->t.n = c->npool = c->npb = c->neb = 0; return 0; }
+    return rc ? rc : take;
+}
+
+extern "C" int gptst_pool_jobs(int njobs, const int* kind, const void* const* emb, const void* const* x, const void* const* pool,
+                               const void* const* out, const int* R, const int* K, const int* cols, const int* nsplit, const int* ldx,
+                               void* stream);
+GPTST_INTERNAL int gptst_pj_carry_rest(const PJCols* j, int taken, void* stream) {
+    if (!pj_cols_ok(j) || taken < 0 || taken > j->njobs) return GPTST_EARG;
+    if (taken == j->njobs) return GPTST_OK;
+    if (taken == 0) return gptst_pool_jobs(j->njobs, j->kind, j->emb, j->x, j->pool, j->out, j->R, j->K, j->cols, j->nsplit, j->ldx, stream);
+    const std::vector<int> ord = pj_order(j->njobs, j->kind, j->R, j->cols, j->nsplit);
+    const PJGathered g(*j, ord, taken, j->njobs);
+    return gptst_pool_jobs(j->njobs - taken, g.kind.data(), g.emb.data(), g.x.data(), g.pool.data(), g.out.data(), g.R.data(), g.K.data(),
+                           g.cols.data(), g.nsplit.data(), g.ldx.data(), stream);
+}
+
 extern "C" int gptst_pool_jobs(int njobs, const int* kind, const void* const* emb, const void* const* x, const void* const* pool,
                                const void* const* out, const int* R, const int* K, const int* cols, const int* nsplit, const int* ldx,
                                void* stream) {
@@ -188,15 +245,7 @@
                     0, kind[p], 0, ldx ? ldx[p] : 0};
     };
     const bool det = g_deterministic != 0;
-    std::vector<int> ord(njobs);
-    std::vector<long> cost(njobs);
-    for (int p = 0; p < njobs; ++p) {
-        ord[p] = p;
-        const long rr = (long)R[p] * nsplit[p], cc = cols[p];
-        cost[p] = kind[p] == PJ_BWD_POOL ? rr * (cc < 64 ? cc : 64) : kind[p] == PJ_BWD_EMB ? 16L * nsplit[p] * (cc < 1024 ? cc : 1024)
-                : kind[p] == PJ_FWD ? 64L * (cc < 256 ? cc : 256) : 1L;
-    }
-    if (g_pg_sort) std::stable_sort(ord.begin(), ord.end(), [&](int a, int b) { return cost[a] > cost[b]; });
+    const std::vector<int> ord = pj_order(njobs, kind, R, cols, nsplit);
     PJobs t; t.n = 0;
     for (int o = 0; o < njobs; ++o) {
         const int p = ord[o];
diff --git a/gpt-st_amd/csrc/poolgen_dev.h b/gpt-st_amd/csrc/poolgen_dev.h
--- a/gpt-st_amd/csrc/poolgen_dev.h
+++ b/gpt-st_amd/csrc/poolgen_dev.h
@@ -85,6 +85,9 @@
     }
 }
 
+#ifndef PJ_OCC
+#define PJ_OCC 6
+#endif
 #ifndef PJ_UC
 #define PJ_UC 4
 #endif
@@ -219,3 +222,24 @@
         if (orow < a.R && i < a.K && (by * 4 + wave) * 256 < a.cols) atomicAdd(a.out + (size_t)orow * a.K + i, acc[r]);
     }
 }
+
+struct PJCarry { PJobs t; int npool, npb, neb; };
+__device__ __forceinline__ void pj_reduce_block(const PJCarry& c, int vb, float (*fold)[PG_MAXK][65], int tid) {
+    if (vb < c.npb) {
+        int p = 0;
+        for (int q = 1; q < c.npool; ++q) if (vb >= c.t.j[q].blk0) p = q;
+        const PJob& a = c.t.j[p];
+        if (((a.cols | a.ldx) & 3) == 0) pj_bwd_pool<4>(a, vb - a.blk0, fold, tid); else pj_bwd_pool<1>(a, vb - a.blk0, fold, tid);
+    } else if (vb < c.npb + c.neb) {
+        vb -= c.npb;
+        int p = c.npool;
+        for (int q = c.npool + 1; q < c.t.n; ++q) if (vb >= c.t.j[q].blk0) p = q;
+        const PJob& a = c.t.j[p];
+        const int rel = vb - a.blk0;
+        if (((a.cols | a.ldx) & 3) == 0) pj_bwd_emb<4>(a, rel % a.nbx, rel / a.nbx, tid); else pj_bwd_emb<1>(a, rel % a.nbx, rel / a.nbx, tid);
+    }
+}
+struct PJCols { int njobs; const int* kind; const void* const* emb; const void* const* x; const void* const* pool; const void* const* out;
+                const int *R, *K, *cols, *nsplit, *ldx; };
+GPTST_INTERNAL int gptst_pj_carry_take(PJCarry* c, const PJCols* j);
+GPTST_INTERNAL int gptst_pj_carry_rest(const PJCols* j, int taken, void* stream);
diff --git a/gpt-st_amd/csrc/timefeat.hip b/gpt-st_amd/csrc/timefeat.hip
--- a/gpt-st_amd/csrc/timefeat.hip
+++ b/gpt-st_amd/csrc/timefeat.hip
@@ -1,4 +1,5 @@
 #include "common.h"
+#include "poolgen_dev.h"
 
 struct TfParams {
     const float *wd, *bd, *ww, *bw, *w1, *b1, *w2, *b2, *w3, *b3;
@@ -143,7 +144,24 @@
 #undef TF_CASE
 }
 
-static int tf_launch(TfJobs& t, int bwd, hipStream_t st) {
+__global__ __launch_bounds__(256, 4) void timefeat_bwd_jobs_kernel(TfJobs t, int nhost, PJCarry jc) {
+    constexpr int FOLD = 4 * PG_MAXK * 65;
+    __shared__ __attribute__((aligned(16))) float sh[FOLD > TF_SH_FLOATS ? FOLD : TF_SH_FLOATS];
+    if ((int)blockIdx.x >= nhost) { pj_reduce_block(jc, (int)blockIdx.x - nhost, reinterpret_cast<float (*)[PG_MAXK][65]>(sh), threadIdx.x); return; }
+    int q = 0;
+    for (int i = 1; i < t.n; ++i) if ((int)blockIdx.x >= t.j[i].blk0) q = i;
+    const TfJob& a = t.j[q];
+    const int blk = blockIdx.x - a.blk0;
+    switch (a.E) {
+    case 2: tf_bwd_body<2, false, 256>(a.p, a.g, a.tidx, a.dout, a.rows, a.K, blk, sh); break;
+    case 4: tf_bwd_body<4, false, 256>(a.p, a.g, a.tidx, a.dout, a.rows, a.K, blk, sh); break;
+    case 8: tf_bwd_body<8, false, 256>(a.p, a.g, a.tidx, a.dout, a.rows, a.K, blk, sh); break;
+    case 16: tf_bwd_body<16, false, 256>(a.p, a.g, a.tidx, a.dout, a.rows, a.K, blk, sh); break;
+    default: break;
+    }
+}
+
+static int tf_launch(TfJobs& t, int bwd, hipStream_t st, const PJCarry* jc = nullptr) {
     int nb = 0;
     for (int q = 0; q < t.n; ++q) {
         TfJob& a = t.j[q];
@@ -153,7 +171,9 @@
         a.blk0 = nb;
         nb += (a.rows + rows_per - 1) / rows_per;
     }
-    if (bwd && g_deterministic) hipLaunchKernelGGL(timefeat_jobs_kernel<2>, dim3(t.n), dim3(TF_DET_T), 0, st, t);
+    if (jc && (!bwd || g_deterministic)) return GPTST_EARG;
+    if (jc) hipLaunchKernelGGL(timefeat_bwd_jobs_kernel, dim3(nb + jc->npb + jc->neb), dim3(256), 0, st, t, nb, *jc);
+    else if (bwd && g_deterministic) hipLaunchKernelGGL(timefeat_jobs_kernel<2>, dim3(t.n), dim3(TF_DET_T), 0, st, t);
     else if (bwd) hipLaunchKernelGGL(timefeat_jobs_kernel<1>, dim3(nb), dim3(256), 0, st, t);
     else hipLaunchKernelGGL(timefeat_jobs_kernel<0>, dim3(nb), dim3(256), 0, st, t);
     GPTST_CHECK_LAUNCH();
@@ -178,8 +198,8 @@
     return tf_launch(t, 1, (hipStream_t)stream);
 }
 
-extern "C" int gptst_timefeat_jobs(int njobs, int bwd, const void* const* params, const void* const* grads, const float* tidx,
-                                   const void* const* io, const int* rows, const int* K, const int* E, void* stream) {
+static int tf_jobs(int njobs, int bwd, const void* const* params, const void* const* grads, const float* tidx,
+                   const void* const* io, const int* rows, const int* K, const int* E, void* stream, const PJCarry* jc) {
     if (njobs <= 0 || njobs > TF_MAXJ || !params || !io || !rows || !K || !E || (bwd && !grads)) return GPTST_EARG;
     TfJobs t; t.n = njobs;
     for (int q = 0; q < njobs; ++q) {
@@ -189,5 +209,23 @@
         t.j[q] = TfJob{TfParams{pp[0], pp[1], pp[2], pp[3], pp[4], pp[5], pp[6], pp[7], pp[8], pp[9]}, g, tidx,
                        bwd ? nullptr : (float*)io[q], bwd ? (const float*)io[q] : nullptr, rows[q], K[q], E[q], 0};
     }
-    return tf_launch(t, bwd, (hipStream_t)stream);
-}
+    return tf_launch(t, bwd, (hipStream_t)stream, jc);
+}
+
+extern "C" int gptst_timefeat_jobs(int njobs, int bwd, const void* const* params, const void* const* grads, const float* tidx,
+                                   const void* const* io, const int* rows, const int* K, const int* E, void* stream) {
+    return tf_jobs(njobs, bwd, params, grads, tidx, io, rows, K, E, stream, nullptr);
+}
+
+extern "C" int gptst_timefeat_jobs_bwd_jobs(int njobs, const void* const* params, const void* const* grads, const float* tidx, const void* const* io,
+                                            const int* rows, const int* K, const int* E, int npj, const int* jkind, const void* const* jemb,
+                                            const void* const* jx, const void* const* jpool, const void* const* jout, const int* jR, const int* jK,
+                                            const int* jcols, const int* jnsplit, const int* jldx, void* stream) {
+    const PJCols cols{npj, jkind, jemb, jx, jpool, jout, jR, jK, jcols, jnsplit, jldx};
+    PJCarry jc;
+    const int taken = gptst_pj_carry_take(&jc, &cols);
+    if (taken < 0) return taken;
+    const int rc = tf_jobs(njobs, 1, params, grads, tidx, io, rows, K, E, stream, taken ? &jc : nullptr);
+    if (rc) return rc;
+    return gptst_pj_carry_rest(&cols, taken, stream);
+}
diff --git a/gpt-st_amd/csrc/tmix.hip b/gpt-st_amd/csrc/tmix.hip
--- a/gpt-st_amd/csrc/tmix.hip
+++ b/gpt-st_amd/csrc/tmix.hip
@@ -1,4 +1,5 @@
 #include "common.h"
+#include "poolgen_dev.h"
 
 #define TT 12
 #define TT2 144
@@ -13,10 +14,9 @@
     G[idx] = s;
 }
 
-__global__ __launch_bounds__(256) void gram_bwd_kernel(const float* __restrict__ A, const float* __restrict__ dG,
-                                                       float* __restrict__ dA, int N, int Hm, int nsplit) {
-    __shared__ float gs[TT2];
-    const int gn = blockIdx.x, l = gn / N, n = gn % N;
+__device__ __forceinline__ void gram_bwd_body(const float* __restrict__ A, const float* __restrict__ dG, float* __restrict__ dA, int N, int Hm,
+                                              int nsplit, int gn, float* __restrict__ gs) {
+    const int l = gn / N, n = gn % N;
     if (threadIdx.x < TT2) {
         const float* g = dG + ((size_t)l * nsplit * N + n) * TT2 + threadIdx.x;
         float part[8];
@@ -39,6 +39,19 @@
 #pragma unroll
     for (int u = 0; u < TT; ++u) s = fmaf(a[u], gs[t * TT + u] + gs[u * TT + t], s);
     dA[((size_t)gn * Hm + h) * TT + t] = s;
+}
+
+__global__ __launch_bounds__(256) void gram_bwd_kernel(const float* __restrict__ A, const float* __restrict__ dG,
+                                                       float* __restrict__ dA, int N, int Hm, int nsplit) {
+    __shared__ float gs[TT2];
+    gram_bwd_body(A, dG, dA, N, Hm, nsplit, blockIdx.x, gs);
+}
+
+__global__ __launch_bounds__(256, PJ_OCC) void gram_bwd_jobs_kernel(const float* __restrict__ A, const float* __restrict__ dG,
+                                                                    float* __restrict__ dA, int N, int Hm, int nsplit, int nhost, PJCarry jc) {
+    __shared__ __attribute__((aligned(16))) float fold[4][PG_MAXK][65];
+    if ((int)blockIdx.x < nhost) gram_bwd_body(A, dG, dA, N, Hm, nsplit, blockIdx.x, &fold[0][0][0]);
+    else pj_reduce_block(jc, (int)blockIdx.x - nhost, fold, threadIdx.x);
 }
 
 template <int C, bool ADD_DPRE>
@@ -230,6 +243,24 @@
     return GPTST_OK;
 }
 
+extern "C" int gptst_gram_bwd_jobs(const float* A, const float* dG, float* dA, int L, int N, int Hm, int nsplit, int njobs, const int* jkind,
+                                   const void* const* jemb, const void* const* jx, const void* const* jpool, const void* const* jout, const int* jR,
+                                   const int* jK, const int* jcols, const int* jnsplit, const int* jldx, void* stream) {
+    if (!A || !dG || !dA || L <= 0 || N <= 0 || nsplit <= 0 || Hm * TT > 256) return GPTST_EARG;
+    const PJCols cols{njobs, jkind, jemb, jx, jpool, jout, jR, jK, jcols, jnsplit, jldx};
+    PJCarry jc;
+    const int taken = gptst_pj_carry_take(&jc, &cols);
+    if (taken < 0) return taken;
+    if (taken == 0) {
+        const int rc = gptst_gram_bwd(A, dG, dA, L, N, Hm, nsplit, stream);
+        if (rc) return rc;
+    } else {
+        hipLaunchKernelGGL(gram_bwd_jobs_kernel, dim3(L * N + jc.npb + jc.neb), dim3(256), 0, (hipStream_t)stream, A, dG, dA, N, Hm, nsplit, L * N, jc);
+        GPTST_CHECK_LAUNCH();
+    }
+    return gptst_pj_carry_rest(&cols, taken, stream);
+}
+
 extern "C" int gptst_tmix_bwd_chain(const float* dR, const float* X, const float* G, const float* dPre, int premul, float* dX, float* dG,
                                     int B, int T, int N, int C, void* stream) {
     if (!dR || !X || !G || !dPre || !dX || !dG || T != TT || B < 1 || N < 1) return GPTST_EARG;
diff --git a/gpt-st_amd/engine.py b/gpt-st_amd/engine.py
--- a/gpt-st_amd/engine.py
+++ b/gpt-st_amd/engine.py
@@ -68,6 +68,8 @@
         self.fork_side = None
         self.forked = False
         self._dG = self._dA = None
+        self.want_tail = False
+        self.tail = False
 
     def take_carry(self, mb):
         if not CARRY_RED or self.no_carry or self.on_bucket is not None or CTX.NODE_REDUCE is not None or not self.jobs.jobs:
@@ -86,6 +88,11 @@
         c.jobs = take
         return c
 
+    def take_all(self):
+        c = ops.PoolJobs()
+        c.jobs, self.jobs.jobs = self.jobs.jobs, []
+        return c
+
     def untake(self, carry):
         if carry is not None and carry.jobs:
             self.jobs.jobs = carry.jobs + self.jobs.jobs
@@ -122,11 +129,16 @@
                 A = torch.as_strided(A, (A.shape[0] + A2.shape[0],) + tuple(A.shape[1:]), A.stride())
                 dG = torch.as_strided(dG, (dG.shape[0] + dG2.shape[0],) + tuple(dG.shape[1:]), dG.stride())
                 dA = torch.as_strided(dA, (dA.shape[0] + dA2.shape[0],) + tuple(dA.shape[1:]), dA.stride())
-            ops.gram_bwd(A, dG, out=dA, layers=A.shape[0] // N, nsplit=nsG)
-        self.jobs.jobs, self.late.jobs = self.jobs.jobs + self.late.jobs, []
-        self.jobs.launch()
+            ops.gram_bwd(A, dG, out=dA, layers=A.shape[0] // N, nsplit=nsG, jobs=self.jobs if self.tail else None)
         tf, self.tf = self.tf, []
-        ops.timefeat_jobs_bwd(tf, tidx)
+        if self.tail:
+            self.jobs.launch()
+            ops.timefeat_jobs_bwd(tf, tidx, jobs=self.late)
+        else:
+            self.jobs.jobs, self.late.jobs = self.jobs.jobs + self.late.jobs, []
+            self.jobs.launch()
+            ops.timefeat_jobs_bwd(tf, tidx)
+        self.tail = False
         self.keep = []
 
 
@@ -245,6 +257,7 @@
 CARRY_RED = os.environ.get("GPTST_CARRY_RED", "1") == "1"
 CARRY_MB = float(os.environ.get("GPTST_CARRY_MB", "25"))
 CARRY_KL = os.environ.get("GPTST_CARRY_KL", "1") == "1"
+TAIL_ROLES = os.environ.get("GPTST_TAIL_ROLES", "1") == "1"
 PAIR_UNDER_DP = os.environ.get("GPTST_PAIR_UNDER_DP", "1") == "1"
 PAIR_BWD = os.environ.get("GPTST_PAIR_BWD", "1") == "1"
 
@@ -268,6 +281,16 @@
 
 def cross_role():
     return 0 if CTX.NO_HANDOFFS else CROSS_ROLE
+
+
+TAIL_MAX_WG = 512
+
+
+def tail_roles_ok(red, dims, sv_e):
+    B, T, N, C = dims
+    return bool(TAIL_ROLES and red.want_tail and CARRY_RED and not red.no_carry and red.on_bucket is None and CTX.NODE_REDUCE is None
+                and cross_role() and FUSE_CROSS and CAP_LIN and C == 64 and T == 12 and sv_e is not None and isinstance(sv_e.h1, EncIn)
+                and B * T + 4 * B <= TAIL_MAX_WG)
 
 
 def _ht_pair_shape_ok(dims):
@@ -632,8 +655,9 @@
         assert chain
         e = sv.h1
         w, bi = p["encoder.dim_in_flow.weight"], p["encoder.dim_in_flow.bias"]
+        carry = red.take_all() if red.tail else None
         if nsG == B:
-            dWb, _, dinp = ops.encin_ht1_bwd(dd.view(B, T, N, C), e.source, e.mask, e.fill, w, bi, e.Wbt, e.ab, e.wv, dG=dG_all[0])
+            dWb, _, dinp = ops.encin_ht1_bwd(dd.view(B, T, N, C), e.source, e.mask, e.fill, w, bi, e.Wbt, e.ab, e.wv, dG=dG_all[0], jobs=carry)
         else:
             dWb, dGb, dinp = ops.encin_ht1_bwd(dd.view(B, T, N, C), e.source, e.mask, e.fill, w, bi, e.Wbt, e.ab, e.wv)
             torch.sum(dGb, 0, out=dG_all[0][0])
@@ -914,8 +938,13 @@
         chain = chain_ok(dims)
         done = kl.out if kl is not None else KlOut()
         _, dd = loss_tail(p, g, fw.dec, source, mask, base, sigma, mu, thresh, sws, red, chain=chain)
+        red.tail = chain and tail_roles_ok(red, dims, fw.sv_e)
+        kl_first = red.tail and with_kl and None not in (done.head, done.tem, done.inp)
+        if kl_first:
+            dh2 = kl_head(p, g, sv_g, prob, fw.c1, N, 0.1, sws, red, chain=chain, carried=done.head)
+            guide_bwd(p, g, source, tidx, sv_g, None, dims, base, red, dh2=dh2, chain=chain, carried=done)
         model_bwd(p, g, source, mask, tidx, fw.sv_e, fw.sv_d, fw.dec, None, None, dims, base, scaler_zeros, red, dd=dd, chain=chain)
-        if with_kl:
+        if with_kl and not kl_first:
             dh2 = kl_head(p, g, sv_g, prob, fw.c1, N, 0.1, sws, red, chain=chain, carried=done.head)
             guide_bwd(p, g, source, tidx, sv_g, None, dims, base, red, dh2=dh2, chain=chain, carried=done)
     else:
diff --git a/gpt-st_amd/ops.py b/gpt-st_amd/ops.py
--- a/gpt-st_amd/ops.py
+++ b/gpt-st_amd/ops.py
@@ -21,20 +21,22 @@
 CALL_LOCK = None
 
 
-def _call(name, *args, tag="", nbytes=0):
+def _call(name, *args, tag="", nbytes=0, entry=None):
+    fn = entry or name
     if CALL_LOCK is not None:
         with CALL_LOCK:
-            _C.lib().call(name, *args, _C.stream())
+            _C.lib().call(fn, *args, _C.stream())
         return
     if TIMER is None:
-        _C.lib().call(name, *args, _C.stream())
+        _C.lib().call(fn, *args, _C.stream())
         return
     e0, e1 = torch.cuda.Event(enable_timing=True), torch.cuda.Event(enable_timing=True)
     e0.record()
-    _C.lib().call(name, *args, _C.stream())
+    _C.lib().call(fn, *args, _C.stream())
     e1.record()
     TIMER.append((name, tag, e0, e1, nbytes))
-    LAST_CALL[(name, tag)] = args
+    if entry is None:
+        LAST_CALL[(name, tag)] = args
 
 
 def _nb(*ts):
@@ -175,6 +177,11 @@
     def columns(js, fields=PoolJob._fields):
         return [len(js)] + [(_ptrs0 if f in ("emb", "dW", "pool", "out") else _ints)([getattr(j, f) for j in js])
                             for f in PoolJob._fields if f in fields]
+
+    def take_reductions(self):
+        assert not self.post and all(j.kind in (self.BWD_POOL, self.BWD_EMB) for j in self.jobs)
+        js, self.jobs = self.jobs, []
+        return self.columns(js), "+jobs%d" % len(js), _nb(*[t for j in js for t in (j.emb, j.dW, j.pool, j.out)]), js
 
     def launch(self):
         js, self.jobs = self.jobs, []
@@ -260,10 +267,15 @@
     return G
 
 
-def gram_bwd(A, dG, out=None, layers=1, nsplit=1):
+def gram_bwd(A, dG, out=None, layers=1, nsplit=1, jobs=None):
     LN, Hm, T = A.shape
     dA = out if out is not None else torch.empty_like(A)
-    _call("gptst_gram_bwd", _p(A), _p(dG), _p(dA), layers, LN // layers, Hm, nsplit)
+    if jobs is not None and jobs.jobs:
+        cols, tag, nb, held = jobs.take_reductions()
+        _call("gptst_gram_bwd", _p(A), _p(dG), _p(dA), layers, LN // layers, Hm, nsplit, *cols, tag=tag, nbytes=nb, entry="gptst_gram_bwd_jobs")
+        del held
+    else:
+        _call("gptst_gram_bwd", _p(A), _p(dG), _p(dA), layers, LN // layers, Hm, nsplit)
     return dA
 
 
@@ -319,7 +331,7 @@
     return out, ab, wv
 
 
-def encin_ht1_bwd(dPre, source, mask, fill, w, bi, Wbt, ab, wv, dG=None):
+def encin_ht1_bwd(dPre, source, mask, fill, w, bi, Wbt, ab, wv, dG=None, jobs=None):
     B, T, N, F = source.shape
     C = Wbt.shape[-1]
     _chk(dPre, source, mask, w, bi, Wbt, ab, wv, dG)
@@ -327,8 +339,13 @@
     dWb, dinp = torch.empty(B * T, C * C + C, **f), torch.empty(B * T, 2 * C, **f)
     if dG is None:
         dG = torch.empty(B, N, T, T, **f)
-    _call("gptst_encin_ht1_bwd", _p(dPre), _p(source), F, _p(mask), float(fill), _p(w), _p(bi), _p(Wbt), _p(ab), _p(wv), _p(dWb), _p(dG), _p(dinp),
-          B, T, N, C, nbytes=_nb(dPre, Wbt, dWb, dG))
+    host = (_p(dPre), _p(source), F, _p(mask), float(fill), _p(w), _p(bi), _p(Wbt), _p(ab), _p(wv), _p(dWb), _p(dG), _p(dinp), B, T, N, C)
+    if jobs is not None and jobs.jobs:
+        cols, tag, nb, held = jobs.take_reductions()
+        _call("gptst_encin_ht1_bwd", *host, *cols, tag=tag, nbytes=_nb(dPre, Wbt, dWb, dG) + nb, entry="gptst_encin_ht1_bwd_jobs")
+        del held
+    else:
+        _call("gptst_encin_ht1_bwd", *host, nbytes=_nb(dPre, Wbt, dWb, dG))
     return dWb, dG, dinp
 
 
@@ -835,11 +852,19 @@
     return outs
 
 
-def timefeat_jobs_bwd(jobs, tidx):
-    if not jobs:
+def timefeat_jobs_bwd(tf, tidx, jobs=None):
+    if not tf:
+        if jobs is not None:
+            jobs.launch()
         return
-    _call("gptst_timefeat_jobs", len(jobs), 1, _ptrs([t for j in jobs for t in j.params]), _ptrs([t for j in jobs for t in j.grads]), _p(tidx),
-          _ptrs([j.dout for j in jobs]), _ints([j.rows for j in jobs]), _ints([j.K for j in jobs]), _ints([j.E for j in jobs]))
+    a = (_ptrs([t for j in tf for t in j.params]), _ptrs([t for j in tf for t in j.grads]), _p(tidx),
+         _ptrs([j.dout for j in tf]), _ints([j.rows for j in tf]), _ints([j.K for j in tf]), _ints([j.E for j in tf]))
+    if jobs is not None and jobs.jobs:
+        cols, tag, nb, held = jobs.take_reductions()
+        _call("gptst_timefeat_jobs", len(tf), *a, *cols, tag=tag, nbytes=nb, entry="gptst_timefeat_jobs_bwd_jobs")
+        del held
+    else:
+        _call("gptst_timefeat_jobs", len(tf), 1, *a)
 
 
 def mae_fwd(out, src, lda, mask, sigma, mu, thresh, rows, J, stats):
diff --git a/gpt-st_amd/step.py b/gpt-st_amd/step.py
--- a/gpt-st_amd/step.py
+++ b/gpt-st_amd/step.py
@@ -147,6 +147,7 @@
         gen = engine.gen_all(p, tidx, dims, guide=need_guide, defer=DEFER_GEN)
         red = engine.Reductions()
         red.no_carry = self.deterministic
+        red.want_tail = True
         self._dec_reduced = False
         if self.dp_overlap and self._dp_in_graph():
             red.on_bucket = self._bucket_ready
diff --git a/include/gptst_hip.h b/include/gptst_hip.h
--- a/include/gptst_hip.h
+++ b/include/gptst_hip.h
@@ -9,7 +9,7 @@
 #pragma GCC visibility push(default)
 #endif
 
-#define GPTST_ABI_VERSION 23
+#define GPTST_ABI_VERSION 24
 int gptst_abi_version(void);
 int gptst_set_deterministic(int on);
 int gptst_deterministic_state(void);
@@ -57,6 +57,10 @@
 
 int gptst_gram_fwd(const float* A, float* G, int N, int Hm, void* stream);
 int gptst_gram_bwd(const float* A, const float* dG, float* dA, int L, int N, int Hm, int nsplit, void* stream);
+int gptst_gram_bwd_jobs(const float* A, const float* dG, float* dA, int L, int N, int Hm, int nsplit,
+                        int njobs, const int* jkind, const void* const* jemb, const void* const* jx, const void* const* jpool,
+                        const void* const* jout, const int* jR, const int* jK, const int* jcols, const int* jnsplit, const int* jldx,
+                        void* stream);
 int gptst_tmix(const float* X, const float* G, const float* dOut, const float* Y, float* out, int B, int T, int N, int C,
                void* stream);
 int gptst_tmix_dgraph(const float* dR, const float* X, float* dG, int B, int T, int N, int C, void* stream);
@@ -78,6 +82,11 @@
 int gptst_encin_ht1_bwd(const float* dPre, const float* src, int lda, const float* mask, float fill, const float* w, const float* bi,
                         const float* Wbt, const float* ab, const float* wv, float* dWb, float* dG, float* dinp, int B, int T, int N, int C,
                         void* stream);
+int gptst_encin_ht1_bwd_jobs(const float* dPre, const float* src, int lda, const float* mask, float fill, const float* w, const float* bi,
+                             const float* Wbt, const float* ab, const float* wv, float* dWb, float* dG, float* dinp, int B, int T, int N, int C,
+                             int njobs, const int* jkind, const void* const* jemb, const void* const* jx, const void* const* jpool,
+                             const void* const* jout, const int* jR, const int* jK, const int* jcols, const int* jnsplit, const int* jldx,
+                             void* stream);
 
 int gptst_guide_in_fwd(const float* src, int lda, const float* w1, const float* b1, const float* Wn, const float* bn, float* h1, int BT, int N,
                        int C, void* stream);
@@ -268,6 +277,11 @@
 
 int gptst_timefeat_jobs(int njobs, int bwd, const void* const* params, const void* const* grads, const float* tidx,
                         const void* const* io, const int* rows, const int* K, const int* E, void* stream);
+int gptst_timefeat_jobs_bwd_jobs(int njobs, const void* const* params, const void* const* grads, const float* tidx, const void* const* io,
+                                 const int* rows, const int* K, const int* E,
+                                 int npj, const int* jkind, const void* const* jemb, const void* const* jx, const void* const* jpool,
+                                 const void* const* jout, const int* jR, const int* jK, const int* jcols, const int* jnsplit, const int* jldx,
+                                 void* stream);
 
 int gptst_step_begin(float* z0, long n0, float* z1, long n1, const float* src, float* tidx, int BT, int N, int lda, int base,
                      float* noise, long n_noise, const int* rng, void* stream);
```
